# spcl/gms

Hardware: AMD Instinct MI355X
Metric: edges-intersected/sec + achieved HBM GB/s, RMAT-26 triangle count @1/2/4/8 GPU (higher is better)
Workload: dtype int32 ids / uint64 counts

## Files before the change

### gms_amd/csrc/hip/device_graph.hip

```cpp
#include "device_graph.hpp"

#include <algorithm>
#include <mutex>
#include <array>
#include <chrono>
#include <cstdio>
#include <cstdlib>
#include <cstring>
#include <memory>
#include <new>
#include <random>

#include <rocprim/device/device_radix_sort.hpp>
#include <rocprim/device/device_scan.hpp>
#include <rocprim/device/device_segmented_radix_sort.hpp>
#include <rocprim/iterator/transform_iterator.hpp>

#include "../host/gmsx_internal.hpp"

namespace gmsx {

Ctx &ctx() {
    static Ctx c;
    return c;
// ... 173 lines not shown
            const uint32_t gap = uint32_t(row[i]) - cur;
            if (gap > 4095u) break;
            const int pos = 20 + 12 * (k - 1), word = pos >> 5, sh = pos & 31;
            w[word] |= gap << sh;
            if (sh > 20) w[word + 1] |= gap >> (32 - sh);
            ++k;
            cur = row[i];
            ++i;
        }
        w[0] |= uint32_t(k) << 16;
        if (emit) {
            emit[units * 4 + 0] = w[0]; emit[units * 4 + 1] = w[1]; emit[units * 4 + 2] = w[2]; emit[units * 4 + 3] = w[3];
        }
        ++units;
    }
    return units;
}
static constexpr int kHybridB[4] = {512, 1024, 2048, 4096};
__device__ inline int lower_bound_u16(const uint16_t *__restrict__ row, int len, uint32_t key) {
    int lo = 0, hi = len;
    while (lo < hi) {
        const int mid = (lo + hi) >> 1;
        if (uint32_t(row[mid]) < key) lo = mid + 1; else hi = mid;
    }
    return lo;
}
__global__ void k_srow_sizes(int64_t n, const int64_t *__restrict__ hoff, const uint16_t *__restrict__ hadj, const int32_t *__restrict__ dplus,
                             int32_t dense_limit, int delta_mode, int delta_pct, int gap12_mode, int hybrid_mode, int64_t *__restrict__ units_out,
                             int64_t *__restrict__ small_out, uint32_t *__restrict__ real_out, unsigned char *__restrict__ form_out,
                             int32_t *__restrict__ ksplit) {
    const int64_t v = int64_t(blockIdx.x) * blockDim.x + threadIdx.x;
    if (v > n) return;
    if (v == n) { units_out[2 * n] = 0; small_out[2 * n] = 0; return; }
    const int64_t b = hoff[v];
    const int len = int(hoff[v + 1] - b);
    uint32_t best = uint32_t((len + 7) / 8);
    int form = kFormList;
    if (len > 0 && v < dense_limit) {
        const uint32_t bits = uint32_t(bitset_words(int32_t(v)) / 4);
        if (bits * 16u + 32u < uint32_t(len) * 2u) { best = bits; form = kFormBitset; }
    }
    if (len > 0 && delta_mode > 0 && (delta_mode == 2 || len >= 24)) {
        const uint32_t d = delta_encode(hadj + b, len, nullptr);
        if ((delta_mode == 2 && form == kFormList) || d * 100u <= best * uint32_t(delta_pct)) { best = d; form = kFormDelta; }
    }
    if (len > 0 && gap12_mode > 0 && form == kFormList && (gap12_mode == 2 || len >= 24)) {
        const uint32_t d = gap12_encode(hadj + b, len, nullptr);
        if (gap12_mode == 2 || d * 100u <= best * 90u) { best = d; form = kFormGap12; }
    }
    uint32_t best2 = 0;
    int form2 = kFormList, ks = 0;
    if (hybrid_mode > 0 && len >= 32 && dplus[v] >= kHeavy && form != kFormBitset) {
        uint32_t tot = best;
        for (int t = 0; t < 4; ++t) {
            const int B = kHybridB[t];
            if (v <= B) break;
            const int k = lower_bound_u16(hadj + b, len, uint32_t(B));
            if (k * 2 <= B / 8 + 16) continue;
            const int rl = len - k;
            uint32_t r = uint32_t((rl + 7) / 8);
            int rf = kFormList;
            if (rl >= 24 && delta_mode > 0) {
                const uint32_t d = delta_encode(hadj + b + k, rl, nullptr);
                if (d * 100u <= r * uint32_t(delta_pct)) { r = d; rf = kFormDelta; }
            }
            const uint32_t cand = uint32_t(B / 128) + r;
            if (cand < tot && (hybrid_mode == 2 || cand * 100u <= best * 90u)) {
                tot = cand;
                ks = k;
                best2 = r;
                form2 = rf;
            }
        }
        if (ks > 0) {
            best = tot - best2;
            form = kFormBitset;
        }
    }
    ksplit[v] = ks;
    const uint32_t u2[2] = {best, best2};
    const int f2[2] = {form, form2};
    for (int sl = 0; sl < 2; ++sl) {
        const bool big = u2[sl] >= 8u;
        units_out[2 * v + sl] = big ? int64_t((u2[sl] + 7u) & ~7u) : 0;
        small_out[2 * v + sl] = big ? 0 : int64_t(u2[sl]);
        real_out[2 * v + sl] = u2[sl];
        form_out[2 * v + sl] = (unsigned char)f2[sl];
    }
}
__global__ void k_srow_fill(int64_t n, const int64_t *__restrict__ hoff, const uint16_t *__restrict__ hadj, const int64_t *__restrict__ bmoff,
                            const uint32_t *__restrict__ bmpool, const int64_t *__restrict__ uoff, const int64_t *__restrict__ soff,
                            const uint32_t *__restrict__ real, const unsigned char *__restrict__ form, const int32_t *__restrict__ ksplit,
                            unsigned long long *__restrict__ srow, unsigned long long *__restrict__ srow2, uint32_t *__restrict__ spool) {
    const int64_t v = int64_t(blockIdx.x) * blockDim.x + threadIdx.x;
    if (v >= n) return;
    const int64_t b = hoff[v];
    const int len = int(hoff[v + 1] - b);
    const int ks = ksplit[v];
    for (int sl = 0; sl < 2; ++sl) {
        const int64_t units = int64_t(real[2 * v + sl]);
        const int64_t u0 = units >= 8 ? uoff[2 * v + sl] : uoff[2 * n] + soff[2 * v + sl];
        const int fm = form[2 * v + sl];
        const unsigned long long d = units ? ((unsigned long long)u0 << 24) | ((unsigned long long)fm << 22) | (unsigned long long)units : 0ull;
        if (sl == 0) srow[v] = units ? d : ((unsigned long long)u0 << 24) | ((unsigned long long)fm << 22);
        else srow2[v] = d;
        if (units == 0) continue;
        uint32_t *dst = spool + u0 * 4;
        const uint16_t *row = hadj + b + (sl ? ks : 0);
        const int rl = sl ? len - ks : len;
        if (sl == 0 && ks > 0) {
            for (int64_t w = 0; w < units * 4; ++w) dst[w] = 0;
            for (int i = 0; i < ks; ++i) dst[row[i] >> 5] |= 1u << (row[i] & 31u);
        } else if (fm == kFormDelta) {
            delta_encode(row, rl, dst);
        } else if (fm == kFormGap12) {
            gap12_encode(row, rl, dst);
        } else if (fm == kFormBitset) {
            const uint32_t *src = bmpool + bmoff[v];
            for (int64_t w = 0; w < units * 4; ++w) dst[w] = src[w];
        } else {
            for (int64_t w = 0; w < units * 4; ++w) {
                const int i = int(w) * 2;
                const uint32_t lo = i < rl ? row[i] : 0xFFFFu, hi = i + 1 < rl ? row[i + 1] : 0xFFFFu;
                dst[w] = lo | (hi << 16);
            }
        }
    }
}

__device__ inline uint32_t tail_delta_encode(const int32_t *__restrict__ row, int len, uint32_t *__restrict__ emit) {
    uint32_t units = 0;
    int i = 0;
    while (i < len) {
        uint32_t w[4] = {uint32_t(row[i]), 0u, 0u, 0u};
        uint32_t cur = uint32_t(row[i]);
        int slot = 1;
        ++i;
        while (i < len && slot < 6) {
            const uint32_t gap = uint32_t(row[i]) - cur;
            if (gap > 65535u) break;
            w[1 + (slot >> 1)] |= gap << ((slot & 1) * 16);
            ++slot;
            cur = uint32_t(row[i]);
            ++i;
        }
        w[1] |= uint32_t(slot);
        if (emit) {
            emit[units * 4 + 0] = w[0]; emit[units * 4 + 1] = w[1]; emit[units * 4 + 2] = w[2]; emit[units * 4 + 3] = w[3];
        }
        ++units;
    }
    return units;
}
__global__ void k_trow_sizes(int64_t n, const int64_t *__restrict__ toff, const int32_t *__restrict__ tadj, int delta_mode,
                             int64_t *__restrict__ units_out, int64_t *__restrict__ small_out, uint32_t *__restrict__ real_out, unsigned char *__restrict__ form_out) {
    const int64_t v = int64_t(blockIdx.x) * blockDim.x + threadIdx.x;
    if (v > n) return;
    if (v == n) { units_out[n] = 0; small_out[n] = 0; return; }
    const int64_t b = toff[v];
    const int len = int(toff[v + 1] - b);
    uint32_t best = uint32_t((len + 3) / 4);
    int form = kFormList;
    if (len >= 8 && delta_mode > 0) {
        const uint32_t d = tail_delta_encode(tadj + b, len, nullptr);
        if (delta_mode == 2 || d * 100u <= best * 85u) { best = d; form = kFormDelta; }
    }
    const bool big = best >= 8u;
    units_out[v] = big ? int64_t((best + 7u) & ~7u) : 0;
    small_out[v] = big ? 0 : int64_t(best);
    real_out[v] = best;
    form_out[v] = (unsigned char)form;
}
__global__ void k_trow_fill(int64_t n, const int64_t *__restrict__ toff, const int32_t *__restrict__ tadj, const int64_t *__restrict__ uoff,
                            const int64_t *__restrict__ soff, const uint32_t *__restrict__ real, const unsigned char *__restrict__ form,
                            unsigned long long *__restrict__ trow, uint32_t *__restrict__ tpool) {
    const int64_t v = int64_t(blockIdx.x) * blockDim.x + threadIdx.x;
    if (v >= n) return;
    const int64_t units = int64_t(real[v]);
    const int64_t u0 = units >= 8 ? uoff[v] : uoff[n] + soff[v];
    trow[v] = ((unsigned long long)u0 << 24) | ((unsigned long long)form[v] << 22) | (unsigned long long)units;
    if (units == 0) return;
    uint32_t *dst = tpool + u0 * 4;
    const int64_t b = toff[v];
    const int64_t len = toff[v + 1] - b;
    if (form[v] == kFormDelta) tail_delta_encode(tadj + b, int(len), dst);
    else
        for (int64_t w = 0; w < units * 4; ++w) dst[w] = w < len ? uint32_t(tadj[b + w]) : 0xfffffffeu;
}

__global__ void k_dense_sizes(int32_t limit, const int32_t *__restrict__ dplus, int64_t *__restrict__ sizes) {
    const int32_t v = int32_t(blockIdx.x * blockDim.x + threadIdx.x);
    if (v < limit) sizes[v] = bitset_words(v);
    if (v == limit) sizes[v] = 0;
}
__global__ __launch_bounds__(256) void k_dense_fill(int32_t limit, const int64_t *__restrict__ hoff, const uint16_t *__restrict__ hadj,
                                                    const int64_t *__restrict__ toff, const int32_t *__restrict__ tadj,
                                                    const int64_t *__restrict__ bmoff, uint32_t *__restrict__ pool) {
    const int lane = threadIdx.x & 63;
    const int32_t wave0 = int32_t((int64_t(blockIdx.x) * blockDim.x + threadIdx.x) >> 6);
    const int32_t nwaves = int32_t((int64_t(gridDim.x) * blockDim.x) >> 6);
    for (int32_t v = wave0; v < limit; v += nwaves) {
        const int64_t b = bmoff[v];
        if (bmoff[v + 1] == b) continue;
        for (int64_t j = hoff[v] + lane; j < hoff[v + 1]; j += 64) {
            const uint32_t id = hadj[j];
            if (id != 0xFFFFu) atomicOr(&pool[b + (id >> 5)], 1u << (id & 31u));
        }
        for (int64_t j = toff[v] + lane; j < toff[v + 1]; j += 64) {
            const uint32_t id = uint32_t(tadj[j]);
            atomicOr(&pool[b + (id >> 5)], 1u << (id & 31u));
        }
    }
}
__global__ __launch_bounds__(256) void k_tail_split(int64_t n, const int64_t *__restrict__ toff, const int32_t *__restrict__ tadj, int32_t limit,
                                                    int32_t *__restrict__ tsplit) {
    const int lane = threadIdx.x & 63;
    const int64_t wave0 = (int64_t(blockIdx.x) * blockDim.x + threadIdx.x) >> 6;
    const int64_t nwaves = (int64_t(gridDim.x) * blockDim.x) >> 6;
    for (int64_t u = wave0; u < n; u += nwaves) {
        int c = 0;
        for (int64_t j = toff[u] + lane; j < toff[u + 1]; j += 64) c += tadj[j] < limit;
        for (int s = 32; s > 0; s >>= 1) c += __shfl_down(c, s);
        if (lane == 0) tsplit[u] = c;
    }
}

__global__ void k_order_keys(int64_t n, const int32_t *__restrict__ dplus, int32_t *__restrict__ keys, int32_t *__restrict__ vals) {
    const int64_t i = int64_t(blockIdx.x) * blockDim.x + threadIdx.x;
    if (i < n) {
        keys[i] = dplus[i];
        vals[i] = int32_t(i);
    }
}

__global__ void k_warm(unsigned long long *p) {
    if (p) p[0] = 0;
}
__global__ void k_count_ge(int64_t n, const int32_t *__restrict__ order, const int32_t *__restrict__ dplus, int32_t thr, int64_t *__restrict__ out) {
    int64_t lo = 0, hi = n;
    while (lo < hi) {
        const int64_t mid = (lo + hi) >> 1;
        if (dplus[order[mid]] >= thr) lo = mid + 1; else hi = mid;
    }
    out[0] = lo;
}
__global__ void k_task_limits(int64_t n, const unsigned long long *__restrict__ srow, const unsigned long long *__restrict__ srow2,
                              const unsigned long long *__restrict__ trow, uint32_t hub_max, uint32_t tail_max, unsigned long long *__restrict__ out) {
    const int64_t v = int64_t(blockIdx.x) * blockDim.x + threadIdx.x;
    if (v >= n) return;
    if ((srow[v] & 0x3fffffull) > hub_max || (srow2[v] & 0x3fffffull) > hub_max || (trow[v] & 0x3fffffull) > tail_max) atomicOr(out, 1ull);
}

static constexpr int kInlineChunk = 64;
static constexpr int kDefaultInlineFirst = 28;
static constexpr int kInlineFirstMax = 64;
__device__ __forceinline__ bool takes_inline(int32_t v, int32_t inline_limit, const int32_t *__restrict__ dplus) {
    return v < inline_limit || dplus[v] >= kHeavy;
}
template <bool FILL>
__global__ __launch_bounds__(256) void k_inline_rows(int64_t first, int64_t end, const int32_t *__restrict__ order, const int64_t *__restrict__ hoff,
                                                     const uint16_t *__restrict__ hadj, const int64_t *__restrict__ toff, const int32_t *__restrict__ tadj,
                                                     const int32_t *__restrict__ dplus, int32_t inline_limit, int inline_first, const int32_t *__restrict__ opos, int nparts, int part,
                                                     unsigned long long *__restrict__ cnt_h,
                                                     unsigned long long *__restrict__ cnt_t, const int64_t *__restrict__ ihoff,
                                                     const int64_t *__restrict__ itoff, int64_t base_h, uint16_t *__restrict__ pool_h, int64_t base_t,
                                                     int32_t *__restrict__ pool_t) {
    const int lane = threadIdx.x & 63;
    const int64_t wave0 = (int64_t(blockIdx.x) * blockDim.x + threadIdx.x) >> 6;
    const int64_t nwaves = (int64_t(gridDim.x) * blockDim.x) >> 6;
    for (int64_t pos = first + wave0; pos < end; pos += nwaves) {
        const int32_t u = order[pos];
        const int64_t hb = hoff[u], tb = toff[u];
        const int first_u = dplus[u] >= kHeavy ? inline_first : kInlineFirstMax;
        const int hl = min(int(hoff[u + 1] - hb), first_u), tl = min(int(toff[u + 1] - tb), first_u - hl);
        int32_t mv = 0x7fffffff;
        if (lane < hl) {
            const uint32_t x = hadj[hb + lane];
            if (x != 0xFFFFu) mv = int32_t(x);
        } else if (lane - hl < tl) {
            mv = tadj[tb + (lane - hl)];
        }
        const bool valid = mv != 0x7fffffff, is_tail = valid && lane >= hl;
        const unsigned long long vmask = __ballot(valid);
        const int nhub = __popcll(__ballot(valid && lane < hl));
        const int below = __popcll(vmask & ((1ull << lane) - 1ull));
        const bool give = valid && below > 0 && takes_inline(mv, inline_limit, dplus);
        const bool mine = give && (nparts <= 1 || shard_of(opos[mv], nparts) == part);
        const int nh = mine ? (is_tail ? nhub : below) : 0;
        const int nt = mine && is_tail ? lane - hl : 0;
        if (!FILL) {
            if (nh) atomicAdd(&cnt_h[mv], (unsigned long long)nh);
            if (nt) atomicAdd(&cnt_t[mv], (unsigned long long)nt);
        } else {
            int64_t at_h = 0, at_t = 0;
            if (nh) at_h = (base_h + ihoff[mv]) * 8 + int64_t(atomicAdd(&cnt_h[mv], (unsigned long long)nh));
            if (nt) at_t = (base_t + itoff[mv]) * 4 + int64_t(atomicAdd(&cnt_t[mv], (unsigned long long)nt));
            for (int k = 0; k < nhub; ++k) {
                const int32_t x = __shfl(mv, k);
                if (k < nh) pool_h[at_h + k] = uint16_t(x);
            }
            for (int k = 0; k < tl; ++k) {
                const int32_t x = __shfl(mv, hl + k);
                if (k < nt) pool_t[at_t + k] = x;
            }
        }
    }
}
__global__ void k_inline_units(int64_t n, const unsigned long long *__restrict__ ids_h, const unsigned long long *__restrict__ ids_t,
                               int64_t *__restrict__ units_h, int64_t *__restrict__ units_t) {
    const int64_t v = int64_t(blockIdx.x) * blockDim.x + threadIdx.x;
    if (v > n) return;
    units_h[v] = v < n ? int64_t((ids_h[v] + 7) / 8) : 0;
    units_t[v] = v < n ? int64_t((ids_t[v] + 3) / 4) : 0;
}
static constexpr int kDefaultHotWindows = 0, kDefaultHotKB = 2048, kDefaultHotMin = 16;
__device__ __forceinline__ int64_t receiver_of(int32_t w, const int32_t *__restrict__ dplus, const int32_t *__restrict__ opos, const int64_t *__restrict__ lidx,
                                               int64_t n_heavy) {
    return dplus[w] >= kHeavy ? int64_t(opos[w]) : n_heavy + lidx[w];
}
__global__ void k_opos(int64_t n, const int32_t *__restrict__ order, int32_t *__restrict__ opos) {
    const int64_t p = int64_t(blockIdx.x) * blockDim.x + threadIdx.x;
    if (p < n) opos[order[p]] = int32_t(p);
}
__global__ void k_light_flags(int64_t limit, const int32_t *__restrict__ dplus, int64_t *__restrict__ flags) {
    const int64_t w = int64_t(blockIdx.x) * blockDim.x + threadIdx.x;
    if (w <= limit) flags[w] = (w < limit && dplus[w] < kHeavy) ? 1 : 0;
}
__global__ void k_recv_vertices(int64_t n_heavy, int64_t limit, const int32_t *__restrict__ order, const int32_t *__restrict__ dplus, const int64_t *__restrict__ lidx,
                                int32_t *__restrict__ recv_v) {
    const int64_t i = int64_t(blockIdx.x) * blockDim.x + threadIdx.x;
    if (i < n_heavy) recv_v[i] = order[i];
    if (i < limit && dplus[i] < kHeavy) recv_v[n_heavy + lidx[i]] = int32_t(i);
}
template <bool FILL>
__global__ void k_inline_entries(int64_t n, const int32_t *__restrict__ dplus, const int32_t *__restrict__ opos, const int64_t *__restrict__ lidx, int64_t n_heavy,
                                 int32_t inline_limit, const int64_t *__restrict__ ihoff, const int64_t *__restrict__ itoff, int64_t base_h, int64_t base_t,
                                 uint32_t *__restrict__ cnt, uint32_t *__restrict__ cur, const int64_t *__restrict__ hbeg, const int64_t *__restrict__ tbeg,
                                 TaskList htask, TaskList ttask, unsigned long long *__restrict__ totals, TcClasses cc) {
    const int kClasses = cc.count();
    const int64_t v = int64_t(blockIdx.x) * blockDim.x + threadIdx.x;
    if (v >= n) return;
    const int64_t uh = ihoff[v + 1] - ihoff[v], ut = itoff[v + 1] - itoff[v];
    if (uh == 0 && ut == 0) return;
    if (dplus[v] < kHeavy && v >= inline_limit) return;
    const int64_t p = receiver_of(int32_t(v), dplus, opos, lidx, n_heavy);
    uint32_t *c = cnt + p * kClasses;
    for (int64_t o = 0; o < uh; o += kInlineChunk) {
        const unsigned long long units = (unsigned long long)min(int64_t(kInlineChunk), uh - o);
        const unsigned long long d = ((unsigned long long)(base_h + ihoff[v] + o) << 24) | ((unsigned long long)kFormList << 22) | units;
        const int cls = hub_class(cc, d);
        if (!FILL) atomicAdd(&c[cls], 1u);
        else htask.put(hbeg[p] + c[cls] + atomicAdd(&cur[p * kClasses + cls], 1u), d);
    }
    for (int64_t o = 0; o < ut; o += kInlineChunk) {
        const unsigned long long units = (unsigned long long)min(int64_t(kInlineChunk), ut - o);
        const unsigned long long d = ((unsigned long long)(base_t + itoff[v] + o) << 24) | ((unsigned long long)kFormList << 22) | units;
        const int cls = tail_class(cc, d);
        if (!FILL) atomicAdd(&c[cls], 1u);
        else ttask.put(tbeg[p] + c[cls] + atomicAdd(&cur[p * kClasses + cls], 1u), d);
    }
    if (!FILL) {
        atomicAdd(&totals[0], (unsigned long long)((uh + kInlineChunk - 1) / kInlineChunk));
        atomicAdd(&totals[1], (unsigned long long)((ut + kInlineChunk - 1) / kInlineChunk));
    }
}
__global__ void k_list_sizes(int64_t n_recv, uint32_t *__restrict__ cnt, int64_t *__restrict__ hcnt, int64_t *__restrict__ tcnt, TcClasses cc) {
    const int kClasses = cc.count(), hub_end = cc.tail_base();
    const int64_t p = int64_t(blockIdx.x) * blockDim.x + threadIdx.x;
    if (p > n_recv) return;
    if (p == n_recv) { hcnt[p] = 0; tcnt[p] = 0; return; }
    uint32_t *c = cnt + p * kClasses;
    uint32_t run = 0;
    for (int k = 0; k < hub_end; ++k) { const uint32_t x = c[k]; c[k] = run; run += x; }
    hcnt[p] = run;
    run = 0;
    for (int k = hub_end; k < kClasses; ++k) { const uint32_t x = c[k]; c[k] = run; run += x; }
    tcnt[p] = run;
}

__global__ void k_ledge_count(int64_t first, int64_t end, const int32_t *__restrict__ order, const int64_t *__restrict__ toff, const int32_t *__restrict__ tadj,
                              const int32_t *__restrict__ tsplit, const int32_t *__restrict__ dplus, int64_t *__restrict__ cnt) {
    const int64_t pos = first + int64_t(blockIdx.x) * blockDim.x + threadIdx.x;
    if (pos > end) return;
    int64_t c = 0;
    if (pos < end) {
        const int32_t u = order[pos];
        const int64_t tb = toff[u];
        const int tl = int(toff[u + 1] - tb);
        for (int i = tsplit[u]; i < tl; ++i) c += dplus[tadj[tb + i]] < kHeavy ? 1 : 0;
    }
    cnt[pos - first] = c;
}
__global__ void k_ledge_fill(int64_t first, int64_t end, const int32_t *__restrict__ order, const int64_t *__restrict__ hoff, const int64_t *__restrict__ toff,
                             const int32_t *__restrict__ tadj, const int32_t *__restrict__ tsplit, const int32_t *__restrict__ dplus,
                             const int64_t *__restrict__ ebeg, int nparts, int part, uint4 *__restrict__ ledge) {
    const int64_t pos = first + int64_t(blockIdx.x) * blockDim.x + threadIdx.x;
    if (pos >= end) return;
    const int32_t u = order[pos];
    const int64_t hb = hoff[u], tb = toff[u];
    const int tl = int(toff[u + 1] - tb);
    const unsigned long long hu = (unsigned long long)hb | ((unsigned long long)(hoff[u + 1] - hb) << 40);
    int64_t e = ebeg[pos - first];
    for (int i = tsplit[u]; i < tl; ++i) {
        const int32_t v = tadj[tb + i];
        if (dplus[v] >= kHeavy) continue;
        if (nparts <= 1 || shard_of(e, nparts) == part) {
            const unsigned long long tu = (unsigned long long)tb | ((unsigned long long)i << 40);
            const unsigned long long hv = (unsigned long long)hoff[v] | ((unsigned long long)(hoff[v + 1] - hoff[v]) << 40);
            const unsigned long long tv = (unsigned long long)toff[v] | ((unsigned long long)(toff[v + 1] - toff[v]) << 40);
            const int64_t slot = nparts <= 1 ? e : e / nparts;
            ledge[2 * slot] = make_uint4(uint32_t(hu), uint32_t(hu >> 32), uint32_t(tu), uint32_t(tu >> 32));
            ledge[2 * slot + 1] = make_uint4(uint32_t(hv), uint32_t(hv >> 32), uint32_t(tv), uint32_t(tv >> 32));
        }
        ++e;
    }
}

__device__ __forceinline__ uint32_t cut_hub_units(const uint32_t *__restrict__ spool, unsigned long long d, int below, int32_t v) {
    const uint32_t units = uint32_t(d) & 0x3fffffu, form = (uint32_t(d) >> 22) & 3u;
    if (form == kFormList) return min(units, uint32_t(below + 7) / 8u);
    if (form == kFormBitset) return min(units, uint32_t(v + 127) / 128u);
    const uint4 *row = reinterpret_cast<const uint4 *>(spool) + (d >> 24);
    uint32_t lo = 0, hi = units;
    while (lo < hi) {
        const uint32_t mid = (lo + hi) >> 1;
        if (int32_t(row[mid].x & 0xffffu) < v) lo = mid + 1; else hi = mid;
    }
    return lo;
}
__device__ __forceinline__ uint32_t cut_tail_units(const uint32_t *__restrict__ tpool, unsigned long long d, int below, int32_t v) {
    const uint32_t units = uint32_t(d) & 0x3fffffu, form = (uint32_t(d) >> 22) & 3u;
    if (form != kFormDelta) return min(units, uint32_t(below + 3) / 4u);
    const uint4 *row = reinterpret_cast<const uint4 *>(tpool) + (d >> 24);
    uint32_t lo = 0, hi = units;
    while (lo < hi) {
        const uint32_t mid = (lo + hi) >> 1;
        if (int32_t(row[mid].x) < v) lo = mid + 1; else hi = mid;
    }
    return lo;
}
__device__ __forceinline__ uint32_t claim_by_class(uint32_t *ctr, int cls, bool active, int lane) {
    uint32_t mine = 0;
    unsigned long long todo = __ballot(active);
    while (todo) {
        const int leader = __ffsll((long long)todo) - 1;
        const int c = __builtin_amdgcn_readlane(cls, leader);
        const unsigned long long same = __ballot(active && cls == c);
        uint32_t base = 0;
        if (lane == leader) base = atomicAdd(&ctr[c], uint32_t(__popcll(same)));
        base = uint32_t(__builtin_amdgcn_readlane(int(base), leader));
        if (active && cls == c) mine = base + uint32_t(__popcll(same & ((1ull << lane) - 1ull)));
        todo &= ~same;
    }
    return mine;
}
template <bool FILL>
__global__ __launch_bounds__(256) void k_task_lists(int64_t n_heavy, const int32_t *__restrict__ order, const int64_t *__restrict__ hoff,
                                                    const uint16_t *__restrict__ hadj, const int64_t *__restrict__ toff, const int32_t *__restrict__ tadj,
                                                    const int32_t *__restrict__ dplus, const unsigned long long *__restrict__ srow,
                                                    const unsigned long long *__restrict__ srow2, const int32_t *__restrict__ ksplit,
                                                    const unsigned long long *__restrict__ trow, int two_sided, const int32_t *__restrict__ opos,
                                                    uint32_t *__restrict__ cnt, uint32_t *__restrict__ cur, const int64_t *__restrict__ hbeg,
                                                    const int64_t *__restrict__ tbeg, TaskList htask, TaskList ttask,
                                                    int32_t *__restrict__ tunits, unsigned long long *__restrict__ reversed, const uint32_t *__restrict__ spool,
                                                    const uint32_t *__restrict__ tpool, int32_t inline_limit, int inline_first, int nparts, int part, TcClasses cc) {
    const int kClasses = cc.count();
    const int lane = threadIdx.x & 63;
    const int64_t wave0 = (int64_t(blockIdx.x) * blockDim.x + threadIdx.x) >> 6;
    const int64_t nwaves = (int64_t(gridDim.x) * blockDim.x) >> 6;
    unsigned long long rev = 0;
    for (int64_t pos = wave0; pos < n_heavy; pos += nwaves) {
        const int32_t u = order[pos];
        const int64_t hb = hoff[u], tb = toff[u];
        const int hl = int(hoff[u + 1] - hb), tl = int(toff[u + 1] - tb);
        const unsigned long long du_s = srow[u], du_s2 = srow2[u], du_t = trow[u];
        const int ks_u = ksplit[u];
        uint32_t *cu = cnt + pos * kClasses, *ru = cur + pos * kClasses;
        const bool own_u = nparts <= 1 || shard_of(pos, nparts) == part;
        int kept = 0;
        for (int base = 0; base < hl + tl; base += 64) {
            const int i = base + lane;
            int32_t v = -1;
            if (i < hl) {
                const uint32_t x = hadj[hb + i];
                if (x != 0xFFFFu) v = int32_t(x);
            } else if (i < hl + tl) v = tadj[tb + i - hl];
            if (v >= 0 && i > 0 && i < inline_first && takes_inline(v, inline_limit, dplus)) v = -1;
            bool reverse = false;
            uint32_t ch = 0, ch2 = 0, ct = 0;
            if (v >= 0 && i > 0 && two_sided && dplus[v] >= kHeavy) {
                if (i < hl) {
                    ch = cut_hub_units(spool, du_s, i, v);
                    if (du_s2 && i > ks_u) ch2 = cut_hub_units(spool, du_s2, i - ks_u, v);
                } else {
                    ch = uint32_t(du_s) & 0x3fffffu;
                    ch2 = uint32_t(du_s2) & 0x3fffffu;
                }
                ct = (i < hl || toff[v + 1] == toff[v]) ? 0u : cut_tail_units(tpool, du_t, i - hl, v);
                const uint32_t keep = uint32_t(srow[v] & 0x3fffffull) + uint32_t(srow2[v] & 0x3fffffull) + (i > hl ? uint32_t(trow[v] & 0x3fffffull) : 0u);
                reverse = ch + ch2 + ct < keep;
            }
            const bool fwd = v >= 0 && !reverse && own_u;
            if (reverse && nparts > 1 && shard_of(opos[v], nparts) != part) v = -1;
            const unsigned long long fh = (fwd && i > 0) ? srow[v] : 0ull, fh2 = (fwd && i > 0) ? srow2[v] : 0ull, ft = (fwd && i > hl) ? trow[v] : 0ull;
            const bool fh_on = (fh & 0x3fffffull) != 0, fh2_on = (fh2 & 0x3fffffull) != 0, ft_on = (ft & 0x3fffffull) != 0;
            const uint32_t sh = claim_by_class(FILL ? ru : cu, hub_class(cc, fh), fh_on, lane);
            const uint32_t sh2 = claim_by_class(FILL ? ru : cu, hub_class(cc, fh2), fh2_on, lane);
            const uint32_t st = claim_by_class(FILL ? ru : cu, tail_class(cc, ft), ft_on, lane);
            if (FILL) {
                if (fh_on) htask.put(hbeg[pos] + cu[hub_class(cc, fh)] + sh, fh);
                if (fh2_on) htask.put(hbeg[pos] + cu[hub_class(cc, fh2)] + sh2, fh2);
                if (ft_on) ttask.put(tbeg[pos] + cu[tail_class(cc, ft)] + st, ft);
            }
            kept += __popcll(__ballot(fwd));
            if (v >= 0 && reverse) {
                const int64_t pv = opos[v];
                const unsigned long long rh = ch ? (du_s & ~0x3fffffull) | ch : 0ull, rh2 = ch2 ? (du_s2 & ~0x3fffffull) | ch2 : 0ull,
                                         rt = ct ? (du_t & ~0x3fffffull) | ct : 0ull;
                uint32_t *cv = cnt + pv * kClasses;
                if (!FILL) {
                    if (rh) atomicAdd(&cv[hub_class(cc, rh)], 1u);
                    if (rh2) atomicAdd(&cv[hub_class(cc, rh2)], 1u);
                    if (rt) atomicAdd(&cv[tail_class(cc, rt)], 1u);
                    atomicAdd(&tunits[pv], 1);
                    ++rev;
                } else {
                    uint32_t *rv = cur + pv * kClasses;
                    if (rh) htask.put(hbeg[pv] + cv[hub_class(cc, rh)] + atomicAdd(&rv[hub_class(cc, rh)], 1u), rh);
                    if (rh2) htask.put(hbeg[pv] + cv[hub_class(cc, rh2)] + atomicAdd(&rv[hub_class(cc, rh2)], 1u), rh2);
                    if (rt) ttask.put(tbeg[pv] + cv[tail_class(cc, rt)] + atomicAdd(&rv[tail_class(cc, rt)], 1u), rt);
                }
            }
        }
        if (!FILL && lane == 0 && kept) atomicAdd(&tunits[pos], kept);
    }
    if (!FILL) {
        for (int s = 32; s > 0; s >>= 1) rev += __shfl_down(rev, s);
        if (lane == 0 && rev) atomicAdd(reversed, rev);
    }
}
__global__ void k_item_counts(int64_t n_recv, const int64_t *__restrict__ lbeg, const uint32_t *__restrict__ cnt, TcClasses cc, int phases, int64_t *__restrict__ items) {
    const int64_t p = int64_t(blockIdx.x) * blockDim.x + threadIdx.x;
    if (p > n_recv) return;
    if (p == n_recv) { items[int64_t(phases) * n_recv] = 0; return; }
    for (int ph = 0; ph < phases; ++ph) {
        int64_t b = 0, e = lbeg[p + 1] - lbeg[p];
        if (phases > 1) hub_phase_range(cc, cnt + p * cc.count(), e, ph, &b, &e);
        items[int64_t(ph) * n_recv + p] = (e - b + kTaskChunk - 1) / kTaskChunk;
    }
}
__global__ void k_item_fill(int64_t n_recv, const int32_t *__restrict__ recv_v, const int32_t *__restrict__ opos, const int64_t *__restrict__ lbeg,
                            const int64_t *__restrict__ ioff, TaskList task, const int64_t *__restrict__ coff, int kind,
                            const uint32_t *__restrict__ cnt, TcClasses cc, int phases, gmsx_tc_item *__restrict__ items) {
    const int64_t p = int64_t(blockIdx.x) * blockDim.x + threadIdx.x;
    if (p >= n_recv) return;
    const int32_t w = recv_v[p];
    const uint64_t cont = uint64_t(coff[w]) | (uint64_t(coff[w + 1] - coff[w]) << 40);
    for (int ph = 0; ph < phases; ++ph) {
    int64_t b = 0, e = lbeg[p + 1] - lbeg[p];
    if (phases > 1) hub_phase_range(cc, cnt + p * cc.count(), e, ph, &b, &e);
    b += lbeg[p];
    e += lbeg[p];
    int64_t k = ioff[int64_t(ph) * n_recv + p];
    for (int64_t x = b; x < e; x += kTaskChunk, ++k) {
        const int ne = int(min(int64_t(kTaskChunk), e - x));
        gmsx_tc_item it{};
        it.bc = uint64_t(x) | (uint64_t(ne) << 40);
        it.cont = cont;
        it.pivot = w;
        it.pos = opos[w];
        it.kind = uint32_t(kind);
        for (int f = 0; f < 4; ++f) {
            int lo = 0, hi = ne;
            while (lo < hi) {
                const int mid = (lo + hi) >> 1;
                if (int((uint32_t(task.get(x + mid)) >> 22) & 3u) < f) lo = mid + 1; else hi = mid;
            }
            it.fbeg[f] = uint16_t(lo);
        }
        items[k] = it;
    }
    }
}

static int grid_for_waves(int64_t rows) {
    const int64_t want = (rows + 3) / 4;
    const int64_t cap = int64_t(ctx().compute_units > 0 ? ctx().compute_units : 256) * 32;
    return int(want < 1 ? 1 : (want > cap ? cap : want));
}

template <class T>
static int dmalloc(T **p, int64_t count, gmsx_graph *g, int line = __builtin_LINE()) {
    const size_t bytes = size_t(count > 0 ? count : 1) * sizeof(T);
    const bool trace = opt("MEM_TRACE") != nullptr;
    if (trace && g && bytes >= (1u << 20)) std::fprintf(stderr, "gmsx mem: device_graph.hip:%d %.3f GB (elements of %zu B)\n", line, double(bytes) * 1e-9, sizeof(T));
    if (g && g->tc_building && g->tc_limit_bytes > 0 && g->device_bytes + int64_t(bytes) - g->tc_base_bytes > g->tc_limit_bytes) {
        *p = nullptr;
        return GMSX_ERR_DEVICE_MEM;
    }
    if (hipMalloc(reinterpret_cast<void **>(p), bytes) != hipSuccess) {
        (void)hipGetLastError();
        *p = nullptr;
        return GMSX_ERR_DEVICE_MEM;
    }
    if (g) g->device_bytes += int64_t(bytes);
    return GMSX_OK;
}

struct DevGuard {
    void *p;
    ~DevGuard() { (void)hipFree(p); }
};

static void free_tc(gmsx_graph *g) {
    auto drop = [](auto *&p) {
        (void)hipFree(p);
        p = nullptr;
    };
    drop(g->tsplit); drop(g->srow); drop(g->srow2); drop(g->ksplit); drop(g->spool); drop(g->trow); drop(g->htask.lo); drop(g->htask.hi); drop(g->ttask.lo); drop(g->ttask.hi); drop(g->hitem); drop(g->titem); drop(g->tunits);
    drop(g->ledge); drop(g->tpool); drop(g->shard_hitem); drop(g->shard_titem);
    g->shard_idx_part = g->shard_idx_nparts = -1;
    g->device_bytes -= g->tc_bytes;
    g->tc_bytes = 0;
    g->tc_ready = false;
    g->htask_entries = g->ttask_entries = g->hitems = g->titems = g->inline_hentries = g->inline_tentries = 0;
    g->n_ledge = g->ledge_total = 0;
    g->task_reverse = g->inline_units = g->spool_units = g->tpool_units = 0;
    g->stats_part = g->stats_nparts = -1;
}

static void free_graph(gmsx_graph *g) {
    if (!g) return;
    (void)hipFree(g->off);
    (void)hipFree(g->adj);
    (void)hipFree(g->newid);
    (void)hipFree(g->oldid);
    (void)hipFree(g->hoff);
    (void)hipFree(g->hadj);
    (void)hipFree(g->toff);
    (void)hipFree(g->tadj);
    (void)hipFree(g->bmoff);
    (void)hipFree(g->bmpool);
    (void)hipFree(g->tsplit);
    (void)hipFree(g->srow);
    (void)hipFree(g->srow2);
    (void)hipFree(g->ksplit);
    (void)hipFree(g->spool);
    (void)hipFree(g->trow);
    (void)hipFree(g->htask.lo);
    (void)hipFree(g->htask.hi);
    (void)hipFree(g->ttask.lo);
    (void)hipFree(g->ttask.hi);
    (void)hipFree(g->hitem);
    (void)hipFree(g->titem);
    (void)hipFree(g->tunits);
    (void)hipFree(g->shard_hitem);
    (void)hipFree(g->shard_titem);
    (void)hipFree(g->ledge);
    (void)hipFree(g->tpool);
    (void)hipFree(g->dplus);
    (void)hipFree(g->order);
    (void)hipFree(g->kc_rel);
    (void)hipFree(g->kc_aoff);
    (void)hipFree(g->kc_arena);
    (void)hipFree(g->kc_rec);
    (void)hipFree(g->kc_item);
    (void)hipFree(g->kc_relt);
    (void)hipFree(g->kc_rect);
    (void)hipFree(g->kc_itemt);
    (void)hipFree(g->scratch);
    (void)hipFree(g->acc);
    delete g;
}

int exclusive_scan_i64(const int64_t *in, int64_t *out, int64_t count, hipStream_t s) {
    size_t tmp_bytes = 0;
    GMSX_HIP(rocprim::exclusive_scan(nullptr, tmp_bytes, in, out, int64_t(0), size_t(count), rocprim::plus<int64_t>(), s));
    void *tmp = nullptr;
    GMSX_HIP(hipMalloc(&tmp, tmp_bytes ? tmp_bytes : 8));
    DevGuard g_tmp{tmp};
    GMSX_HIP(rocprim::exclusive_scan(tmp, tmp_bytes, in, out, int64_t(0), size_t(count), rocprim::plus<int64_t>(), s));
    GMSX_HIP(hipStreamSynchronize(s));
    return GMSX_OK;
}

struct OffsetMinus {
    int64_t base;
    __host__ __device__ int64_t operator()(int64_t x) const { return x - base; }
};
__global__ void k_lower_bound_i64(int64_t count, const int64_t *__restrict__ a, int64_t target, int64_t *__restrict__ out) {
    int64_t lo = 0, hi = count;
    while (lo < hi) {
        const int64_t mid = (lo + hi) >> 1;
        if (a[mid] < target) lo = mid + 1; else hi = mid;
    }
    out[0] = lo;
}
template <class K>
static int sort_rows(K *keys, int64_t entries, int64_t n, const int64_t *d_off, int end_bit, hipStream_t s) {
    if (n <= 0 || entries <= 0) return GMSX_OK;
    int64_t chunk = int64_t(1) << 31;
    if (const char *e = opt("SORT_CHUNK")) {
        const long long v = std::atoll(e);
        if (v > 0) chunk = v;
    }
    int64_t *d_v = nullptr;
    GMSX_HIP(hipMalloc(reinterpret_cast<void **>(&d_v), sizeof(int64_t)));
    DevGuard g_v{d_v};
    GMSX_HIP(hipStreamSynchronize(s));
    int64_t v0 = 0, base = 0;
    while (v0 < n) {
        int64_t v1 = n;
        if (entries - base > chunk) {
            hipLaunchKernelGGL(k_lower_bound_i64, dim3(1), dim3(1), 0, s, n + 1, d_off, base + chunk + 1, d_v);
            GMSX_HIP(hipStreamSynchronize(s));
            GMSX_HIP(hipMemcpy(&v1, d_v, sizeof(int64_t), hipMemcpyDeviceToHost));
            v1 = std::max(v0 + 1, std::min(n, v1 - 1));
        }
        int64_t end = 0;
        GMSX_HIP(hipMemcpy(&end, d_off + v1, sizeof(int64_t), hipMemcpyDeviceToHost));
        const int64_t cnt = end - base;
        if (cnt >= (int64_t(1) << 32)) return GMSX_ERR_UNSUPPORTED;
        if (cnt > 0) {
            K *sorted = nullptr;
            GMSX_HIP(hipMalloc(reinterpret_cast<void **>(&sorted), size_t(cnt) * sizeof(K)));
            DevGuard g_sorted{sorted};
            auto begin = rocprim::make_transform_iterator(d_off + v0, OffsetMinus{base});
            auto endit = rocprim::make_transform_iterator(d_off + v0 + 1, OffsetMinus{base});
            size_t tmp_bytes = 0;
            GMSX_HIP(rocprim::segmented_radix_sort_keys(nullptr, tmp_bytes, keys + base, sorted, unsigned(cnt), unsigned(v1 - v0), begin, endit, 0, end_bit, s));
            void *tmp = nullptr;
            GMSX_HIP(hipMalloc(&tmp, tmp_bytes ? tmp_bytes : 8));
            DevGuard g_tmp{tmp};
            GMSX_HIP(rocprim::segmented_radix_sort_keys(tmp, tmp_bytes, keys + base, sorted, unsigned(cnt), unsigned(v1 - v0), begin, endit, 0, end_bit, s));
            GMSX_HIP(hipMemcpyAsync(keys + base, sorted, size_t(cnt) * sizeof(K), hipMemcpyDeviceToDevice, s));
            GMSX_HIP(hipStreamSynchronize(s));
        }
        v0 = v1;
        base = end;
    }
    return GMSX_OK;
}

template <class K, class V>
static int sort_segment_pairs(K *keys, V *vals, int64_t entries, int64_t n, const int64_t *d_off, int end_bit, hipStream_t s) {
    if (n <= 0 || entries <= 0) return GMSX_OK;
    int64_t chunk = int64_t(1) << 31;
    if (const char *e = opt("SORT_CHUNK")) {
        const long long v = std::atoll(e);
        if (v > 0) chunk = v;
    }
    int64_t *d_v = nullptr;
    GMSX_HIP(hipMalloc(reinterpret_cast<void **>(&d_v), sizeof(int64_t)));
    DevGuard g_v{d_v};
    GMSX_HIP(hipStreamSynchronize(s));
    int64_t v0 = 0, base = 0;
    while (v0 < n) {
        int64_t v1 = n;
        if (entries - base > chunk) {
            hipLaunchKernelGGL(k_lower_bound_i64, dim3(1), dim3(1), 0, s, n + 1, d_off, base + chunk + 1, d_v);
            GMSX_HIP(hipStreamSynchronize(s));
            GMSX_HIP(hipMemcpy(&v1, d_v, sizeof(int64_t), hipMemcpyDeviceToHost));
            v1 = std::max(v0 + 1, std::min(n, v1 - 1));
        }
        int64_t end = 0;
        GMSX_HIP(hipMemcpy(&end, d_off + v1, sizeof(int64_t), hipMemcpyDeviceToHost));
        const int64_t cnt = end - base;
        if (cnt >= (int64_t(1) << 32)) return GMSX_ERR_UNSUPPORTED;
        if (cnt > 0) {
            K *k_out = nullptr;
            V *v_out = nullptr;
            GMSX_HIP(hipMalloc(reinterpret_cast<void **>(&k_out), size_t(cnt) * sizeof(K)));
            DevGuard g_ko{k_out};
            GMSX_HIP(hipMalloc(reinterpret_cast<void **>(&v_out), size_t(cnt) * sizeof(V)));
            DevGuard g_vo{v_out};
            auto begin = rocprim::make_transform_iterator(d_off + v0, OffsetMinus{base});
            auto endit = rocprim::make_transform_iterator(d_off + v0 + 1, OffsetMinus{base});
            size_t tmp_bytes = 0;
            GMSX_HIP(rocprim::segmented_radix_sort_pairs(nullptr, tmp_bytes, keys + base, k_out, vals + base, v_out, unsigned(cnt), unsigned(v1 - v0), begin, endit, 0,
                                                         end_bit, s));
            void *tmp = nullptr;
            GMSX_HIP(hipMalloc(&tmp, tmp_bytes ? tmp_bytes : 8));
            DevGuard g_tmp{tmp};
            GMSX_HIP(rocprim::segmented_radix_sort_pairs(tmp, tmp_bytes, keys + base, k_out, vals + base, v_out, unsigned(cnt), unsigned(v1 - v0), begin, endit, 0,
                                                         end_bit, s));
            GMSX_HIP(hipMemcpyAsync(vals + base, v_out, size_t(cnt) * sizeof(V), hipMemcpyDeviceToDevice, s));
            GMSX_HIP(hipStreamSynchronize(s));
        }
        v0 = v1;
        base = end;
    }
    return GMSX_OK;
}

struct PhaseTimer {
    hipStream_t s;
    bool on;
    std::chrono::steady_clock::time_point t0;
    const char *what;
    PhaseTimer(hipStream_t st, const char *w) : s(st), on(opt("TIMING") != nullptr), t0(std::chrono::steady_clock::now()), what(w) {}
    void mark(const char *phase) {
        if (!on) return;
        (void)hipStreamSynchronize(s);
        const auto t1 = std::chrono::steady_clock::now();
        std::fprintf(stderr, "[gmsx %s] %-28s %8.1f ms\n", what, phase, std::chrono::duration<double, std::milli>(t1 - t0).count());
        t0 = t1;
    }
};

static constexpr size_t kH2dChunk = size_t(64) << 20;
struct H2dStage {
    char *pin[2] = {nullptr, nullptr};
// ... 36 lines not shown
    for (size_t at = 0; at < bytes; at += kChunk, b ^= 1) {
        const size_t n = std::min(kChunk, bytes - at);
        if (used[b]) GMSX_HIP(hipEventSynchronize(st.ev[b]));
        char *to = st.pin[b];
        parallel_memcpy(to, static_cast<const char *>(src) + at, n);
        GMSX_HIP(hipMemcpyAsync(static_cast<char *>(dst) + at, to, n, hipMemcpyHostToDevice, s));
        GMSX_HIP(hipEventRecord(st.ev[b], s));
        used[b] = true;
    }
    return GMSX_OK;
}

static int build_device_sets(gmsx_graph *g, uint32_t flags) {
    hipStream_t s = ctx().stream;
    PhaseTimer pt(s, "base build");
    const int64_t n = g->n;
    if (int rc = dmalloc(&g->scratch, 16, g)) return rc;
    if (int rc = dmalloc(&g->acc, kAccWords, g)) return rc;
    GMSX_HIP(hipMemsetAsync(g->scratch, 0, 16 * sizeof(unsigned long long), s));

    const int check_sym = (flags & GMSX_UPLOAD_TRUSTED) ? 0 : 1;
    static const std::array<unsigned long long, 2> sym_keys = []() noexcept {
        try {
            std::random_device rd;
            return std::array<unsigned long long, 2>{((unsigned long long)rd() << 32) | rd(), ((unsigned long long)rd() << 32) | rd()};
        } catch (...) {
            const unsigned long long t = (unsigned long long)std::chrono::steady_clock::now().time_since_epoch().count();
            const unsigned long long a = (unsigned long long)reinterpret_cast<uintptr_t>(&t);
            return std::array<unsigned long long, 2>{t * 0x9E3779B97F4A7C15ull ^ a, (a * 0xC2B2AE3D27D4EB4Full) ^ (t << 17)};
        }
    }();
    if (n > 0)
        hipLaunchKernelGGL(k_validate, dim3(grid_for_waves(n)), dim3(256), 0, s, n, g->off, g->adj, check_sym, sym_keys[0], sym_keys[1], g->scratch);
    unsigned long long acc[7] = {0, 0, 0, 0, 0, 0, 0};
    GMSX_HIP(hipMemcpyAsync(acc, g->scratch, sizeof(acc), hipMemcpyDeviceToHost, s));
    GMSX_HIP(hipStreamSynchronize(s));
    if (check_sym && (acc[3] != acc[4] || acc[5] != acc[6])) acc[0] |= 8;
    if (!(flags & GMSX_UPLOAD_TRUSTED) && acc[0] != 0) return GMSX_ERR_NOT_CANONICAL;
    if ((flags & GMSX_UPLOAD_TRUSTED) && (acc[0] & 2)) return GMSX_ERR_NOT_CANONICAL;
    if (!(flags & GMSX_UPLOAD_TRUSTED) && (g->nnz & 1)) return GMSX_ERR_NOT_CANONICAL;
    g->alg_elements = acc[1];
    g->max_deg = int32_t(acc[2]);
    g->m = g->nnz / 2;

    pt.mark("validate");
    const unsigned tb = unsigned((n + 255) / 256);
    if (int rc = dmalloc(&g->newid, n, g)) return rc;
    if (int rc = dmalloc(&g->oldid, n, g)) return rc;
    if (n > 0) {
        unsigned long long *k_in = nullptr, *k_out = nullptr;
        if (int rc = dmalloc(&k_in, n, nullptr)) return rc;
        DevGuard g1{k_in};
        if (int rc = dmalloc(&k_out, n, nullptr)) return rc;
        DevGuard g2{k_out};
        hipLaunchKernelGGL(k_rank_keys, dim3(tb), dim3(256), 0, s, n, g->off, k_in);
        size_t tmp_bytes = 0;
        GMSX_HIP(rocprim::radix_sort_keys_desc(nullptr, tmp_bytes, k_in, k_out, size_t(n), 0, 64, s));
        void *tmp = nullptr;
        GMSX_HIP(hipMalloc(&tmp, tmp_bytes ? tmp_bytes : 8));
        DevGuard g3{tmp};
        GMSX_HIP(rocprim::radix_sort_keys_desc(tmp, tmp_bytes, k_in, k_out, size_t(n), 0, 64, s));
        hipLaunchKernelGGL(k_assign_ids, dim3(tb), dim3(256), 0, s, n, k_out, g->oldid, g->newid);
        GMSX_HIP(hipStreamSynchronize(s));
    }

    pt.mark("rank ids");
    int hub_limit = int((flags >> 8) & 0xffffu);
    if (hub_limit == 0 || hub_limit > kHub) hub_limit = kHub;
    int64_t *hcnt = nullptr, *tcnt = nullptr;
    if (int rc = dmalloc(&hcnt, n + 1, nullptr)) return rc;
    DevGuard g_h{hcnt};
    if (int rc = dmalloc(&tcnt, n + 1, nullptr)) return rc;
    DevGuard g_t{tcnt};
    GMSX_HIP(hipMemsetAsync(hcnt, 0, size_t(n + 1) * sizeof(int64_t), s));
    GMSX_HIP(hipMemsetAsync(tcnt, 0, size_t(n + 1) * sizeof(int64_t), s));
    if (int rc = dmalloc(&g->dplus, n, g)) return rc;
    if (n > 0)
        hipLaunchKernelGGL(k_count_parts, dim3(grid_for_waves(n)), dim3(256), 0, s, n, g->off, g->adj, g->newid, hub_limit, hcnt, tcnt, g->dplus);
    if (int rc = dmalloc(&g->hoff, n + 1, g)) return rc;
    if (int rc = dmalloc(&g->toff, n + 1, g)) return rc;
    if (int rc = exclusive_scan_i64(hcnt, g->hoff, n + 1, s)) return rc;
    if (int rc = exclusive_scan_i64(tcnt, g->toff, n + 1, s)) return rc;
    GMSX_HIP(hipMemcpy(&g->hub_entries, g->hoff + n, sizeof(int64_t), hipMemcpyDeviceToHost));
    GMSX_HIP(hipMemcpy(&g->tail_entries, g->toff + n, sizeof(int64_t), hipMemcpyDeviceToHost));

    if (int rc = dmalloc(&g->hadj, g->hub_entries + 8, g)) return rc;
    if (int rc = dmalloc(&g->tadj, g->tail_entries + 4, g)) return rc;
    GMSX_HIP(hipMemsetAsync(g->hadj + g->hub_entries, 0xff, 8 * sizeof(uint16_t), s));
    GMSX_HIP(hipMemsetAsync(g->tadj + g->tail_entries, 0xff, 4 * sizeof(int32_t), s));
    if (n > 0)
        hipLaunchKernelGGL(k_fill_parts, dim3(grid_for_waves(n)), dim3(256), 0, s, n, g->off, g->adj, g->newid, hub_limit, g->hoff, g->toff,
                           g->hadj, g->tadj);

    pt.mark("containers count+fill");
    if (int rc = sort_rows(g->hadj, g->hub_entries, n, g->hoff, 16, s)) return rc;
    if (int rc = sort_rows(g->tadj, g->tail_entries, n, g->toff, 32, s)) return rc;
    g->rows_sorted = true;

    pt.mark("row sorts");
    g->dense_limit = int32_t(std::min<int64_t>(n, hub_limit));
    g->bitset_limit = g->dense_limit;
    {
        const int32_t K = g->bitset_limit;
        int64_t *sizes = nullptr;
        if (int rc = dmalloc(&sizes, int64_t(K) + 1, nullptr)) return rc;
        DevGuard g_sz{sizes};
        if (int rc = dmalloc(&g->bmoff, int64_t(K) + 1, g)) return rc;
        hipLaunchKernelGGL(k_dense_sizes, dim3(unsigned(K / 256 + 1)), dim3(256), 0, s, K, g->dplus, sizes);
        if (int rc = exclusive_scan_i64(sizes, g->bmoff, int64_t(K) + 1, s)) return rc;
        GMSX_HIP(hipMemcpy(&g->bmpool_words, g->bmoff + K, sizeof(int64_t), hipMemcpyDeviceToHost));
        if (int rc = dmalloc(&g->bmpool, g->bmpool_words + 4, g)) return rc;
        GMSX_HIP(hipMemsetAsync(g->bmpool, 0, size_t(g->bmpool_words + 4) * sizeof(uint32_t), s));
        if (K > 0 && g->bmpool_words > 0)
            hipLaunchKernelGGL(k_dense_fill, dim3(grid_for_waves(K)), dim3(256), 0, s, K, g->hoff, g->hadj, g->toff, g->tadj, g->bmoff, g->bmpool);
    }
    pt.mark("bitsets");
    if (int rc = dmalloc(&g->order, n, g)) return rc;
    if (n > 0) {
        int32_t *keys_in = nullptr, *vals_in = nullptr, *keys_out = nullptr;
        if (int rc = dmalloc(&keys_out, n, nullptr)) return rc;
        DevGuard g_ko{keys_out};
        if (int rc = dmalloc(&keys_in, n, nullptr)) return rc;
        DevGuard g_ki{keys_in};
        if (int rc = dmalloc(&vals_in, n, nullptr)) return rc;
        DevGuard g_vi{vals_in};
        hipLaunchKernelGGL(k_order_keys, dim3(tb), dim3(256), 0, s, n, g->dplus, keys_in, vals_in);
        size_t tmp_bytes = 0;
        GMSX_HIP(rocprim::radix_sort_pairs_desc(nullptr, tmp_bytes, keys_in, keys_out, vals_in, g->order, size_t(n), 0, 32, s));
        void *tmp = nullptr;
        GMSX_HIP(hipMalloc(&tmp, tmp_bytes ? tmp_bytes : 8));
        DevGuard g_tmp{tmp};
        GMSX_HIP(rocprim::radix_sort_pairs_desc(tmp, tmp_bytes, keys_in, keys_out, vals_in, g->order, size_t(n), 0, 32, s));
        int32_t top = 0;
        GMSX_HIP(hipMemcpyAsync(&top, keys_out, sizeof(int32_t), hipMemcpyDeviceToHost, s));
        GMSX_HIP(hipStreamSynchronize(s));
        g->max_dplus = top;
    }

    pt.mark("d+ order");
    GMSX_HIP(hipStreamSynchronize(s));
    GMSX_HIP(hipGetLastError());
    g->hub_limit = hub_limit;
    g->upload_flags = flags;
    return GMSX_OK;
}

static int build_tc_sets(gmsx_graph *g) {
    hipStream_t s = ctx().stream;
    PhaseTimer pt(s, "tc build");
    const int64_t n = g->n;
    const uint32_t flags = g->upload_flags;
    const int hub_limit = g->hub_limit;
    const unsigned tb = unsigned((n + 255) / 256);
    int32_t *opos = nullptr;
    if (int rc = dmalloc(&opos, n + 1, nullptr)) return rc;
    DevGuard g_opos{opos};
    if (n > 0) hipLaunchKernelGGL(k_opos, dim3(tb), dim3(256), 0, s, n, g->order, opos);
    {
        int64_t want = std::min<int64_t>(524288, n / 256);
        bool forced = false;
        if (const char *e = opt("INLINE_LIMIT")) {
            const long long v = std::atoll(e);
            if (v >= 0 && v <= (1ll << 31) - 1) { want = v; forced = true; }
        }
        if (!forced && ((flags >> 8) & 0xffffu)) want = int64_t(4) * hub_limit;
        g->inline_limit = int32_t(std::min<int64_t>(n, std::max<int64_t>(want, g->dense_limit)));
        g->inline_first = kDefaultInlineFirst;
        if (const char *e = opt("TC_INLINE_FIRST")) g->inline_first = std::max(1, std::min(kInlineFirstMax, std::atoi(e)));
        if (int rc = dmalloc(&g->tsplit, n, g)) return rc;
        if (n > 0) hipLaunchKernelGGL(k_tail_split, dim3(grid_for_waves(n)), dim3(256), 0, s, n, g->toff, g->tadj, g->inline_limit, g->tsplit);
    }

    pt.mark("tail split");
    int64_t n_heavy = 0, n_work = 0;
    unsigned long long *inl_h = nullptr, *inl_t = nullptr;
    int64_t *ihoff = nullptr, *itoff = nullptr;
    if (int rc = dmalloc(&inl_h, n + 1, nullptr)) return rc;
    DevGuard g_inl_h{inl_h};
    if (int rc = dmalloc(&inl_t, n + 1, nullptr)) return rc;
    DevGuard g_inl_t{inl_t};
    if (int rc = dmalloc(&ihoff, n + 1, nullptr)) return rc;
    DevGuard g_ihoff{ihoff};
    if (int rc = dmalloc(&itoff, n + 1, nullptr)) return rc;
    DevGuard g_itoff{itoff};
    int64_t inline_h_units = 0, inline_t_units = 0;
    {
        if (n > 0) {
            int64_t *d_cnt = nullptr;
            if (int rc = dmalloc(&d_cnt, 2, nullptr)) return rc;
            DevGuard g_c{d_cnt};
            hipLaunchKernelGGL(k_count_ge, dim3(1), dim3(1), 0, s, n, g->order, g->dplus, int32_t(kHeavy), d_cnt);
            hipLaunchKernelGGL(k_count_ge, dim3(1), dim3(1), 0, s, n, g->order, g->dplus, int32_t(2), d_cnt + 1);
            GMSX_HIP(hipStreamSynchronize(s));
            int64_t h[2] = {0, 0};
            GMSX_HIP(hipMemcpy(h, d_cnt, sizeof(h), hipMemcpyDeviceToHost));
            n_heavy = h[0];
            n_work = h[1];
        }
        GMSX_HIP(hipMemsetAsync(inl_h, 0, size_t(n + 1) * sizeof(unsigned long long), s));
        GMSX_HIP(hipMemsetAsync(inl_t, 0, size_t(n + 1) * sizeof(unsigned long long), s));
        if (n_work > 0)
            hipLaunchKernelGGL(k_inline_rows<false>, dim3(grid_for_waves(n_work)), dim3(256), 0, s, int64_t(0), n_work, g->order, g->hoff, g->hadj,
                               g->toff, g->tadj, g->dplus, g->inline_limit, g->inline_first, opos, g->shard_nparts, g->shard_part, inl_h, inl_t, ihoff, itoff, int64_t(0), static_cast<uint16_t *>(nullptr),
                               int64_t(0), static_cast<int32_t *>(nullptr));
        int64_t *uh = nullptr, *ut = nullptr;
        if (int rc = dmalloc(&uh, n + 1, nullptr)) return rc;
        DevGuard g_uh{uh};
        if (int rc = dmalloc(&ut, n + 1, nullptr)) return rc;
        DevGuard g_ut{ut};
        hipLaunchKernelGGL(k_inline_units, dim3(unsigned(n / 256 + 1)), dim3(256), 0, s, n, inl_h, inl_t, uh, ut);
        if (int rc = exclusive_scan_i64(uh, ihoff, n + 1, s)) return rc;
        if (int rc = exclusive_scan_i64(ut, itoff, n + 1, s)) return rc;
        GMSX_HIP(hipMemcpy(&inline_h_units, ihoff + n, sizeof(int64_t), hipMemcpyDeviceToHost));
        GMSX_HIP(hipMemcpy(&inline_t_units, itoff + n, sizeof(int64_t), hipMemcpyDeviceToHost));
        g->inline_units = inline_h_units + inline_t_units;
    }

    pt.mark("inline row sizes");
    int64_t inline_h_base = 0, inline_t_base = 0;
    {
        int delta_mode = g->rows_sorted ? 1 : 0;
        if (const char *e = opt("TC_DELTA")) {
            const int v = std::atoi(e);
            if (v >= 0 && v <= 2 && g->rows_sorted) delta_mode = v;
        }
        int delta_pct = 85;
        if (const char *e = opt("TC_DELTA_PCT")) {
            const int v = std::atoi(e);
            if (v >= 10 && v <= 100) delta_pct = v;
        }
        int gap12_mode = 0;
        if (const char *e = opt("TC_GAP12")) {
            const int v = std::atoi(e);
            if (v >= 0 && v <= 2 && g->rows_sorted) gap12_mode = v;
        }
        int hybrid_mode = 0;
        if (const char *e = opt("TC_HYBRID")) {
            const int v = std::atoi(e);
            if (v >= 0 && v <= 2 && g->rows_sorted) hybrid_mode = v;
        }
        int64_t *units = nullptr, *uoff = nullptr, *small = nullptr, *soff = nullptr;
        uint32_t *real = nullptr;
        unsigned char *form = nullptr;
        const int64_t n2 = 2 * n;
        if (int rc = dmalloc(&units, n2 + 1, nullptr)) return rc;
        DevGuard g_u{units};
        if (int rc = dmalloc(&uoff, n2 + 1, nullptr)) return rc;
        DevGuard g_o{uoff};
        if (int rc = dmalloc(&small, n2 + 1, nullptr)) return rc;
        DevGuard g_s{small};
        if (int rc = dmalloc(&soff, n2 + 1, nullptr)) return rc;
        DevGuard g_so{soff};
        if (int rc = dmalloc(&real, n2 + 1, nullptr)) return rc;
        DevGuard g_r{real};
        if (int rc = dmalloc(&form, n2 + 1, nullptr)) return rc;
        DevGuard g_f{form};
        if (int rc = dmalloc(&g->ksplit, n + 1, g)) return rc;
        hipLaunchKernelGGL(k_srow_sizes, dim3(unsigned(n / 256 + 1)), dim3(256), 0, s, n, g->hoff, g->hadj, g->dplus, g->dense_limit, delta_mode, delta_pct, gap12_mode,
                           hybrid_mode, units, small, real, form, g->ksplit);
        if (int rc = exclusive_scan_i64(units, uoff, n2 + 1, s)) return rc;
        if (int rc = exclusive_scan_i64(small, soff, n2 + 1, s)) return rc;
        int64_t big_units = 0, small_units = 0;
        GMSX_HIP(hipMemcpy(&big_units, uoff + n2, sizeof(int64_t), hipMemcpyDeviceToHost));
        GMSX_HIP(hipMemcpy(&small_units, soff + n2, sizeof(int64_t), hipMemcpyDeviceToHost));
        g->spool_units = big_units + small_units + inline_h_units;
        inline_h_base = big_units + small_units;
        if (g->spool_units >= (int64_t(1) << 40)) return GMSX_ERR_DEVICE_MEM;
        if (int rc = dmalloc(&g->srow, n, g)) return rc;
        if (int rc = dmalloc(&g->srow2, n, g)) return rc;
        if (int rc = dmalloc(&g->spool, (g->spool_units + kPoolSlack) * 4, g)) return rc;
        GMSX_HIP(hipMemsetAsync(g->spool, 0, size_t((g->spool_units + kPoolSlack) * 4) * sizeof(uint32_t), s));
        if (inline_h_units > 0) GMSX_HIP(hipMemsetAsync(g->spool + inline_h_base * 4, 0xff, size_t(inline_h_units) * 16, s));
        if (n > 0)
            hipLaunchKernelGGL(k_srow_fill, dim3(unsigned((n + 255) / 256)), dim3(256), 0, s, n, g->hoff, g->hadj, g->bmoff, g->bmpool, uoff, soff, real, form,
                               g->ksplit, g->srow, g->srow2, g->spool);
        GMSX_HIP(hipStreamSynchronize(s));
    }
    {
        int delta_mode = g->rows_sorted ? 1 : 0;
        if (const char *e = opt("TC_TAIL_DELTA")) {
            const int v = std::atoi(e);
            if (v >= 0 && v <= 2 && g->rows_sorted) delta_mode = v;
        }
        int64_t *units = nullptr, *uoff = nullptr, *small = nullptr, *soff = nullptr;
        uint32_t *real = nullptr;
        unsigned char *form = nullptr;
        if (int rc = dmalloc(&units, n + 1, nullptr)) return rc;
        DevGuard g_u{units};
        if (int rc = dmalloc(&uoff, n + 1, nullptr)) return rc;
        DevGuard g_o{uoff};
        if (int rc = dmalloc(&small, n + 1, nullptr)) return rc;
        DevGuard g_s{small};
        if (int rc = dmalloc(&soff, n + 1, nullptr)) return rc;
        DevGuard g_so{soff};
        if (int rc = dmalloc(&real, n + 1, nullptr)) return rc;
        DevGuard g_r{real};
        if (int rc = dmalloc(&form, n + 1, nullptr)) return rc;
        DevGuard g_f{form};
        hipLaunchKernelGGL(k_trow_sizes, dim3(unsigned(n / 256 + 1)), dim3(256), 0, s, n, g->toff, g->tadj, delta_mode, units, small, real, form);
        if (int rc = exclusive_scan_i64(units, uoff, n + 1, s)) return rc;
        if (int rc = exclusive_scan_i64(small, soff, n + 1, s)) return rc;
        int64_t big_units = 0, small_units = 0;
        GMSX_HIP(hipMemcpy(&big_units, uoff + n, sizeof(int64_t), hipMemcpyDeviceToHost));
        GMSX_HIP(hipMemcpy(&small_units, soff + n, sizeof(int64_t), hipMemcpyDeviceToHost));
        inline_t_base = big_units + small_units;
        g->tpool_units = inline_t_base + inline_t_units;
        if (g->tpool_units >= (int64_t(1) << 40)) return GMSX_ERR_DEVICE_MEM;
        if (int rc = dmalloc(&g->trow, n, g)) return rc;
        if (int rc = dmalloc(&g->tpool, (g->tpool_units + kPoolSlack) * 4, g)) return rc;
        GMSX_HIP(hipMemsetD32Async(reinterpret_cast<hipDeviceptr_t>(g->tpool), int(0xFFFFFFFEu), size_t(g->tpool_units + kPoolSlack) * 4, s));
        if (n > 0)
            hipLaunchKernelGGL(k_trow_fill, dim3(unsigned((n + 255) / 256)), dim3(256), 0, s, n, g->toff, g->tadj, uoff, soff, real, form, g->trow, g->tpool);
        GMSX_HIP(hipStreamSynchronize(s));
    }

    pt.mark("tail stream rows");
    if (n_work > 0) {
        GMSX_HIP(hipMemsetAsync(inl_h, 0, size_t(n + 1) * sizeof(unsigned long long), s));
        GMSX_HIP(hipMemsetAsync(inl_t, 0, size_t(n + 1) * sizeof(unsigned long long), s));
        hipLaunchKernelGGL(k_inline_rows<true>, dim3(grid_for_waves(n_work)), dim3(256), 0, s, int64_t(0), n_work, g->order, g->hoff, g->hadj, g->toff,
                           g->tadj, g->dplus, g->inline_limit, g->inline_first, opos, g->shard_nparts, g->shard_part, inl_h, inl_t, ihoff, itoff, inline_h_base, reinterpret_cast<uint16_t *>(g->spool),
                           inline_t_base, reinterpret_cast<int32_t *>(g->tpool));
    }
    pt.mark("inline rows fill");
    {
        const int64_t nl = n_work - n_heavy;
        g->n_ledge = g->ledge_total = 0;
        if (nl > 0) {
            int64_t *ecnt = nullptr, *ebeg = nullptr;
            if (int rc = dmalloc(&ecnt, nl + 1, nullptr)) return rc;
            DevGuard g_ec{ecnt};
            if (int rc = dmalloc(&ebeg, nl + 1, nullptr)) return rc;
            DevGuard g_eb{ebeg};
            hipLaunchKernelGGL(k_ledge_count, dim3(unsigned(nl / 256 + 1)), dim3(256), 0, s, n_heavy, n_work, g->order, g->toff, g->tadj, g->tsplit, g->dplus, ecnt);
            if (int rc = exclusive_scan_i64(ecnt, ebeg, nl + 1, s)) return rc;
            GMSX_HIP(hipMemcpy(&g->ledge_total, ebeg + nl, sizeof(int64_t), hipMemcpyDeviceToHost));
            const int np = g->shard_nparts > 1 ? g->shard_nparts : 1, pp = g->shard_nparts > 1 ? g->shard_part : 0;
            {
                const int64_t full = g->ledge_total / np, rem = g->ledge_total % np;
                g->n_ledge = np <= 1 ? g->ledge_total : full + (((full & 1) ? np - 1 - pp : pp) < rem ? 1 : 0);
            }
            if (int rc = dmalloc(&g->ledge, 2 * g->n_ledge + 2, g)) return rc;
            hipLaunchKernelGGL(k_ledge_fill, dim3(unsigned(nl / 256 + 1)), dim3(256), 0, s, n_heavy, n_work, g->order, g->hoff, g->toff, g->tadj, g->tsplit, g->dplus, ebeg,
                               np, pp, g->ledge);
            GMSX_HIP(hipStreamSynchronize(s));
        }
    }
    pt.mark("light pivot list");
    {
        int two_sided = 1;
        if (const char *e = opt("TC_TWO_SIDED")) two_sided = std::atoi(e) != 0;
        const unsigned vb = unsigned(n / 256 + 1);
        const int64_t L = g->inline_limit;
        int64_t *lflag = nullptr, *lidx = nullptr;
        if (int rc = dmalloc(&lflag, L + 1, nullptr)) return rc;
        DevGuard g_lf{lflag};
        if (int rc = dmalloc(&lidx, L + 1, nullptr)) return rc;
        DevGuard g_li{lidx};
        hipLaunchKernelGGL(k_light_flags, dim3(unsigned(L / 256 + 1)), dim3(256), 0, s, L, g->dplus, lflag);
        if (int rc = exclusive_scan_i64(lflag, lidx, L + 1, s)) return rc;
        int64_t n_light_recv = 0;
        GMSX_HIP(hipMemcpy(&n_light_recv, lidx + L, sizeof(int64_t), hipMemcpyDeviceToHost));
        const int64_t n_recv = n_heavy + n_light_recv;
        int32_t *recv_v = nullptr;
        if (int rc = dmalloc(&recv_v, n_recv + 1, nullptr)) return rc;
        DevGuard g_rv{recv_v};
        if (std::max<int64_t>(n_heavy, L) > 0)
            hipLaunchKernelGGL(k_recv_vertices, dim3(unsigned(std::max<int64_t>(n_heavy, L) / 256 + 1)), dim3(256), 0, s, n_heavy, L, g->order, g->dplus, lidx, recv_v);
        {
            auto env_int = [](const char *name, int dflt) { return int(opt_int(name, dflt)); };
            g->tc_hot_windows = std::max(0, std::min(kMaxHotWindows, env_int("TC_HOT_WINDOWS", kDefaultHotWindows)));
            g->tc_window_units = uint32_t(std::max(1, env_int("TC_HOT_KB", kDefaultHotKB))) * 64u;
            g->tc_hot_min = std::max(1, env_int("TC_HOT_MIN", kDefaultHotMin));
        }
        const TcClasses cc{g->tc_hot_windows, g->tc_window_units, g->tc_hot_min};
        const int kClasses = cc.count();
        uint32_t *cnt = nullptr, *cur = nullptr;
        if (int rc = dmalloc(&cnt, n_recv * kClasses + 1, nullptr)) return rc;
        DevGuard g_cnt{cnt};
        if (int rc = dmalloc(&cur, n_recv * kClasses + 1, nullptr)) return rc;
        DevGuard g_cur{cur};
        GMSX_HIP(hipMemsetAsync(cnt, 0, size_t(n_recv * kClasses + 1) * sizeof(uint32_t), s));
        GMSX_HIP(hipMemsetAsync(cur, 0, size_t(n_recv * kClasses + 1) * sizeof(uint32_t), s));
        if (int rc = dmalloc(&g->tunits, n_heavy + 1, g)) return rc;
        GMSX_HIP(hipMemsetAsync(g->tunits, 0, size_t(n_heavy + 1) * sizeof(int32_t), s));
        unsigned long long *totals = nullptr;
        if (int rc = dmalloc(&totals, 4, nullptr)) return rc;
        DevGuard g_tot{totals};
        GMSX_HIP(hipMemsetAsync(totals, 0, 4 * sizeof(unsigned long long), s));
        int64_t *hcnt = nullptr, *tcnt = nullptr, *hbeg = nullptr, *tbeg = nullptr;
        if (int rc = dmalloc(&hcnt, n_recv + 1, nullptr)) return rc;
        DevGuard g_hc{hcnt};
        if (int rc = dmalloc(&tcnt, n_recv + 1, nullptr)) return rc;
        DevGuard g_tc{tcnt};
        if (int rc = dmalloc(&hbeg, n_recv + 1, nullptr)) return rc;
        DevGuard g_hb{hbeg};
        if (int rc = dmalloc(&tbeg, n_recv + 1, nullptr)) return rc;
        DevGuard g_tb{tbeg};
        const int grid = grid_for_waves(n_heavy);
        if (g->spool_units + kPoolSlack >= (int64_t(1) << 32) || g->tpool_units + kPoolSlack >= (int64_t(1) << 32)) return GMSX_ERR_DEVICE_MEM;
        {
            uint32_t hub_max = kTaskHubUnitsMax, tail_max = kTaskTailUnitsMax;
            if (const char *e = opt("TC_TEST_MAX_UNITS")) hub_max = tail_max = uint32_t(std::max(1, std::atoi(e)));
            if (n > 0) hipLaunchKernelGGL(k_task_limits, dim3(vb), dim3(256), 0, s, n, g->srow, g->srow2, g->trow, hub_max, tail_max, totals + 3);
        }
        if (n > 0)
            hipLaunchKernelGGL(k_inline_entries<false>, dim3(vb), dim3(256), 0, s, n, g->dplus, opos, lidx, n_heavy, g->inline_limit, ihoff, itoff, inline_h_base,
                               inline_t_base, cnt, cur, hbeg, tbeg, TaskList{}, TaskList{}, totals, cc);
        if (n_heavy > 0)
            hipLaunchKernelGGL(k_task_lists<false>, dim3(grid), dim3(256), 0, s, n_heavy, g->order, g->hoff, g->hadj, g->toff, g->tadj, g->dplus, g->srow, g->srow2, g->ksplit, g->trow,
                               two_sided, opos, cnt, cur, hbeg, tbeg, TaskList{}, TaskList{}, g->tunits,
                               totals + 2, g->spool, g->tpool, g->inline_limit, g->inline_first, g->shard_nparts, g->shard_part, cc);
        pt.mark("task lists count");
        hipLaunchKernelGGL(k_list_sizes, dim3(unsigned(n_recv / 256 + 1)), dim3(256), 0, s, n_recv, cnt, hcnt, tcnt, cc);
        if (int rc = exclusive_scan_i64(hcnt, hbeg, n_recv + 1, s)) return rc;
        if (int rc = exclusive_scan_i64(tcnt, tbeg, n_recv + 1, s)) return rc;
        unsigned long long tot[4] = {0, 0, 0, 0};
        GMSX_HIP(hipMemcpy(&g->htask_entries, hbeg + n_recv, sizeof(int64_t), hipMemcpyDeviceToHost));
        GMSX_HIP(hipMemcpy(&g->ttask_entries, tbeg + n_recv, sizeof(int64_t), hipMemcpyDeviceToHost));
        GMSX_HIP(hipMemcpy(tot, totals, sizeof(tot), hipMemcpyDeviceToHost));
        if (tot[3]) return GMSX_ERR_UNSUPPORTED;
        g->inline_hentries = int64_t(tot[0]);
        g->inline_tentries = int64_t(tot[1]);
        g->task_reverse = int64_t(tot[2]);
        if (g->htask_entries >= (int64_t(1) << 40) || g->ttask_entries >= (int64_t(1) << 40)) return GMSX_ERR_DEVICE_MEM;
        if (int rc = dmalloc(&g->htask.lo, g->htask_entries + 2, g)) return rc;
        if (int rc = dmalloc(&g->htask.hi, g->htask_entries + 2, g)) return rc;
        if (int rc = dmalloc(&g->ttask.lo, g->ttask_entries + 2, g)) return rc;
        if (int rc = dmalloc(&g->ttask.hi, g->ttask_entries + 2, g)) return rc;
        if (n > 0)
            hipLaunchKernelGGL(k_inline_entries<true>, dim3(vb), dim3(256), 0, s, n, g->dplus, opos, lidx, n_heavy, g->inline_limit, ihoff, itoff, inline_h_base,
                               inline_t_base, cnt, cur, hbeg, tbeg, g->htask, g->ttask, totals, cc);
        if (n_heavy > 0)
            hipLaunchKernelGGL(k_task_lists<true>, dim3(grid), dim3(256), 0, s, n_heavy, g->order, g->hoff, g->hadj, g->toff, g->tadj, g->dplus, g->srow, g->srow2, g->ksplit, g->trow,
                               two_sided, opos, cnt, cur, hbeg, tbeg, g->htask, g->ttask, g->tunits, totals + 2, g->spool, g->tpool, g->inline_limit, g->inline_first, g->shard_nparts, g->shard_part, cc);
        pt.mark("task lists fill");
        const int hub_phases = cc.hub_phases();
        const int64_t slots = int64_t(hub_phases) * n_recv;
        int64_t *icnt = nullptr, *ioff = nullptr;
        if (int rc = dmalloc(&icnt, slots + 1, nullptr)) return rc;
        DevGuard g_ic{icnt};
        if (int rc = dmalloc(&ioff, slots + 1, nullptr)) return rc;
        DevGuard g_io{ioff};
        const unsigned rb = unsigned(n_recv / 256 + 1);
        hipLaunchKernelGGL(k_item_counts, dim3(rb), dim3(256), 0, s, n_recv, hbeg, cnt, cc, hub_phases, icnt);
        if (int rc = exclusive_scan_i64(icnt, ioff, slots + 1, s)) return rc;
        GMSX_HIP(hipMemcpy(&g->hitems, ioff + slots, sizeof(int64_t), hipMemcpyDeviceToHost));
        if (int rc = dmalloc(&g->hitem, g->hitems + 1, g)) return rc;
        if (n_recv > 0) hipLaunchKernelGGL(k_item_fill, dim3(rb), dim3(256), 0, s, n_recv, recv_v, opos, hbeg, ioff, g->htask, g->hoff, 0, cnt, cc, hub_phases, g->hitem);
        hipLaunchKernelGGL(k_item_counts, dim3(rb), dim3(256), 0, s, n_recv, tbeg, cnt, cc, 1, icnt);
        if (int rc = exclusive_scan_i64(icnt, ioff, n_recv + 1, s)) return rc;
        GMSX_HIP(hipMemcpy(&g->titems, ioff + n_recv, sizeof(int64_t), hipMemcpyDeviceToHost));
        if (int rc = dmalloc(&g->titem, g->titems + 1, g)) return rc;
        if (n_recv > 0) hipLaunchKernelGGL(k_item_fill, dim3(rb), dim3(256), 0, s, n_recv, recv_v, opos, tbeg, ioff, g->ttask, g->toff, 1, cnt, cc, 1, g->titem);
        if (g->hitems >= (int64_t(1) << 31) || g->titems >= (int64_t(1) << 31)) return GMSX_ERR_DEVICE_MEM;
        GMSX_HIP(hipStreamSynchronize(s));
    }
    pt.mark("work items");
    GMSX_HIP(hipStreamSynchronize(s));
    GMSX_HIP(hipGetLastError());
    {
        auto drop = [&](auto *&p, size_t bytes) {
            if (!p) return;
            (void)hipFree(p);
            p = nullptr;
            g->device_bytes -= int64_t(bytes);
        };
        const size_t nn = size_t(n > 0 ? n : 1);
        drop(g->tsplit, nn * sizeof(int32_t));
        drop(g->srow2, nn * sizeof(unsigned long long));
        const char *keep = opt("TC_KEEP_ROWS");
        if (!(keep && std::atoi(keep) != 0)) {
            drop(g->srow, nn * sizeof(unsigned long long));
            drop(g->trow, nn * sizeof(unsigned long long));
        }
        drop(g->ksplit, size_t(n + 1) * sizeof(int32_t));
    }
    return GMSX_OK;
}

static int build_tc_once(gmsx_graph *g) {
    g->tc_base_bytes = g->device_bytes;
    g->tc_building = true;
    const int rc = build_tc_sets(g);
    g->tc_building = false;
    g->tc_bytes = g->device_bytes - g->tc_base_bytes;
    if (rc) {
        free_tc(g);
        return rc;
    }
    g->tc_ready = true;
    return GMSX_OK;
}

int ensure_tc(const gmsx_graph *cg) {
    gmsx_graph *g = const_cast<gmsx_graph *>(cg);
    if (g->tc_ready) return GMSX_OK;
    if (const char *e = opt("TC_MEM_LIMIT_MB")) {
        const long long v = std::atoll(e);
        g->tc_limit_bytes = v > 0 ? int64_t(v) << 20 : 0;
    }
    int rc = build_tc_once(g);
    if (rc == GMSX_ERR_DEVICE_MEM && g->shard_nparts == 1) {
        (void)hipGetLastError();
        for (int k = 2; k <= 4096 && rc == GMSX_ERR_DEVICE_MEM; k *= 2) {
            g->shard_part = 0;
            g->shard_nparts = k;
            rc = build_tc_once(g);
            if (rc == GMSX_OK) g->tc_passes = k;
        }
        if (rc) {
            g->shard_part = 0;
            g->shard_nparts = 1;
        }
    }
    return rc;
}

__global__ void k_shard_flags(int64_t n_items, const gmsx_tc_item *__restrict__ items, int nparts, int part, int64_t *__restrict__ flags) {
    const int64_t i = int64_t(blockIdx.x) * blockDim.x + threadIdx.x;
    if (i <= n_items) flags[i] = (i < n_items && shard_of(items[i].pos, nparts) == part) ? 1 : 0;
}
__global__ void k_shard_scatter(int64_t n_items, const int64_t *__restrict__ flags, const int64_t *__restrict__ slot, const gmsx_tc_item *__restrict__ items,
                                gmsx_tc_item *__restrict__ out) {
    const int64_t i = int64_t(blockIdx.x) * blockDim.x + threadIdx.x;
    if (i < n_items && flags[i]) out[slot[i]] = items[i];
}
int tc_shard_items(const gmsx_graph *g, int part, int nparts) {
    if (g->shard_idx_part == part && g->shard_idx_nparts == nparts) return GMSX_OK;
    hipStream_t s = ctx().stream;
    (void)hipFree(g->shard_hitem);
    (void)hipFree(g->shard_titem);
    g->shard_hitem = g->shard_titem = nullptr;
    g->shard_idx_part = g->shard_idx_nparts = -1;
    auto one = [&](const gmsx_tc_item *items, int64_t n_items, gmsx_tc_item **idx, int64_t *count) -> int {
        *count = 0;
        if (n_items == 0) return GMSX_OK;
        int64_t *flags = nullptr, *slot = nullptr;
        if (int rc = dmalloc(&flags, n_items + 1, nullptr)) return rc;
        DevGuard g_f{flags};
        if (int rc = dmalloc(&slot, n_items + 1, nullptr)) return rc;
        DevGuard g_s{slot};
        hipLaunchKernelGGL(k_shard_flags, dim3(unsigned(n_items / 256 + 1)), dim3(256), 0, s, n_items, items, nparts, part, flags);
        if (int rc = exclusive_scan_i64(flags, slot, n_items + 1, s)) return rc;
        GMSX_HIP(hipMemcpy(count, slot + n_items, sizeof(int64_t), hipMemcpyDeviceToHost));
        if (int rc = dmalloc(idx, *count + 1, nullptr)) return rc;
        hipLaunchKernelGGL(k_shard_scatter, dim3(unsigned(n_items / 256 + 1)), dim3(256), 0, s, n_items, flags, slot, items, *idx);
        GMSX_HIP(hipStreamSynchronize(s));
        return GMSX_OK;
    };
    if (int rc = one(g->hitem, g->hitems, &g->shard_hitem, &g->shard_hitems)) return rc;
    if (int rc = one(g->titem, g->titems, &g->shard_titem, &g->shard_titems)) return rc;
    g->shard_idx_part = part;
    g->shard_idx_nparts = nparts;
    return GMSX_OK;
}

int ensure_tc_shard(const gmsx_graph *cg, int part, int nparts) {
    gmsx_graph *g = const_cast<gmsx_graph *>(cg);
    if (g->tc_ready && g->shard_part == part && g->shard_nparts == nparts) return GMSX_OK;
    free_tc(g);
    g->shard_part = part;
    g->shard_nparts = nparts;
    return build_tc_once(g);
}

int count_dplus_ge(const gmsx_graph *g, int32_t threshold, int64_t *out) {
    if (g->n == 0) {
        *out = 0;
        return GMSX_OK;
    }
    for (int i = 0; i < g->ge_used; ++i)
        if (g->ge_thr[i] == threshold) {
            *out = g->ge_cnt[i];
            return GMSX_OK;
        }
    hipStream_t s = ctx().stream;
    hipLaunchKernelGGL(k_count_ge, dim3(1), dim3(1), 0, s, g->n, g->order, g->dplus, threshold, reinterpret_cast<int64_t *>(g->scratch + 8));
    GMSX_HIP(hipMemcpyAsync(out, g->scratch + 8, sizeof(int64_t), hipMemcpyDeviceToHost, s));
    GMSX_HIP(hipStreamSynchronize(s));
    if (g->ge_used < 40) {
        g->ge_thr[g->ge_used] = threshold;
        g->ge_cnt[g->ge_used] = *out;
        ++g->ge_used;
    }
// ... 170 lines not shown
```

### gms_amd/csrc/hip/device_graph.hpp

```cpp
#pragma once
#include <hip/hip_runtime.h>

#include <cstdint>

#include "gmsx.h"
#include "gmsx_internal.hpp"

#if !defined(GMSX_DEV_HOOKS) &&                                                                                                               \
    (defined(GMSX_KC_NO_PROBE) || defined(GMSX_KC_NO_HITS) || defined(GMSX_KC_NO_TAIL) || defined(GMSX_KC_NO_INNER) || defined(GMSX_KC_CELLS_ONLY) ||   \
     defined(GMSX_KC_NO_ROWS) || defined(GMSX_KC_BUILD_ONLY) || defined(GMSX_KC_NO_SLAB_CALL) || defined(GMSX_KC_NO_PAIRS) || defined(GMSX_KC_SLAB_ROW_SCAN) || \
     defined(GMSX_BK_AB) || defined(GMSX_BK_NO_HIT_ATOMICS) || defined(GMSX_BK_STATS) || defined(GMSX_TC_NO_PROBE) || defined(GMSX_TC_STAGING_ONLY))
#error "A/B switches need -DGMSX_DEV_HOOKS (tools/ab_lib.sh sets it); the default build of libgmsx.so carries none of them"
#endif

struct __attribute__((aligned(64))) gmsx_tc_item {
    uint64_t bc;
    uint64_t cont;
    int32_t pivot;
    int32_t pos;
    uint32_t kind;
    uint16_t fbeg[4];
    uint32_t reserved[7];
};
static_assert(sizeof(gmsx_tc_item) == 64, "work item record = one 64-byte line");
constexpr uint32_t kTaskHubUnitsMax = (1u << 14) - 1, kTaskTailUnitsMax = (1u << 15) - 1;
struct TaskList {
    uint32_t *lo = nullptr;
    uint16_t *hi = nullptr;
    bool tail = false;
    __host__ __device__ TaskList at(int64_t first) const { return TaskList{lo + first, hi + first, tail}; }
    __device__ __forceinline__ unsigned long long get(int64_t i) const {
        const uint32_t l = lo[i], h = hi[i];
        const unsigned long long first = ((unsigned long long)h << 16) | (l >> 16);
        const uint32_t form = tail ? ((l >> 15) & 1u) << 1 : (l >> 14) & 3u, units = tail ? l & kTaskTailUnitsMax : l & kTaskHubUnitsMax;
        return (first << 24) | ((unsigned long long)form << 22) | units;
    }
    __device__ __forceinline__ void put(int64_t i, unsigned long long d) const {
        const uint32_t first = uint32_t(d >> 24), form = (uint32_t(d) >> 22) & 3u, units = uint32_t(d) & 0x3fffffu;
        lo[i] = (first << 16) | (tail ? (form >> 1) << 15 : form << 14) | units;
        hi[i] = uint16_t(first >> 16);
    }
};
struct gmsx_graph {
    int64_t n = 0, nnz = 0, m = 0;
    int64_t *off = nullptr;
    int32_t *adj = nullptr;
    int32_t *newid = nullptr;
    int32_t *oldid = nullptr;
    int64_t *hoff = nullptr;
    uint16_t *hadj = nullptr;
    int64_t *toff = nullptr;
    int32_t *tadj = nullptr;
    int64_t *bmoff = nullptr;
    uint32_t *bmpool = nullptr;
    int32_t dense_limit = 0;
    int32_t bitset_limit = 0;
    unsigned long long *srow = nullptr;
    unsigned long long *srow2 = nullptr;
    int32_t *ksplit = nullptr;
    uint32_t *spool = nullptr;
    int64_t spool_units = 0;
    TaskList htask{nullptr, nullptr, false};
    TaskList ttask{nullptr, nullptr, true};
    int64_t htask_entries = 0, ttask_entries = 0;
    struct gmsx_tc_item *hitem = nullptr, *titem = nullptr;
    int64_t hitems = 0, titems = 0;
    int64_t inline_hentries = 0, inline_tentries = 0;
    mutable struct gmsx_tc_item *shard_hitem = nullptr, *shard_titem = nullptr;
    mutable int64_t shard_hitems = 0, shard_titems = 0;
    mutable int shard_idx_part = -1, shard_idx_nparts = -1;
    int32_t *tunits = nullptr;
    int64_t task_reverse = 0;
    uint4 *ledge = nullptr;
    int64_t n_ledge = 0, ledge_total = 0;
    int tc_hot_windows = 0;
    uint32_t tc_window_units = 1;
    int tc_hot_min = 0;
    int inline_first = 64;
    int32_t inline_limit = 0;
    int64_t inline_units = 0;
    unsigned long long *trow = nullptr;
    uint32_t *tpool = nullptr;
    int64_t tpool_units = 0;
    int32_t *tsplit = nullptr;
    int64_t dense_rows = 0, bmpool_words = 0;
    bool rows_sorted = false;
    int32_t *dplus = nullptr;
    int32_t *order = nullptr;
    int64_t hub_entries = 0, tail_entries = 0;
    int32_t max_dplus = 0;
    int32_t max_deg = 0;
    mutable bool kc_rev_tried = false;
    mutable uint32_t *kc_rel = nullptr;
    mutable int64_t *kc_aoff = nullptr;
    mutable uint32_t *kc_arena = nullptr;
    mutable ulonglong2 *kc_rec = nullptr;
    mutable uint4 *kc_item = nullptr;
    mutable uint32_t *kc_relt = nullptr;
    mutable ulonglong2 *kc_rect = nullptr;
    mutable uint4 *kc_itemt = nullptr;
    mutable int64_t kc_recst = 0, kc_itemst = 0;
    mutable int64_t kc_recs = 0, kc_items = 0, kc_arena_words = 0, kc_rev_bytes = 0;
    mutable double kc_rev_build_ms = 0.0;
    unsigned long long *scratch = nullptr;
    unsigned long long *acc = nullptr;
    mutable int32_t ge_thr[40] = {0};
    mutable int64_t ge_cnt[40] = {0};
    mutable int ge_used = 0;
    mutable int stats_part = -1, stats_nparts = -1;
    mutable uint64_t stats_units = 0, stats_probes = 0, stats_bytes = 0;
    int shard_part = 0, shard_nparts = 1;
    int tc_passes = 1;
    int64_t tc_limit_bytes = 0, tc_base_bytes = 0;
    bool tc_building = false;
    bool tc_ready = false;
    int64_t tc_bytes = 0;
    int hub_limit = 0;
    uint32_t upload_flags = 0;
    uint64_t alg_elements = 0;
    int64_t device_bytes = 0;
};

namespace gmsx {

static constexpr int kHub = 65535;
static constexpr int kBitmapWords = 2048;
static constexpr int kAccWords = 64 * 16 + 16;
static constexpr int kFormList = 0, kFormBitset = 1, kFormDelta = 2, kFormGap12 = 3;
static constexpr int kPoolSlack = 64;
static constexpr int kTaskChunk = 512;
static constexpr int kLenClasses = 12;
static constexpr int kHubClasses = 4 * kLenClasses, kTailClasses = 2 * kLenClasses;
static constexpr int kMaxHotWindows = 8;
struct TcClasses {
    int hot_windows;
    uint32_t window_units;
    int hot_min;
    __host__ __device__ int hub_phases() const { return hot_windows + 1; }
    __host__ __device__ int tail_base() const { return hub_phases() * kHubClasses; }
    __host__ __device__ int count() const { return tail_base() + kTailClasses; }
    __host__ __device__ int phase(unsigned long long d) const {
        if (hot_windows <= 0) return 0;
        const unsigned long long w = (d >> 24) / window_units;
        return w < (unsigned long long)hot_windows ? int(w) : hot_windows;
    }
};
__host__ __device__ inline int length_class(uint32_t u) {
    return u <= 16 ? (u <= 4 ? 0 : u <= 8 ? 1 : u <= 12 ? 2 : 3) : u <= 64 ? (u <= 24 ? 4 : u <= 32 ? 5 : u <= 48 ? 6 : 7) : (u <= 96 ? 8 : u <= 128 ? 9 : u <= 192 ? 10 : 11);
}
__host__ __device__ inline int hub_class(const TcClasses &cc, unsigned long long d) {
    return cc.phase(d) * kHubClasses + int((uint32_t(d) >> 22) & 3u) * kLenClasses + length_class(uint32_t(d) & 0x3fffffu);
}
__host__ __device__ inline int tail_class(const TcClasses &cc, unsigned long long d) {
    return cc.tail_base() + (((uint32_t(d) >> 22) & 3u) == 2u ? kLenClasses : 0) + length_class(uint32_t(d) & 0x3fffffu);
}
__host__ __device__ inline void hub_phase_range(const TcClasses &cc, const uint32_t *c, int64_t len, int ph, int64_t *b, int64_t *e) {
    int64_t start = 0;
    for (int q = 0;; ++q) {
        const int64_t end = q < cc.hot_windows ? int64_t(c[(q + 1) * kHubClasses]) : len;
        const bool own = q == cc.hot_windows || end - start >= cc.hot_min;
        if (q == ph) {
            *b = start;
            *e = own ? end : start;
            return;
        }
        if (own) start = end;
    }
}
__host__ __device__ inline int shard_of(int64_t pos, int nparts) {
    const int j = int(pos % nparts);
    return ((pos / nparts) & 1) ? nparts - 1 - j : j;
}
static constexpr int kHeavy = 64;
static constexpr int kDeltaIds = 14;

__host__ __device__ inline int64_t bitset_words(int32_t v) { return ((int64_t(v) + 31) / 32 + 3) & ~int64_t(3); }

struct Ctx {
    int device = -1;
    hipStream_t stream = nullptr;
    hipStream_t own_stream = nullptr;
    hipEvent_t ev[4] = {nullptr, nullptr, nullptr, nullptr};
    hipStream_t side[2] = {nullptr, nullptr};
    hipEvent_t ev_fork = nullptr, ev_join[2] = {nullptr, nullptr};
    int compute_units = 0;
};
Ctx &ctx();
int ensure_init();
int kclique_vertex_counts(const gmsx_graph *g, unsigned long long *d_counts, gmsx_stats *st);
int count_dplus_ge(const gmsx_graph *g, int32_t threshold, int64_t *out);
int exclusive_scan_i64(const int64_t *in, int64_t *out, int64_t count, hipStream_t s);
int ensure_tc(const gmsx_graph *g);
int ensure_tc_shard(const gmsx_graph *g, int part, int nparts);
int tc_shard_items(const gmsx_graph *g, int part, int nparts);
int tc_vertex_counts_device(const gmsx_graph *g, unsigned long long *d_counts, gmsx_stats *st);
int tc_full_partial(const gmsx_graph *g, int part, int nparts, uint64_t *partial, gmsx_stats *st);

__device__ __forceinline__ int uni32(int x) { return __builtin_amdgcn_readfirstlane(x); }
__device__ __forceinline__ uint32_t uni32(uint32_t x) { return uint32_t(__builtin_amdgcn_readfirstlane(int(x))); }
__device__ __forceinline__ int64_t uni64(int64_t x) {
    const uint32_t lo = uint32_t(__builtin_amdgcn_readfirstlane(int(uint32_t(uint64_t(x)))));
    const uint32_t hi = uint32_t(__builtin_amdgcn_readfirstlane(int(uint32_t(uint64_t(x) >> 32))));
    return int64_t((uint64_t(hi) << 32) | lo);
}
__device__ __forceinline__ unsigned long long uni64(unsigned long long x) { return (unsigned long long)uni64(int64_t(x)); }

#define GMSX_HIP(call)                                                    \
    do {                                                                  \
        hipError_t e_ = (call);                                           \
        if (e_ != hipSuccess) {                                           \
            (void)hipGetLastError();                                      \
            return e_ == hipErrorOutOfMemory ? GMSX_ERR_DEVICE_MEM : GMSX_ERR_KERNEL; \
        }                                                                 \
    } while (0)

}
```

### gms_amd/csrc/hip/tc.hip

```cpp
#include "device_graph.hpp"

#include <algorithm>
#include <type_traits>
#include <rocprim/device/device_radix_sort.hpp>
#include <rocprim/device/device_reduce.hpp>
#include <rocprim/device/device_reduce_by_key.hpp>
#include <cstdio>
#include <cstdlib>
#include <cstring>

namespace gmsx {

static constexpr int kAccSlots = 64;
static constexpr int kAccStride = 16;

struct __attribute__((packed, aligned(4))) u4u { uint32_t x, y, z, w; };

__device__ __forceinline__ int64_t readlane64(int64_t x, int l) {
    const uint32_t lo = __builtin_amdgcn_readlane(uint32_t(uint64_t(x)), l);
    const uint32_t hi = __builtin_amdgcn_readlane(uint32_t(uint64_t(x) >> 32), l);
    return int64_t((uint64_t(hi) << 32) | lo);
}

__device__ __forceinline__ uint32_t bit_lo(const uint32_t *bm, uint32_t p) {
    const uint32_t word = bm[(p >> 5) & 0x7ffu];
    return __builtin_amdgcn_ubfe(word, p, 1u);
}
__device__ __forceinline__ uint32_t bit_hi(const uint32_t *bm, uint32_t p) {
    const uint32_t q = p >> 16;
    const uint32_t word = bm[q >> 5];
    return __builtin_amdgcn_ubfe(word, q & 31u, 1u);
}
__device__ __forceinline__ uint32_t hub_hits8(const uint32_t *bm, u4u p) {
    return bit_lo(bm, p.x) + bit_hi(bm, p.x) + bit_lo(bm, p.y) + bit_hi(bm, p.y) + bit_lo(bm, p.z) + bit_hi(bm, p.z) +
           bit_lo(bm, p.w) + bit_hi(bm, p.w);
}

__device__ __forceinline__ uint32_t delta_unit_hits(const uint32_t *bm, uint4 p) {
    uint32_t id[14];
    id[0] = p.x & 0xffffu;
    id[1] = id[0] + (p.x >> 24);
    id[2] = id[1] + (p.y & 0xffu);
    id[3] = id[2] + ((p.y >> 8) & 0xffu);
    id[4] = id[3] + ((p.y >> 16) & 0xffu);
    id[5] = id[4] + (p.y >> 24);
    id[6] = id[5] + (p.z & 0xffu);
    id[7] = id[6] + ((p.z >> 8) & 0xffu);
    id[8] = id[7] + ((p.z >> 16) & 0xffu);
    id[9] = id[8] + (p.z >> 24);
    id[10] = id[9] + (p.w & 0xffu);
    id[11] = id[10] + ((p.w >> 8) & 0xffu);
    id[12] = id[11] + ((p.w >> 16) & 0xffu);
    id[13] = id[12] + (p.w >> 24);
    uint32_t w[14];
#pragma unroll
    for (int k = 0; k < 14; ++k) w[k] = bm[id[k] >> 5];
    uint32_t hits = 0;
#pragma unroll
    for (int k = 0; k < 14; ++k) hits |= __builtin_amdgcn_ubfe(w[k], id[k], 1u) << k;
    const uint32_t n = (p.x >> 16) & 0xffu;
    return uint32_t(__popc(hits & ((1u << n) - 1u)));
}

__device__ __forceinline__ uint32_t gap12_unit_hits(const uint32_t *bm, uint4 p) {
    uint32_t id[10];
    id[0] = p.x & 0xffffu;
    id[1] = id[0] + (p.x >> 20);
    id[2] = id[1] + (p.y & 0xfffu);
    id[3] = id[2] + __builtin_amdgcn_ubfe(p.y, 12u, 12u);
    id[4] = id[3] + (__builtin_amdgcn_alignbit(p.z, p.y, 24u) & 0xfffu);
    id[5] = id[4] + __builtin_amdgcn_ubfe(p.z, 4u, 12u);
    id[6] = id[5] + __builtin_amdgcn_ubfe(p.z, 16u, 12u);
    id[7] = id[6] + (__builtin_amdgcn_alignbit(p.w, p.z, 28u) & 0xfffu);
    id[8] = id[7] + __builtin_amdgcn_ubfe(p.w, 8u, 12u);
    id[9] = id[8] + (p.w >> 20);
    uint32_t w[10];
#pragma unroll
    for (int k = 0; k < 10; ++k) w[k] = bm[id[k] >> 5];
    uint32_t hits = 0;
#pragma unroll
    for (int k = 0; k < 10; ++k) hits |= __builtin_amdgcn_ubfe(w[k], id[k], 1u) << k;
    const uint32_t n = (p.x >> 16) & 0xfu;
    return uint32_t(__popc(hits & ((1u << n) - 1u)));
}

__device__ __forceinline__ uint32_t hash_slot(int32_t w, int shift) { return (uint32_t(w) * 0x9E3779B1u) >> shift; }

__device__ __forceinline__ void set_insert(int32_t *tbl, uint32_t mask, int shift, int32_t w) {
    uint32_t h = hash_slot(w, shift);
    while (atomicCAS(&tbl[h], -1, w) != -1) h = (h + 1) & mask;
}
__device__ __forceinline__ uint32_t set_contains(const int32_t *tbl, uint32_t mask, int shift, int32_t w) {
    uint32_t h = hash_slot(w, shift), found = 0u;
    bool go;
    do {
        const int32_t x = tbl[h];
        found |= x == w ? 1u : 0u;
        go = x != w && x != -1;
        h = (h + 1) & mask;
    } while (go);
    return found;
}
static constexpr int kFilterWords = 1024;
__device__ __forceinline__ uint32_t flt_word(const uint32_t *flt, uint32_t id) { return flt[(id >> 5) & uint32_t(kFilterWords - 1)] >> (id & 31u); }
__device__ __forceinline__ uint32_t pick(uint32_t c, uint32_t x, uint32_t y) { return x ^ ((x ^ y) & (0u - c)); }
__device__ __forceinline__ uint32_t probe_set_bits(const int32_t *tbl, uint32_t mask, int shift, uint32_t m, const uint32_t (&id)[6]) {
    uint32_t c = 0;
    while (m) {
        const uint32_t k = uint32_t(__ffs(int(m)) - 1);
        m &= m - 1u;
        const uint32_t b0 = k & 1u, b1 = (k >> 1) & 1u, b2 = k >> 2;
        const uint32_t w = pick(b2, pick(b1, pick(b0, id[0], id[1]), pick(b0, id[2], id[3])), pick(b0, id[4], id[5]));
        c += set_contains(tbl, mask, shift, int32_t(w));
    }
    return c;
}
__device__ __forceinline__ uint32_t tail_unit_hits(const uint32_t *flt, const int32_t *tbl, uint32_t mask, int shift, uint4 p) {
    const uint32_t w0 = flt_word(flt, p.x), w1 = flt_word(flt, p.y), w2 = flt_word(flt, p.z), w3 = flt_word(flt, p.w);
    if (((w0 | w1 | w2 | w3) & 1u) == 0) return 0u;
    const uint32_t id[6] = {p.x, p.y, p.z, p.w, 0u, 0u};
    return probe_set_bits(tbl, mask, shift, (w0 & 1u) | ((w1 & 1u) << 1) | ((w2 & 1u) << 2) | ((w3 & 1u) << 3), id);
}
__device__ __forceinline__ uint32_t tail_delta_unit_hits(const uint32_t *flt, const int32_t *tbl, uint32_t mask, int shift, uint4 p) {
    const uint32_t id0 = p.x, id1 = id0 + (p.y >> 16), id2 = id1 + (p.z & 0xffffu), id3 = id2 + (p.z >> 16), id4 = id3 + (p.w & 0xffffu),
                   id5 = id4 + (p.w >> 16);
    const uint32_t w0 = flt_word(flt, id0), w1 = flt_word(flt, id1), w2 = flt_word(flt, id2), w3 = flt_word(flt, id3), w4 = flt_word(flt, id4),
                   w5 = flt_word(flt, id5);
    if (((w0 | w1 | w2 | w3 | w4 | w5) & 1u) == 0) return 0u;
    const uint32_t n = p.y & 0xffu;
    const uint32_t m = ((w0 & 1u) | ((w1 & 1u) << 1) | ((w2 & 1u) << 2) | ((w3 & 1u) << 3) | ((w4 & 1u) << 4) | ((w5 & 1u) << 5)) & ((1u << n) - 1u);
    const uint32_t id[6] = {id0, id1, id2, id3, id4, id5};
    return probe_set_bits(tbl, mask, shift, m, id);
}
static constexpr int kBlockLog = 10;
template <int FORM>
__device__ __forceinline__ uint32_t hub_unit_hits(const uint32_t *bm, uint4 p, int j) {
    if (FORM == kFormBitset) {
        const uint4 q = *reinterpret_cast<const uint4 *>(bm + 4 * j);
        return uint32_t(__popc(p.x & q.x) + __popc(p.y & q.y) + __popc(p.z & q.z) + __popc(p.w & q.w));
    }
    if (FORM == kFormDelta) return delta_unit_hits(bm, p);
    if (FORM == kFormGap12) return gap12_unit_hits(bm, p);
    return hub_hits8(bm, u4u{p.x, p.y, p.z, p.w});
}
template <int FORM>
__device__ __forceinline__ uint32_t tail_unit_hits_f(const uint32_t *flt, const int32_t *tbl, uint32_t mask, int shift, uint4 p) {
    return FORM == kFormDelta ? tail_delta_unit_hits(flt, tbl, mask, shift, p) : tail_unit_hits(flt, tbl, mask, shift, p);
}
#ifndef GMSX_TC_TAIL_DEPTH
#define GMSX_TC_TAIL_DEPTH 1
#endif
#ifndef GMSX_TC_HUB_GROUP
#define GMSX_TC_HUB_GROUP 16
#endif
#ifndef GMSX_TC_TAIL_GROUP
#define GMSX_TC_TAIL_GROUP 16
#endif
#ifndef GMSX_TC_HUB_DEPTH
#define GMSX_TC_HUB_DEPTH 1
#endif
struct StagedTasks {
    uint32_t lo[kTaskChunk];
    uint32_t hi[kTaskChunk / 2 + 2];
};
template <int W, int D, bool TAIL>
struct StepStream {
    static constexpr int G = 256 / W;
    const uint32_t *slo;
    const uint16_t *shi;
    const uint4 *pool4;
    int hi, sub;
    int e, units, last, lim, j, form;
    const uint4 *row;
    int pending;
    static constexpr int S = D == 1 ? 2 : D;
    uint4 p[S];
    int pj[S];
    __device__ __forceinline__ void open_row() {
        int ee = e;
        asm volatile("" : "+v"(ee));
        const uint32_t l = e < hi ? slo[ee] : 0u, h = e < hi ? uint32_t(shi[ee]) : 0u;
        row = pool4 + __builtin_amdgcn_alignbit(h, l, 16);
        units = int(l & (TAIL ? kTaskTailUnitsMax : kTaskHubUnitsMax));
        form = TAIL ? int((l >> 15) & 1u) << 25 : int((l >> 14) & 3u) << 24;
        last = max(units - 1, 0);
        lim = units + sub;
        j = sub;
    }
    __device__ __forceinline__ void issue(int k) {
        p[k] = row[uint32_t(min(j, last))];
        pj[k] = j < units ? (j | form) : -1;
        pending += e < hi ? 1 : 0;
        j += W;
        if (j >= lim) {
            e += G;
            open_row();
        }
    }
    __device__ __forceinline__ void start(const StagedTasks &sd, int odd, const uint32_t *__restrict__ pool, int lo, int hi_, int tid) {
        slo = sd.lo;
        shi = reinterpret_cast<const uint16_t *>(sd.hi) + odd;
        pool4 = reinterpret_cast<const uint4 *>(pool);
        hi = hi_;
        sub = tid % W;
        e = lo + tid / W;
        pending = 0;
        open_row();
#pragma unroll
        for (int k = 0; k < D; ++k) issue(k);
    }
    template <class Hit>
    __device__ __forceinline__ uint32_t run(Hit hit) {
        uint32_t cnt = 0;
        if constexpr (D == 1) {
            auto step = [&](int cur, int nxt) {
                pending -= 1;
                issue(nxt);
#ifdef GMSX_TC_NO_PROBE
                if (pj[cur] >= 0) cnt += p[cur].x & 1u;
#else
                if (pj[cur] >= 0) cnt += hit(p[cur], pj[cur] & 0xffffff, pj[cur] >> 24);
#endif
            };
            while (pending > 0) {
                step(0, 1);
                if (!(pending > 0)) break;
                step(1, 0);
            }
            return cnt;
        }
        while (pending > 0) {
#pragma unroll
            for (int k = 0; k < D; ++k) {
                const uint4 pc = p[k];
                const int jc = pj[k];
                pending -= 1;
                issue(k);
#ifdef GMSX_TC_NO_PROBE
                if (jc >= 0) cnt += pc.x & 1u;
#else
                if (jc >= 0) cnt += hit(pc, jc & 0xffffff, jc >> 24);
#endif
            }
        }
        return cnt;
    }
};
__device__ __forceinline__ uint32_t hub_hits_by_form(const uint32_t *bm, uint4 p, int j, int f) {
    if (f == kFormList) return hub_unit_hits<kFormList>(bm, p, j);
    if (f == kFormDelta) return hub_unit_hits<kFormDelta>(bm, p, j);
    if (f == kFormBitset) return hub_unit_hits<kFormBitset>(bm, p, j);
    return hub_unit_hits<kFormGap12>(bm, p, j);
}
__device__ __forceinline__ uint32_t tail_hits_by_form(const uint32_t *flt, const int32_t *tbl, uint32_t mask, int shift, uint4 p, int f) {
    return f == kFormDelta ? tail_delta_unit_hits(flt, tbl, mask, shift, p) : tail_unit_hits(flt, tbl, mask, shift, p);
}
__device__ __forceinline__ void stage_item(const TaskList ent, int ne, int tid, StagedTasks &sd) {
    for (int i = tid; i < ne; i += 256) {
        sd.lo[i] = ent.lo[i];
        reinterpret_cast<uint16_t *>(sd.hi)[i] = ent.hi[i];
    }
    __syncthreads();
}
__device__ __forceinline__ void block_add(unsigned long long cnt, unsigned long long *red, int lane, int wave, int tid, unsigned long long *__restrict__ acc) {
    for (int s = 32; s > 0; s >>= 1) cnt += __shfl_down(cnt, s);
    if (lane == 0) red[wave] = cnt;
    __syncthreads();
    if (tid == 0) {
        const unsigned long long t = red[0] + red[1] + red[2] + red[3];
        if (t) atomicAdd(&acc[(blockIdx.x & (kAccSlots - 1)) * kAccStride], t);
    }
}


__global__ __launch_bounds__(256) __attribute__((amdgpu_waves_per_eu(8, 8))) void k_tc_block(const int64_t *__restrict__ hoff, const uint16_t *__restrict__ hadj,
                                                  const uint32_t *__restrict__ spool, const TaskList htask,
                                                  const gmsx_tc_item *__restrict__ items, unsigned long long *__restrict__ acc) {
    __shared__ __attribute__((aligned(16))) uint32_t bm[kBitmapWords + 128];
    __shared__ StagedTasks sdesc;
    __shared__ unsigned long long red[4];
    const int tid = threadIdx.x, lane = tid & 63, wave = tid >> 6;
    const gmsx_tc_item &it = items[blockIdx.x];
    const int32_t u = it.pivot;
    const int64_t hb = hoff[u];
    const int hl = int(hoff[u + 1] - hb);
    const int ne = int(it.bc >> 40);
    for (int i = tid; i < (kBitmapWords + 128) / 4; i += 256) reinterpret_cast<uint4 *>(bm)[i] = make_uint4(0u, 0u, 0u, 0u);
    stage_item(htask.at(int64_t(it.bc & 0xffffffffffull)), ne, tid, sdesc);
    for (int i = tid; i < hl; i += 256) {
        const uint32_t id = hadj[hb + i];
        if (id != 0xFFFFu) atomicOr(&bm[id >> 5], 1u << (id & 31u));
    }
    __syncthreads();
    uint32_t cnt = 0;
#ifndef GMSX_TC_STAGING_ONLY
    StepStream<GMSX_TC_HUB_GROUP, GMSX_TC_HUB_DEPTH, false> st;
    st.start(sdesc, 0, spool, 0, ne, tid);
    cnt += st.run([](uint4 p, int j, int f) { return hub_hits_by_form(bm, p, j, f); });
#endif
    block_add(cnt, red, lane, wave, tid, acc);
}

__global__ __launch_bounds__(256) __attribute__((amdgpu_waves_per_eu(8, 8))) void k_tc_tail(const int64_t *__restrict__ toff, const int32_t *__restrict__ tadj,
                                                 const uint32_t *__restrict__ tpool, const TaskList ttask,
                                                 const gmsx_tc_item *__restrict__ items, unsigned long long *__restrict__ acc) {
    __shared__ __attribute__((aligned(16))) int32_t tbl[1 << kBlockLog];
    __shared__ __attribute__((aligned(16))) uint32_t flt[kFilterWords];
    __shared__ StagedTasks sdesc;
    __shared__ unsigned long long red[4];
    constexpr int TILE = (1 << kBlockLog) / 2;
    const int tid = threadIdx.x, lane = tid & 63, wave = tid >> 6;
    const gmsx_tc_item &it = items[blockIdx.x];
    const int32_t u = it.pivot;
    const int64_t tb = toff[u];
    const int tl = int(toff[u + 1] - tb);
    const int ne = int(it.bc >> 40);
    stage_item(ttask.at(int64_t(it.bc & 0xffffffffffull)), ne, tid, sdesc);
    int log = 6;
    while ((1 << log) < 2 * min(tl, TILE)) ++log;
    const int size = 1 << log, shift = 32 - log;
    const uint32_t mask = uint32_t(size - 1);
    uint32_t cnt = 0;
    for (int t0 = 0; t0 < tl; t0 += TILE) {
        const int tn = min(TILE, tl - t0);
        __syncthreads();
        for (int i = tid; i < size; i += 256) tbl[i] = -1;
        reinterpret_cast<uint4 *>(flt)[tid] = make_uint4(0u, 0u, 0u, 0u);
        __syncthreads();
        for (int i = tid; i < tn; i += 256) {
            const int32_t t = tadj[tb + t0 + i];
            set_insert(tbl, mask, shift, t);
            atomicOr(&flt[(uint32_t(t) >> 5) & uint32_t(kFilterWords - 1)], 1u << (uint32_t(t) & 31u));
        }
        __syncthreads();
#ifndef GMSX_TC_STAGING_ONLY
        StepStream<GMSX_TC_TAIL_GROUP, GMSX_TC_TAIL_DEPTH, true> st;
        st.start(sdesc, 0, tpool, 0, ne, tid);
        cnt += st.run([mask, shift](uint4 p, int, int f) { return tail_hits_by_form(flt, tbl, mask, shift, p, f); });
#endif
    }
    block_add(cnt, red, lane, wave, tid, acc);
}

static constexpr int kGrab = 8;
static constexpr int kIdStage = 256;
static constexpr int kQueueStride = 16;

__device__ __forceinline__ uint32_t lds_addr(const void *p) { return uint32_t(uintptr_t((const __attribute__((address_space(3))) void *)p)); }
__device__ __forceinline__ void glds_dword(const uint32_t *src, uint32_t lds_byte_addr) {
    unsigned keep;
    const unsigned dst = uni32(lds_byte_addr);
    asm volatile("s_mov_b32 %0, m0\n\ts_mov_b32 m0, %2\n\ts_nop 0\n\tglobal_load_lds_dword %1, off\n\ts_mov_b32 m0, %0" : "=&s"(keep) : "v"(src), "s"(dst) : "memory");
}
__device__ __forceinline__ void stage_dwords(const uint32_t *__restrict__ src, uint32_t lds_byte_addr, int ndw, int lane, int wave) {
    asm volatile("" : "+v"(lane));
    for (int base = wave * 64; base < ndw; base += 256)
        if (base + lane < ndw) glds_dword(src + base + lane, lds_byte_addr + 4u * uint32_t(base));
}
struct ItemLds {
    uint32_t bm[kBitmapWords + 128];
    StagedTasks sdesc[2];
    uint32_t idst[2][kIdStage];
    uint32_t rec[3][16];
    unsigned long long red[4];
    int chunk[2];
};
template <bool TAIL>
__device__ __forceinline__ void item_loop(ItemLds &L, const uint16_t *__restrict__ hadj, const int32_t *__restrict__ tadj, const uint32_t *__restrict__ pool,
                                          const TaskList task, const gmsx_tc_item *__restrict__ items, int n_items,
                                          unsigned int *__restrict__ qhead, unsigned long long &total) {
    constexpr int TILE = (1 << kBlockLog) / 2;
    const int tid = threadIdx.x, lane = tid & 63, wave = tid >> 6;
    uint32_t *bm = L.bm;
    const uint32_t a_slo = lds_addr(&L.sdesc[0].lo[0]), a_shi = lds_addr(&L.sdesc[0].hi[0]), a_idst = lds_addr(&L.idst[0][0]), a_rec = lds_addr(&L.rec[0][0]);
    __syncthreads();
    if (tid == 0) {
        const unsigned a = atomicAdd(qhead, unsigned(kGrab));
        const unsigned b = a < unsigned(n_items) ? atomicAdd(qhead, unsigned(kGrab)) : a;
        L.chunk[0] = a < unsigned(n_items) ? int(a) : -1;
        L.chunk[1] = b < unsigned(n_items) ? int(b) : -1;
    }
    if (!TAIL)
        for (int i = tid; i < (kBitmapWords + 128) / 4; i += 256) reinterpret_cast<uint4 *>(bm)[i] = make_uint4(0u, 0u, 0u, 0u);
    __syncthreads();
    int ci = uni32(L.chunk[0]);
    int ce = ci < 0 ? 0 : min(ci + kGrab, n_items);
    auto advance = [&]() -> bool {
        if (ci < 0) return false;
        if (++ci < ce) return false;
        ci = uni32(L.chunk[1]);
        ce = ci < 0 ? 0 : min(ci + kGrab, n_items);
        return true;
    };
    auto fetch_rec = [&](int slot, int lane, int wave) {
        if (wave == 0 && lane < 16) glds_dword(reinterpret_cast<const uint32_t *>(items + ci) + lane, a_rec + 64u * uint32_t(slot));
    };
    auto stage = [&](const uint32_t *rec, int b, int lane, int wave) {
        const uint32_t bc_lo = uni32(rec[0]), bc_hi = uni32(rec[1]), c_lo = uni32(rec[2]), c_hi = uni32(rec[3]);
        const uint64_t first = (uint64_t(bc_hi & 0xffu) << 32) | bc_lo, cb = (uint64_t(c_hi & 0xffu) << 32) | c_lo;
        const int ne = int(bc_hi >> 8), cn = int(c_hi >> 8);
        stage_dwords(task.lo + first, a_slo + uint32_t(b) * uint32_t(sizeof(StagedTasks)), ne, lane, wave);
        stage_dwords(reinterpret_cast<const uint32_t *>(task.hi + (first & ~uint64_t(1))), a_shi + uint32_t(b) * uint32_t(sizeof(StagedTasks)), (int(first & 1u) + ne + 1) / 2, lane, wave);
        if (TAIL) stage_dwords(reinterpret_cast<const uint32_t *>(tadj + cb), a_idst + uint32_t(b) * uint32_t(sizeof(L.idst[0])), min(cn, kIdStage), lane, wave);
        else stage_dwords(reinterpret_cast<const uint32_t *>(hadj + cb), a_idst + uint32_t(b) * uint32_t(sizeof(L.idst[0])), min(cn, 2 * kIdStage) / 2, lane, wave);
    };
    auto flip2 = [&](uint32_t w) {
        const uint32_t lo = w & 0xffffu, hi = w >> 16;
        if (lo != 0xFFFFu) atomicXor(&bm[lo >> 5], 1u << (lo & 31u));
        if (hi != 0xFFFFu) atomicXor(&bm[hi >> 5], 1u << (hi & 31u));
    };
    bool vA = ci >= 0, vB = false;
    if (vA) fetch_rec(0, lane, wave);
    if (advance()) {
        __syncthreads();
        if (tid == 0 && ci >= 0) {
            const unsigned x = atomicAdd(qhead, unsigned(kGrab));
            L.chunk[1] = x < unsigned(n_items) ? int(x) : -1;
        }
    }
    vB = ci >= 0;
    if (vB) fetch_rec(1, lane, wave);
    asm volatile("s_waitcnt vmcnt(0)" ::: "memory");
    __syncthreads();
    if (vA) stage(L.rec[0], 0, lane, wave);
    int ra = 0, buf = 0;
    bool bm_valid = true, bm_small = true;
    int bm_pivot = -1, bm_n = 0;
    const int tid0 = tid;
    while (vA) {
        int tid = tid0;
        asm volatile("" : "+v"(tid));
        const int lane = tid & 63, wave = tid >> 6;
        const int rb = ra == 2 ? 0 : ra + 1, rc = rb == 2 ? 0 : rb + 1;
        asm volatile("s_waitcnt vmcnt(0)" ::: "memory");
        __syncthreads();
        const bool crossed = advance();
        const bool vC = ci >= 0;
        if (vC) fetch_rec(rc, lane, wave);
        unsigned pend = 0;
        const bool fetch = tid == 0 && crossed && vC;
        if (fetch) pend = atomicAdd(qhead, unsigned(kGrab));
        const uint32_t *recA = L.rec[ra];
        const uint32_t c_lo = uni32(recA[2]), c_hi = uni32(recA[3]);
        const int64_t cb = int64_t((uint64_t(c_hi & 0xffu) << 32) | c_lo);
        const int cn = int(c_hi >> 8);
        const StagedTasks &sd = L.sdesc[buf];
        const int neA = int(uni32(recA[1]) >> 8), oddA = int(uni32(recA[0]) & 1u);
        uint32_t c = 0;
        StepStream<TAIL ? GMSX_TC_TAIL_GROUP : GMSX_TC_HUB_GROUP, TAIL ? GMSX_TC_TAIL_DEPTH : GMSX_TC_HUB_DEPTH, TAIL> st;
#ifndef GMSX_TC_STAGING_ONLY
        if (!TAIL) st.start(sd, oddA, pool, 0, neA, tid);
#endif
        if (!TAIL) {
            const int pivotA = int(uni32(recA[4]));
            if (!(bm_valid && bm_pivot == pivotA)) {
                if (bm_valid && bm_small) {
                    for (int i = tid; i < bm_n / 2; i += 256) flip2(L.idst[buf ^ 1][i]);
                } else {
                    for (int i = tid; i < (kBitmapWords + 128) / 4; i += 256) reinterpret_cast<uint4 *>(bm)[i] = make_uint4(0u, 0u, 0u, 0u);
                    __syncthreads();
                }
                const int ns = min(cn, 2 * kIdStage);
                for (int i = tid; i < ns / 2; i += 256) flip2(L.idst[buf][i]);
                for (int i = 2 * kIdStage + 2 * tid; i < cn; i += 512) flip2(*reinterpret_cast<const uint32_t *>(hadj + cb + i));
                bm_valid = true;
                bm_pivot = pivotA;
                bm_n = ns;
                bm_small = cn <= 2 * kIdStage;
            }
            __syncthreads();
            if (vB) stage(L.rec[rb], buf ^ 1, lane, wave);
            if (fetch) L.chunk[1] = pend < unsigned(n_items) ? int(pend) : -1;
#ifndef GMSX_TC_STAGING_ONLY
            c += st.run([bm](uint4 p, int j, int f) { return hub_hits_by_form(bm, p, j, f); });
#endif
        } else {
            int32_t *tbl = reinterpret_cast<int32_t *>(bm);
            uint32_t *flt = bm + (1 << kBlockLog);
            int log = 6;
            while ((1 << log) < 2 * min(cn, TILE)) ++log;
            const int size = 1 << log, shift = 32 - log;
            const uint32_t mask = uint32_t(size - 1);
            bool staged = false;
            for (int t0 = 0; t0 < cn; t0 += TILE) {
                const int tn = min(TILE, cn - t0);
                if (t0 > 0) __syncthreads();
                for (int i = tid; i < size; i += 256) tbl[i] = -1;
                reinterpret_cast<uint4 *>(flt)[tid] = make_uint4(0u, 0u, 0u, 0u);
                __syncthreads();
                int tin = tid0;
                asm volatile("" : "+v"(tin));
                for (int i = tin; i < tn; i += 256) {
                    const int32_t t = t0 + i < kIdStage ? int32_t(L.idst[buf][t0 + i]) : tadj[cb + t0 + i];
                    set_insert(tbl, mask, shift, t);
                    atomicOr(&flt[(uint32_t(t) >> 5) & uint32_t(kFilterWords - 1)], 1u << (uint32_t(t) & 31u));
                }
                __syncthreads();
                if (!staged && vB) stage(L.rec[rb], buf ^ 1, lane, wave);
                if (!staged && fetch) L.chunk[1] = pend < unsigned(n_items) ? int(pend) : -1;
                staged = true;
#ifndef GMSX_TC_STAGING_ONLY
                const int nl = int(uni32(recA[8]) & 0xffffu);
                if (nl > 0) {
                    st.start(sd, oddA, pool, 0, nl, tid);
                    c += st.run([=](uint4 p, int, int) { return tail_unit_hits(flt, tbl, mask, shift, p); });
                }
                if (neA > nl) {
                    st.start(sd, oddA, pool, nl, neA, tid);
                    c += st.run([=](uint4 p, int, int) { return tail_delta_unit_hits(flt, tbl, mask, shift, p); });
                }
#endif
            }
            if (!staged) {
                __syncthreads();
                if (vB) stage(L.rec[rb], buf ^ 1, lane, wave);
                if (fetch) L.chunk[1] = pend < unsigned(n_items) ? int(pend) : -1;
            }
        }
        total += c;
        ra = rb;
        vA = vB;
        vB = vC;
        buf ^= 1;
    }
}

#ifndef GMSX_TC_HUB_MIN_WAVES
#define GMSX_TC_HUB_MIN_WAVES 8
#endif
#ifndef GMSX_TC_TAIL_MIN_WAVES
#define GMSX_TC_TAIL_MIN_WAVES 8
#endif
template <bool TAIL>
__global__ __launch_bounds__(256) __attribute__((amdgpu_waves_per_eu(TAIL ? GMSX_TC_TAIL_MIN_WAVES : GMSX_TC_HUB_MIN_WAVES, 8))) void k_tc_items(
    const uint16_t *__restrict__ hadj, const int32_t *__restrict__ tadj, const uint32_t *__restrict__ pool, const TaskList task,
    const gmsx_tc_item *__restrict__ items, int n_items, unsigned int *__restrict__ qhead, unsigned long long *__restrict__ acc) {
    __shared__ __attribute__((aligned(16))) ItemLds L;
    const int tid = threadIdx.x;
    unsigned long long total = 0;
    item_loop<TAIL>(L, hadj, tadj, pool, task, items, n_items, qhead, total);
    block_add(total, L.red, tid & 63, tid >> 6, tid, acc);
}

template <int K>
__device__ __forceinline__ uint32_t ror_in_row(uint32_t x) {
    if constexpr (K == 0) return x;
    else return uint32_t(__builtin_amdgcn_mov_dpp(int(x), 0x120 + K, 0xf, 0xf, false));
}
__device__ __forceinline__ bool row_has(uint32_t a, uint32_t x) {
    bool m = false;
#define GMSX_ROT(K) m |= a == ror_in_row<K>(x);
    GMSX_ROT(0) GMSX_ROT(1) GMSX_ROT(2) GMSX_ROT(3) GMSX_ROT(4) GMSX_ROT(5) GMSX_ROT(6) GMSX_ROT(7)
    GMSX_ROT(8) GMSX_ROT(9) GMSX_ROT(10) GMSX_ROT(11) GMSX_ROT(12) GMSX_ROT(13) GMSX_ROT(14) GMSX_ROT(15)
#undef GMSX_ROT
    return m;
}
struct LightRows {
    uint32_t ah[4], at[4], bh[4], bt[4];
};
struct LightRec {
    uint4 r0, r1;
};
__global__ __launch_bounds__(256) void k_tc_light(const uint16_t *__restrict__ hadj, const int32_t *__restrict__ tadj, const uint4 *__restrict__ ledge, int nparts,
                                                  int part, int64_t count, unsigned long long *__restrict__ acc) {
    __shared__ unsigned long long red[4];
    const int tid = threadIdx.x, lane = tid & 63, wave = tid >> 6, sub = lane & 15;
    const int64_t ngroups = int64_t(gridDim.x) * 16, g0 = int64_t(blockIdx.x) * 16 + (tid >> 4);
    const int64_t trips = (count + ngroups - 1) / ngroups;
    auto load_rec = [&](int64_t t) -> LightRec {
        const int64_t k = g0 + t * ngroups;
        const int64_t kk = k < count ? k : 0;
        const int64_t e = nparts <= 1 ? kk : kk * nparts + ((kk & 1) ? nparts - 1 - part : part);
        LightRec r;
        r.r0 = ledge[2 * e];
        r.r1 = ledge[2 * e + 1];
        if (k >= count) {
            r.r0.y &= 0xffu;
            r.r0.w &= 0xffu;
            r.r1.y &= 0xffu;
            r.r1.w &= 0xffu;
        }
        return r;
    };
    auto wave_max = [](int x) {
        return max(max(__builtin_amdgcn_readlane(x, 0), __builtin_amdgcn_readlane(x, 16)), max(__builtin_amdgcn_readlane(x, 32), __builtin_amdgcn_readlane(x, 48)));
    };
    auto load_rows = [&](const LightRec &r) -> LightRows {
        const int64_t hu = int64_t((uint64_t(r.r0.y & 0xffu) << 32) | r.r0.x), tu = int64_t((uint64_t(r.r0.w & 0xffu) << 32) | r.r0.z);
        const int64_t hv = int64_t((uint64_t(r.r1.y & 0xffu) << 32) | r.r1.x), tv = int64_t((uint64_t(r.r1.w & 0xffu) << 32) | r.r1.z);
        const int hlu = int(r.r0.y >> 8), tlu = int(r.r0.w >> 8), hlv = int(r.r1.y >> 8), tlv = int(r.r1.w >> 8);
        const int more = wave_max((max(max(hlu, hlv), max(tlu, tlv)) + 15) >> 4);
        LightRows w;
        w.ah[0] = hadj[hlu ? hu + min(sub, hlu - 1) : 0];
        w.bh[0] = hadj[hlv ? hv + min(sub, hlv - 1) : 0];
        w.at[0] = uint32_t(tadj[tlu ? tu + min(sub, tlu - 1) : 0]);
        w.bt[0] = uint32_t(tadj[tlv ? tv + min(sub, tlv - 1) : 0]);
#pragma unroll
        for (int k = 1; k < 4; ++k) {
            w.ah[k] = w.bh[k] = w.at[k] = w.bt[k] = 0;
            if (k < more) {
                const int i = sub + 16 * k;
                w.ah[k] = hadj[hlu ? hu + min(i, hlu - 1) : 0];
                w.bh[k] = hadj[hlv ? hv + min(i, hlv - 1) : 0];
                w.at[k] = uint32_t(tadj[tlu ? tu + min(i, tlu - 1) : 0]);
                w.bt[k] = uint32_t(tadj[tlv ? tv + min(i, tlv - 1) : 0]);
            }
        }
        return w;
    };
    unsigned long long total = 0;
    if (trips > 0) {
        LightRec rec = load_rec(0);
        LightRows rows = load_rows(rec);
        LightRec rec_n = load_rec(1);
        for (int64_t t = 0; t < trips; ++t) {
            const LightRows rows_n = load_rows(rec_n);
            const LightRec rec_nn = load_rec(t + 2);
            const int hlu = int(rec.r0.y >> 8), tlu = int(rec.r0.w >> 8), hlv = int(rec.r1.y >> 8), tlv = int(rec.r1.w >> 8);
            const int nah = wave_max((hlu + 15) >> 4), nbh = wave_max((hlv + 15) >> 4), nat = wave_max((tlu + 15) >> 4), nbt = wave_max((tlv + 15) >> 4);
            uint32_t c = 0;
#pragma unroll
            for (int ka = 0; ka < 4; ++ka) {
                if (ka >= nah) break;
                const int ia = sub + 16 * ka;
                const uint32_t a = (ia < hlu && rows.ah[ka] != 0xFFFFu) ? rows.ah[ka] : 0xFFFFFFFFu;
                bool m = false;
#pragma unroll
                for (int kb = 0; kb < 4; ++kb) {
                    if (kb >= nbh) break;
                    const int ib = sub + 16 * kb;
                    const uint32_t x = (ib < hlv && rows.bh[kb] != 0xFFFFu) ? rows.bh[kb] : 0xFFFFFFFEu;
                    m |= row_has(a, x);
                }
                c += m ? 1u : 0u;
            }
#pragma unroll
            for (int ka = 0; ka < 4; ++ka) {
                if (ka >= nat) break;
                const int ia = sub + 16 * ka;
                const uint32_t a = ia < tlu ? rows.at[ka] : 0xFFFFFFFFu;
                bool m = false;
#pragma unroll
                for (int kb = 0; kb < 4; ++kb) {
                    if (kb >= nbt) break;
                    const int ib = sub + 16 * kb;
                    const uint32_t x = ib < tlv ? rows.bt[kb] : 0xFFFFFFFEu;
                    m |= row_has(a, x);
                }
                c += m ? 1u : 0u;
            }
            total += c;
            rec = rec_n;
            rows = rows_n;
            rec_n = rec_nn;
        }
    }
    block_add(total, red, lane, wave, tid, acc);
}

__global__ __launch_bounds__(256) void k_tc_stats(const int64_t *__restrict__ hoff, const uint16_t *__restrict__ hadj,
                                                  const int64_t *__restrict__ toff, const int32_t *__restrict__ tadj,
                                                  const int32_t *__restrict__ dplus, const int32_t *__restrict__ order,
                                                  const int32_t *__restrict__ tunits, int32_t inline_limit, int inline_first, int64_t end, int nparts, int part,
                                                  unsigned long long *__restrict__ out) {
    const int lane = threadIdx.x & 63;
    const int64_t wave0 = (int64_t(blockIdx.x) * blockDim.x + threadIdx.x) >> 6;
    const int64_t nwaves = (int64_t(gridDim.x) * blockDim.x) >> 6;
    unsigned long long units = 0, probes = 0, bytes = 0;
    for (int64_t pos = wave0; pos < end; pos += nwaves) {
        if (nparts > 1 && shard_of(pos, nparts) != part) continue;
        const int32_t u = order[pos];
        const int du = dplus[u];
        if (du >= kHeavy) {
            if (lane == 0) units += (unsigned long long)tunits[pos];
            const int hl = min(int(hoff[u + 1] - hoff[u]), inline_first), tl = min(int(toff[u + 1] - toff[u]), inline_first - hl);
            int32_t v = -1;
            if (lane < hl) {
                const uint32_t x = hadj[hoff[u] + lane];
                if (x != 0xFFFFu) v = int32_t(x);
            } else if (lane - hl < tl) v = tadj[toff[u] + lane - hl];
            if (v >= 0 && lane > 0 && (v < inline_limit || dplus[v] >= kHeavy)) ++units;
            continue;
        }
        const int hl = int(hoff[u + 1] - hoff[u]);
        if (lane == 0) units += (unsigned long long)du;
        if (du < 2) continue;
        for (int64_t j = toff[u] + lane; j < toff[u + 1]; j += 64) {
            const int32_t v = tadj[j];
            if (v < inline_limit || dplus[v] >= kHeavy) continue;
            const unsigned long long hv = (unsigned long long)(hoff[v + 1] - hoff[v]), tv = (unsigned long long)(toff[v + 1] - toff[v]);
            bytes += 32ull + 2ull * hl + 4ull * (unsigned long long)(j - toff[u]) + 2ull * hv + 4ull * tv;
            probes += hv + tv;
        }
    }
    for (int s = 32; s > 0; s >>= 1) {
        units += __shfl_down(units, s);
        probes += __shfl_down(probes, s);
        bytes += __shfl_down(bytes, s);
    }
    if (lane == 0) {
        if (units) atomicAdd(&out[0], units);
        if (probes) atomicAdd(&out[1], probes);
        if (bytes) atomicAdd(&out[2], bytes);
    }
}
__global__ __launch_bounds__(256) void k_tc_item_stats(const int64_t *__restrict__ coff, int bytes_per_id, int tail, const TaskList task,
                                                       const gmsx_tc_item *__restrict__ items, int64_t n_items, int nparts, int part,
                                                       unsigned long long *__restrict__ out) {
    const int lane = threadIdx.x & 63;
    const int64_t wave0 = (int64_t(blockIdx.x) * blockDim.x + threadIdx.x) >> 6;
    const int64_t nwaves = (int64_t(gridDim.x) * blockDim.x) >> 6;
    unsigned long long probes = 0, bytes = 0;
    auto slots = [tail](unsigned long long d) -> unsigned long long {
        const unsigned long long n = d & 0x3fffffull, f = (d >> 22) & 3ull;
        return n * (tail ? (f == kFormDelta ? 6ull : 4ull) : (f == kFormList ? 8ull : f == kFormDelta ? 14ull : f == kFormGap12 ? 10ull : 4ull));
    };
    for (int64_t q = wave0; q < n_items; q += nwaves) {
        const gmsx_tc_item &it = items[q];
        if (nparts > 1 && shard_of(it.pos, nparts) != part) continue;
        const int ne = int(it.bc >> 40);
        const int64_t b = int64_t(it.bc & 0xffffffffffull);
        if (lane == 0) bytes += (unsigned long long)bytes_per_id * (unsigned long long)(coff[it.pivot + 1] - coff[it.pivot]);
        for (int i = lane; i < ne; i += 64) {
            const unsigned long long d = task.get(b + i);
            bytes += 6ull + 16ull * (d & 0x3fffffull);
            probes += slots(d);
        }
    }
    for (int s = 32; s > 0; s >>= 1) {
        probes += __shfl_down(probes, s);
        bytes += __shfl_down(bytes, s);
    }
    if (lane == 0) {
        if (probes) atomicAdd(&out[1], probes);
        if (bytes) atomicAdd(&out[2], bytes);
    }
}

__global__ __launch_bounds__(256) void k_tc_breakdown(const int64_t *__restrict__ hoff, const int64_t *__restrict__ toff, const int32_t *__restrict__ tadj,
                                                      const int32_t *__restrict__ dplus, const int32_t *__restrict__ order,
                                                      const TaskList htask, const gmsx_tc_item *__restrict__ hitem, int64_t hitems,
                                                      const TaskList ttask, const gmsx_tc_item *__restrict__ titem, int64_t titems,
                                                      int32_t inline_limit, int64_t first_light, int64_t end_light,
                                                      unsigned long long *__restrict__ out) {
    const int lane = threadIdx.x & 63;
    const int64_t wave0 = (int64_t(blockIdx.x) * blockDim.x + threadIdx.x) >> 6;
    const int64_t nwaves = (int64_t(gridDim.x) * blockDim.x) >> 6;
    unsigned long long c[15] = {0, 0, 0, 0, 0, 0, 0, 0, 0, 0, 0, 0, 0, 0, 0};
    for (int64_t q = wave0; q < hitems + titems; q += nwaves) {
        const bool tail = q >= hitems;
        const gmsx_tc_item &it = tail ? titem[q - hitems] : hitem[q];
        const TaskList task = tail ? ttask : htask;
        const int ne = int(it.bc >> 40);
        const int64_t b0 = int64_t(it.bc & 0xffffffffffull);
        if (lane == 0) {
            c[6] += tail ? 4ull * (unsigned long long)(toff[it.pivot + 1] - toff[it.pivot]) : 2ull * (unsigned long long)(hoff[it.pivot + 1] - hoff[it.pivot]);
            c[11] += (unsigned long long)ne;
            c[13] += 1;
        }
        for (int i = lane; i < ne; i += 64) {
            const unsigned long long d = task.get(b0 + i);
            const unsigned long long db = 16ull * (d & 0x3fffffull);
            const int fd = int((d >> 22) & 3);
            if (tail) c[fd == kFormDelta ? 4 : 3] += db;
            else c[fd == kFormList ? 0 : fd == kFormBitset ? 1 : 2] += db;
            c[5] += 6;
        }
    }
    for (int64_t pos = first_light + wave0; pos < end_light; pos += nwaves) {
        const int32_t u = order[pos];
        const int64_t tb0 = toff[u], te = toff[u + 1];
        const unsigned long long hl = (unsigned long long)(hoff[u + 1] - hoff[u]);
        for (int64_t j = tb0 + lane; j < te; j += 64) {
            const int32_t v = tadj[j];
            if (v < inline_limit || dplus[v] >= kHeavy) continue;
            c[8] += 2ull * (unsigned long long)(hoff[v + 1] - hoff[v]);
            c[9] += 4ull * (unsigned long long)(toff[v + 1] - toff[v]);
            c[10] += 32ull + 2ull * hl + 4ull * (unsigned long long)(j - tb0);
            c[14] += 1;
        }
    }
    for (int k = 0; k < 15; ++k) {
        unsigned long long x = c[k];
        for (int s = 32; s > 0; s >>= 1) x += __shfl_down(x, s);
        if (lane == 0 && x) atomicAdd(&out[k], x);
    }
}

__device__ __forceinline__ int hist_bin(unsigned long long units) {
    if (units <= 16) return int(units) - 1;
    int b = 16;
    for (unsigned long long lim = 32; units > lim && b < 23; lim <<= 1) ++b;
    return b;
}
__global__ __launch_bounds__(256) void k_tc_comember_keys(const TaskList htask, const gmsx_tc_item *__restrict__ hitem, int64_t hitems, int batch,
                                                         unsigned long long *__restrict__ keys, uint32_t *__restrict__ vals, unsigned long long *__restrict__ sums) {
    unsigned long long ents = 0, units = 0;
    for (int64_t i = blockIdx.x; i < hitems; i += gridDim.x) {
        const gmsx_tc_item it = hitem[i];
        const unsigned long long first = it.bc & 0xffffffffffull;
        const int n = int(it.bc >> 40);
        const unsigned long long b = (unsigned long long)(it.pos / batch) << 40;
        for (int e = threadIdx.x; e < n; e += 256) {
            const unsigned long long d = htask.get(int64_t(first + e));
            keys[first + e] = b | (d >> 24);
            vals[first + e] = uint32_t(d & 0x3fffffull);
            ++ents;
            units += d & 0x3fffffull;
        }
    }
    for (int sft = 32; sft > 0; sft >>= 1) {
        ents += __shfl_xor(ents, sft);
        units += __shfl_xor(units, sft);
    }
    if ((threadIdx.x & 63) == 0) {
        atomicAdd(&sums[0], ents);
        atomicAdd(&sums[1], units);
    }
}
__global__ __launch_bounds__(256) void k_tc_sum_u32(const uint32_t *__restrict__ v, unsigned long long n, unsigned long long *__restrict__ out) {
    unsigned long long t = 0;
    for (unsigned long long i = (unsigned long long)blockIdx.x * 256 + threadIdx.x; i < n; i += (unsigned long long)gridDim.x * 256) t += v[i];
    for (int sft = 32; sft > 0; sft >>= 1) t += __shfl_xor(t, sft);
    if ((threadIdx.x & 63) == 0) atomicAdd(out, t);
}
__global__ __launch_bounds__(256) void k_tc_row_hist(const int64_t *__restrict__ hoff, const uint16_t *__restrict__ hadj,
                                                     const int64_t *__restrict__ toff, const int32_t *__restrict__ tadj,
                                                     const int32_t *__restrict__ dplus, const int32_t *__restrict__ order,
                                                     const unsigned long long *__restrict__ srow, const unsigned long long *__restrict__ trow,
                                                     const TaskList htask, const gmsx_tc_item *__restrict__ hitem, int64_t hitems,
                                                     const TaskList ttask, const gmsx_tc_item *__restrict__ titem, int64_t titems,
                                                     int64_t end, unsigned long long *__restrict__ out) {
    __shared__ unsigned long long h[256];
    for (int i = threadIdx.x; i < 256; i += 256) h[i] = 0;
    __syncthreads();
    const int lane = threadIdx.x & 63;
    const int64_t wave0 = (int64_t(blockIdx.x) * blockDim.x + threadIdx.x) >> 6;
    const int64_t nwaves = (int64_t(gridDim.x) * blockDim.x) >> 6;
    auto add = [&](int cls, unsigned long long units) {
        if (units == 0) return;
        const int b = (cls * 24 + hist_bin(units)) * 2;
        atomicAdd(&h[b], 1ull);
        atomicAdd(&h[b + 1], units);
    };
    for (int64_t q = wave0; q < hitems + titems; q += nwaves) {
        const bool tail = q >= hitems;
        const gmsx_tc_item &it = tail ? titem[q - hitems] : hitem[q];
        const TaskList task = tail ? ttask : htask;
        const int ne = int(it.bc >> 40);
        const int64_t b0 = int64_t(it.bc & 0xffffffffffull);
        if (lane == 0) {
            atomicAdd(&h[240], (unsigned long long)ne);
            atomicAdd(&h[242], 1ull);
            atomicAdd(&h[243], tail ? 4ull * (unsigned long long)(toff[it.pivot + 1] - toff[it.pivot]) : 2ull * (unsigned long long)(hoff[it.pivot + 1] - hoff[it.pivot]));
        }
        for (int i = lane; i < ne; i += 64) {
            const unsigned long long d = task.get(b0 + i);
            if (tail) add(((d >> 22) & 3) == kFormDelta ? 4 : 3, d & 0x3fffffull);
            else add(min(int((d >> 22) & 3), 2), d & 0x3fffffull);
        }
    }
    for (int64_t pos = wave0; pos < end; pos += nwaves) {
        if (!srow || !trow) break;
        const int32_t u = order[pos];
        const int du = dplus[u];
        if (du < 2) continue;
        const int64_t hb = hoff[u], tb = toff[u];
        const int hl = int(hoff[u + 1] - hb), tl = int(toff[u + 1] - tb);
        const unsigned long long su = (srow[u] & 0x3fffffull) + (trow[u] & 0x3fffffull);
        unsigned long long cur = 0, best = 0, cut = 0;
        for (int i = lane; i < hl + tl; i += 64) {
            int32_t v;
            if (i < hl) {
                const uint32_t x = hadj[hb + i];
                if (x == 0xFFFFu) continue;
                v = int32_t(x);
            } else v = tadj[tb + i - hl];
            const unsigned long long sv = (srow[v] & 0x3fffffull) + (trow[v] & 0x3fffffull);
            cur += sv;
            best += min(su, sv);
            cut += min(sv, dplus[v] >= kHeavy ? (su * (unsigned long long)i + du - 1) / (unsigned long long)du : ~0ull);
        }
        atomicAdd(&h[du >= kHeavy ? 248 : 250], cur);
        atomicAdd(&h[du >= kHeavy ? 249 : 251], best);
        if (du >= kHeavy) atomicAdd(&h[252], cut);
    }
    __syncthreads();
    for (int i = threadIdx.x; i < 256; i += 256)
        if (h[i]) atomicAdd(&out[i], h[i]);
}

static int tc_one(const gmsx_graph *g, int part, int nparts, uint64_t *partial, gmsx_stats *st);

static int tc_oriented(const gmsx_graph *g, int part, int nparts, uint64_t *partial, gmsx_stats *st) {
    if (int rc = ensure_tc(g)) return rc;
    if (g->tc_passes == 1) return tc_one(g, part, nparts, partial, st);
    if (nparts > 1) {
        auto restore = [&](int rc) {
            gmsx_graph *m = const_cast<gmsx_graph *>(g);
            if (m->tc_ready && m->shard_part == 0 && m->shard_nparts == m->tc_passes) return rc;
            (void)ensure_tc_shard(g, 0, g->tc_passes);
            return rc;
        };
        int J = nparts >= g->tc_passes ? 1 : (g->tc_passes + nparts - 1) / nparts;
        if (J > 1 && (J & 1)) ++J;
        for (;; J *= 2) {
            uint64_t total = 0;
            gmsx_stats sum{};
            int rc = GMSX_OK;
            for (int a = 0; a < J && rc == GMSX_OK; ++a) {
                const int sub = a * nparts + ((a & 1) ? nparts - 1 - part : part);
                rc = ensure_tc_shard(g, sub, nparts * J);
                if (rc) break;
                uint64_t pp = 0;
                gmsx_stats sp{};
                rc = tc_one(g, sub, nparts * J, &pp, st ? &sp : nullptr);
                total += pp;
                sum.kernel_ms += sp.kernel_ms;
                sum.setup_ms += sp.setup_ms;
                sum.units += sp.units;
                sum.probes += sp.probes;
                sum.stream_bytes += sp.stream_bytes;
                sum.launches += sp.launches;
            }
            if (rc == GMSX_ERR_DEVICE_MEM && nparts * J <= (1 << 20)) continue;
            if (rc) return restore(rc);
            *partial = total;
            if (st) *st = sum;
            return GMSX_OK;
        }
    }
    uint64_t total = 0;
    gmsx_stats sum{};
    for (int p = 0; p < g->tc_passes; ++p) {
        if (int rc = ensure_tc_shard(g, p, g->tc_passes)) return rc;
        uint64_t pp = 0;
        gmsx_stats sp{};
        if (int rc = tc_one(g, p, g->tc_passes, &pp, st ? &sp : nullptr)) return rc;
        total += pp;
        sum.kernel_ms += sp.kernel_ms;
        sum.setup_ms += sp.setup_ms;
        sum.units += sp.units;
        sum.probes += sp.probes;
        sum.stream_bytes += sp.stream_bytes;
        sum.launches += sp.launches;
    }
    *partial = total;
    if (st) {
        sum.alg_elements = g->alg_elements;
        *st = sum;
    }
    return GMSX_OK;
}

static int tc_one(const gmsx_graph *g, int part, int nparts, uint64_t *partial, gmsx_stats *st) {
    const bool use_idx = nparts > 1 && g->shard_nparts == 1;
    if (use_idx)
        if (int rc = tc_shard_items(g, part, nparts)) return rc;
    const gmsx_tc_item *hitem = use_idx ? g->shard_hitem : g->hitem, *titem = use_idx ? g->shard_titem : g->titem;
    int64_t n_hitems = use_idx ? g->shard_hitems : g->hitems, n_titems = use_idx ? g->shard_titems : g->titems;
#ifdef GMSX_DEV_HOOKS
    const char *only = std::getenv("GMSX_TC_ONLY");
    if (only) {
        if (std::strcmp(only, "hub") != 0) n_hitems = 0;
        if (std::strcmp(only, "tail") != 0) n_titems = 0;
    }
#else
    const char *only = nullptr;
#endif
    Ctx &c = ctx();
    hipStream_t s = c.stream;
    unsigned long long *acc = g->acc;
    static_assert(kAccSlots * kAccStride + 16 <= kAccWords, "gmsx_graph::acc too small");
    unsigned int *qhead = reinterpret_cast<unsigned int *>(acc + kAccSlots * kAccStride + 4);
    static_assert((kQueueStride + 1) * sizeof(unsigned int) <= 12 * sizeof(unsigned long long), "queue heads past gmsx_graph::acc");
    GMSX_HIP(hipEventRecord(c.ev[0], s));
    GMSX_HIP(hipMemsetAsync(acc, 0, sizeof(unsigned long long) * kAccWords, s));
    GMSX_HIP(hipEventRecord(c.ev[1], s));

    int launches = 0;
    const int cus = c.compute_units > 0 ? c.compute_units : 256;
    const int64_t cap_blocks = int64_t(cus) * 16;
    const bool run_light = !only || std::strcmp(only, "light") == 0;
    const bool strided = nparts > 1 && g->shard_nparts == 1;
    const int64_t cnt_light = [&]() -> int64_t {
        if (!run_light) return 0;
        if (!strided) return g->n_ledge;
        const int64_t full = g->n_ledge / nparts, rem = g->n_ledge % nparts;
        return full + (((full & 1) ? nparts - 1 - part : part) < rem ? 1 : 0);
    }();
    const int overlap = [] { const char *e = opt("TC_OVERLAP"); return e ? std::atoi(e) : 0; }();
    const int persist = [] { const char *e = opt("TC_PERSIST"); return e ? std::atoi(e) : 1; }();
    const bool sides = overlap && c.side[0] && c.side[1];
    struct Join {
        Ctx &c;
        hipStream_t s;
        bool armed[2] = {false, false};
        ~Join() {
            for (int i = 0; i < 2; ++i)
                if (armed[i] && hipEventRecord(c.ev_join[i], c.side[i]) == hipSuccess) (void)hipStreamWaitEvent(s, c.ev_join[i], 0);
        }
    } join{c, s};
    const bool side_light = sides && cnt_light > 0 && n_hitems + n_titems > 0;
    const bool side_tail = sides && !persist && n_hitems > 0 && n_titems > 0;
    if (side_light || side_tail) GMSX_HIP(hipEventRecord(c.ev_fork, s));
    if (side_tail) {
        GMSX_HIP(hipStreamWaitEvent(c.side[0], c.ev_fork, 0));
        join.armed[0] = true;
    }
    if (side_light) {
        GMSX_HIP(hipStreamWaitEvent(c.side[1], c.ev_fork, 0));
        join.armed[1] = true;
    }
    if (persist) {
        const int wgs_env = [] { const char *e = opt("TC_ITEM_WGS"); return e ? std::atoi(e) : 0; }();
        auto grid = [&](int64_t n, int wgs) {
            return unsigned(std::max<int64_t>(1, std::min<int64_t>((n + kGrab - 1) / kGrab, int64_t(cus) * (wgs_env > 0 ? wgs_env : wgs))));
        };
        if (n_hitems > 0) {
            hipLaunchKernelGGL(k_tc_items<false>, dim3(grid(n_hitems, GMSX_TC_HUB_MIN_WAVES)), dim3(256), 0, s, g->hadj, g->tadj, g->spool, g->htask, hitem, int(n_hitems), qhead, acc);
            ++launches;
        }
        if (n_titems > 0) {
            hipLaunchKernelGGL(k_tc_items<true>, dim3(grid(n_titems, GMSX_TC_TAIL_MIN_WAVES)), dim3(256), 0, s, g->hadj, g->tadj, g->tpool, g->ttask, titem, int(n_titems),
                               qhead + kQueueStride, acc);
            ++launches;
        }
    } else {
        if (n_hitems > 0) {
            hipLaunchKernelGGL(k_tc_block, dim3(unsigned(n_hitems)), dim3(256), 0, s, g->hoff, g->hadj, g->spool, g->htask, hitem, acc);
            ++launches;
        }
        if (n_titems > 0) {
            hipLaunchKernelGGL(k_tc_tail, dim3(unsigned(n_titems)), dim3(256), 0, side_tail ? c.side[0] : s, g->toff, g->tadj, g->tpool, g->ttask, titem, acc);
            ++launches;
        }
    }
    if (cnt_light > 0) {
        const int64_t blocks = std::min<int64_t>((cnt_light + 15) / 16, int64_t(cus) * 8);
        hipLaunchKernelGGL(k_tc_light, dim3(unsigned(blocks)), dim3(256), 0, side_light ? c.side[1] : s, g->hadj, g->tadj, g->ledge, strided ? nparts : 1,
                           strided ? part : 0, cnt_light, acc);
        ++launches;
    }
    for (int i = 0; i < 2; ++i)
        if (join.armed[i]) {
            join.armed[i] = false;
            GMSX_HIP(hipEventRecord(c.ev_join[i], c.side[i]));
            GMSX_HIP(hipStreamWaitEvent(s, c.ev_join[i], 0));
        }
    GMSX_HIP(hipEventRecord(c.ev[2], s));
    GMSX_HIP(hipGetLastError());

    const bool need_stats = st && !(g->stats_part == part && g->stats_nparts == nparts);
    if (need_stats) {
        if (g->n > 0) {
            const int64_t blocks = std::min<int64_t>((g->n + 3) / 4, cap_blocks);
            hipLaunchKernelGGL(k_tc_stats, dim3(unsigned(blocks)), dim3(256), 0, s, g->hoff, g->hadj, g->toff, g->tadj, g->dplus, g->order,
                               g->tunits, g->inline_limit, g->inline_first, g->n, nparts, part, acc + kAccSlots * kAccStride);
        }
        if (g->hitems > 0)
            hipLaunchKernelGGL(k_tc_item_stats, dim3(unsigned(std::min<int64_t>((g->hitems + 3) / 4, cap_blocks))), dim3(256), 0, s, g->hoff, 2, 0, g->htask, g->hitem,
                               g->hitems, nparts, part, acc + kAccSlots * kAccStride);
        if (g->titems > 0)
            hipLaunchKernelGGL(k_tc_item_stats, dim3(unsigned(std::min<int64_t>((g->titems + 3) / 4, cap_blocks))), dim3(256), 0, s, g->toff, 4, 1, g->ttask, g->titem,
                               g->titems, nparts, part, acc + kAccSlots * kAccStride);
    }
    unsigned long long host[kAccSlots * kAccStride + 3];
    GMSX_HIP(hipMemcpyAsync(host, acc, sizeof(host), hipMemcpyDeviceToHost, s));
    GMSX_HIP(hipStreamSynchronize(s));
    unsigned long long total = 0;
    for (int i = 0; i < kAccSlots; ++i) total += host[i * kAccStride];
    *partial = total;
    if (st) {
        float ms_setup = 0.f, ms_kernel = 0.f;
        GMSX_HIP(hipEventElapsedTime(&ms_setup, c.ev[0], c.ev[1]));
        GMSX_HIP(hipEventElapsedTime(&ms_kernel, c.ev[1], c.ev[2]));
        st->kernel_ms = ms_kernel;
        st->setup_ms = ms_setup;
        if (need_stats) {
            g->stats_part = part;
            g->stats_nparts = nparts;
            g->stats_units = host[kAccSlots * kAccStride];
            g->stats_probes = host[kAccSlots * kAccStride + 1];
            g->stats_bytes = host[kAccSlots * kAccStride + 2];
        }
        st->units = g->stats_units;
        st->probes = g->stats_probes;
        st->alg_elements = nparts == 1 ? g->alg_elements : 0;
        st->launches = launches;
        st->reserved = 0;
        st->stream_bytes = g->stats_bytes;
    }
    return GMSX_OK;
}

}

using namespace gmsx;

extern "C" {

int gmsx_tc_divisor(int algo) { return algo == GMSX_TC_FULL ? 3 : 1; }

int gmsx_tc_stream_breakdown(const gmsx_graph *g, uint64_t *out21) {
    return gmsx::guard([&]() -> int {
        if (!g || !out21) return GMSX_ERR_INVALID;
        if (int rc = ensure_init()) return rc;
        if (int rc = ensure_tc(g)) return rc;
        hipStream_t s = ctx().stream;
        std::memset(out21, 0, 21 * sizeof(uint64_t));
        if (g->n == 0) return GMSX_OK;
        int64_t n_block = 0, n_work = 0;
        if (int rc = count_dplus_ge(g, kHeavy, &n_block)) return rc;
        if (int rc = count_dplus_ge(g, 2, &n_work)) return rc;
        unsigned long long *acc = nullptr;
        GMSX_HIP(hipMalloc(reinterpret_cast<void **>(&acc), 21 * 8));
        struct Guard { void *p; ~Guard() { (void)hipFree(p); } } g1{acc};
        GMSX_HIP(hipMemsetAsync(acc, 0, 21 * 8, s));
        const int cus = ctx().compute_units > 0 ? ctx().compute_units : 256;
        hipLaunchKernelGGL(k_tc_breakdown, dim3(unsigned(cus * 16)), dim3(256), 0, s, g->hoff, g->toff, g->tadj, g->dplus, g->order, g->htask,
                           g->hitem, g->hitems, g->ttask, g->titem, g->titems, g->inline_limit, n_block, n_work, acc);
        GMSX_HIP(hipMemcpyAsync(out21, acc, 21 * 8, hipMemcpyDeviceToHost, s));
        GMSX_HIP(hipStreamSynchronize(s));
        GMSX_HIP(hipGetLastError());
        out21[7] = uint64_t(g->inline_units) * 16ull;
        out21[12] = uint64_t(g->inline_hentries + g->inline_tentries);
        return GMSX_OK;
    });
}

int gmsx_tc_row_histogram(const gmsx_graph *g, uint64_t *out256) {
    return gmsx::guard([&]() -> int {
        uint64_t *out248 = out256;
        if (!g || !out248) return GMSX_ERR_INVALID;
        if (int rc = ensure_init()) return rc;
        if (int rc = ensure_tc(g)) return rc;
        hipStream_t s = ctx().stream;
        std::memset(out248, 0, 256 * sizeof(uint64_t));
        if (g->n == 0) return GMSX_OK;
        unsigned long long *acc = nullptr;
        GMSX_HIP(hipMalloc(reinterpret_cast<void **>(&acc), 256 * 8));
        struct Guard { void *p; ~Guard() { (void)hipFree(p); } } g1{acc};
        GMSX_HIP(hipMemsetAsync(acc, 0, 256 * 8, s));
        const int cus = ctx().compute_units > 0 ? ctx().compute_units : 256;
        hipLaunchKernelGGL(k_tc_row_hist, dim3(unsigned(cus * 8)), dim3(256), 0, s, g->hoff, g->hadj, g->toff, g->tadj, g->dplus, g->order, g->srow, g->trow,
                           g->htask, g->hitem, g->hitems, g->ttask, g->titem, g->titems, g->n, acc);
        GMSX_HIP(hipGetLastError());
        GMSX_HIP(hipMemcpyAsync(out248, acc, 256 * 8, hipMemcpyDeviceToHost, s));
        GMSX_HIP(hipStreamSynchronize(s));
        GMSX_HIP(hipGetLastError());
        out248[241] = uint64_t(g->inline_hentries + g->inline_tentries);
        return GMSX_OK;
    });
}

int gmsx_tc_comembership(const gmsx_graph *g, int batch, uint64_t *out8) {
    return gmsx::guard([&]() -> int {
        if (!g || !out8 || batch < 1) return GMSX_ERR_INVALID;
        if (int rc = ensure_init()) return rc;
        if (int rc = ensure_tc(g)) return rc;
        hipStream_t s = ctx().stream;
        std::memset(out8, 0, 8 * sizeof(uint64_t));
        const int64_t ne = g->htask_entries;
        if (g->n == 0 || ne == 0 || g->hitems == 0) return GMSX_OK;
        struct Guard { void *p = nullptr; ~Guard() { (void)hipFree(p); } } gk0, gk1, gv0, gv1, gu, ga, gc, gt, gsum;
        unsigned long long *k0 = nullptr, *k1 = nullptr, *uk = nullptr, *cnt = nullptr, *sum = nullptr;
        uint32_t *v0 = nullptr, *v1 = nullptr, *agg = nullptr;
        GMSX_HIP(hipMalloc(reinterpret_cast<void **>(&k0), size_t(ne) * 8)); gk0.p = k0;
        GMSX_HIP(hipMalloc(reinterpret_cast<void **>(&k1), size_t(ne) * 8)); gk1.p = k1;
        GMSX_HIP(hipMalloc(reinterpret_cast<void **>(&v0), size_t(ne) * 4)); gv0.p = v0;
        GMSX_HIP(hipMalloc(reinterpret_cast<void **>(&v1), size_t(ne) * 4)); gv1.p = v1;
        GMSX_HIP(hipMalloc(reinterpret_cast<void **>(&sum), 4 * 8)); gsum.p = sum;
        GMSX_HIP(hipMemsetAsync(k0, 0xff, size_t(ne) * 8, s));
        GMSX_HIP(hipMemsetAsync(v0, 0, size_t(ne) * 4, s));
        GMSX_HIP(hipMemsetAsync(sum, 0, 4 * 8, s));
        hipLaunchKernelGGL(k_tc_comember_keys, dim3(unsigned(std::min<int64_t>(g->hitems, 1 << 20))), dim3(256), 0, s, g->htask, g->hitem, g->hitems, batch, k0, v0, sum);
        size_t tb = 0;
        GMSX_HIP(rocprim::radix_sort_pairs(nullptr, tb, k0, k1, v0, v1, size_t(ne), 0, 64, s));
        void *tmp = nullptr;
        GMSX_HIP(hipMalloc(&tmp, tb ? tb : 8)); gt.p = tmp;
        GMSX_HIP(rocprim::radix_sort_pairs(tmp, tb, k0, k1, v0, v1, size_t(ne), 0, 64, s));
        uk = k0;
        agg = v0;
        GMSX_HIP(hipMalloc(reinterpret_cast<void **>(&cnt), 8)); gc.p = cnt;
        size_t rb = 0;
        GMSX_HIP(rocprim::reduce_by_key(nullptr, rb, k1, v1, size_t(ne), uk, agg, cnt, rocprim::maximum<uint32_t>(), rocprim::equal_to<unsigned long long>(), s));
        void *tmp2 = nullptr;
// ... 45 lines not shown
```

### gms_amd/csrc/host/loader.cpp

```cpp
#include "gmsx_internal.hpp"

#include <fcntl.h>
#include <sys/mman.h>
#include <sys/stat.h>
#include <unistd.h>

#include <algorithm>
#ifdef _OPENMP
#include <parallel/algorithm>
#endif
#include <atomic>
#include <cerrno>
#include <cmath>
#include <cstdio>
#include <cstdlib>
#include <cstring>
#include <ctime>
#include <fstream>
#include <limits>
#include <memory>
#include <new>
#include <random>
#include <sstream>
#include <string>
// ... 499 lines not shown
                if (int rc = push_edge(us, vs, u, v - 1)) return rc;
        }
        ++u;
    }
    return finish_el(us, vs, el);
}
static int read_mtx(const std::string &path, EdgeList &el) {
    std::ifstream in(path);
    if (!in.is_open()) return GMSX_ERR_IO;
    std::string start, object, format, field, symmetry, line;
    if (!(in >> start >> object >> format >> field >> symmetry)) return GMSX_ERR_FORMAT;
    if (start != "%%MatrixMarket" || object != "matrix" || format != "coordinate" || field == "complex") return GMSX_ERR_FORMAT;
    const bool weights = field == "real" || field == "double" || field == "integer";
    if (!weights && field != "pattern") return GMSX_ERR_FORMAT;
    if (symmetry != "symmetric" && symmetry != "general" && symmetry != "skew-symmetric") return GMSX_ERR_FORMAT;
    std::getline(in, line);
    long long rows = -1, cols = -1, nz = -1;
    while (std::getline(in, line)) {
        if (!line.empty() && line[0] == '%') continue;
        std::istringstream hs(line);
        if (!(hs >> rows >> cols >> nz)) return GMSX_ERR_FORMAT;
        break;
    }
    if (rows < 0 || rows != cols) return GMSX_ERR_FORMAT;
    std::vector<int32_t> us, vs;
    while (std::getline(in, line)) {
        std::istringstream ls(line);
        long long a, b;
        if (!(ls >> a >> b)) continue;
        if (int rc = push_edge(us, vs, a - 1, b - 1)) return rc;
        if (symmetry == "symmetric")
            if (int rc = push_edge(us, vs, b - 1, a - 1)) return rc;
    }
    return finish_el(us, vs, el);
}

static int validate_csr_arrays(const int64_t *off, const int32_t *ng, int64_t n, int64_t nnz);
static int read_sg(const std::string &path, Csr &g) {
    std::FILE *f = std::fopen(path.c_str(), "rb");
    if (!f) return GMSX_ERR_IO;
    struct Closer { std::FILE *f; ~Closer() { std::fclose(f); } } closer{f};
    unsigned char directed = 0;
    int64_t nnz = 0, n = 0;
    if (std::fread(&directed, 1, 1, f) != 1 || std::fread(&nnz, 8, 1, f) != 1 || std::fread(&n, 8, 1, f) != 1)
        return GMSX_ERR_FORMAT;
    if (n < 0 || nnz < 0 || n > std::numeric_limits<int32_t>::max()) return GMSX_ERR_FORMAT;
    if (int rc = alloc_csr(g, n, nnz)) return rc;
    if (std::fread(g.off.get(), 8, size_t(n + 1), f) != size_t(n + 1)) return GMSX_ERR_FORMAT;
    if (nnz && std::fread(g.neigh.get(), 4, size_t(nnz), f) != size_t(nnz)) return GMSX_ERR_FORMAT;
    if (int rc = validate_csr_arrays(g.off.get(), g.neigh.get(), n, nnz)) return rc;
    g.directed = directed != 0;
    return GMSX_OK;
}


static constexpr char kSgxMagic[8] = {'G', 'M', 'S', 'X', 'C', 'S', 'R', '1'};
static constexpr int64_t kSgxAlign = 64;
static int64_t sgx_neigh_offset(int64_t n) { return (kSgxAlign + (n + 1) * 8 + kSgxAlign - 1) / kSgxAlign * kSgxAlign; }

void ArrayFree::unmap(void *base, size_t bytes) { (void)munmap(base, bytes); }

static int write_sgx(const Csr &g, const char *path) {
    std::FILE *f = std::fopen(path, "wb");
    if (!f) return GMSX_ERR_IO;
    int64_t head[8] = {0, g.directed ? 1 : 0, g.n, g.nnz, 0, 0, 0, 0};
    std::memcpy(head, kSgxMagic, 8);
    const int64_t pad = sgx_neigh_offset(g.n) - (kSgxAlign + (g.n + 1) * 8);
    const char zeros[64] = {0};
    bool ok = std::fwrite(head, 8, 8, f) == 8 && std::fwrite(g.off.get(), 8, size_t(g.n + 1), f) == size_t(g.n + 1) &&
              (pad == 0 || std::fwrite(zeros, 1, size_t(pad), f) == size_t(pad)) &&
              (g.nnz == 0 || std::fwrite(g.neigh.get(), 4, size_t(g.nnz), f) == size_t(g.nnz));
    ok = (std::fclose(f) == 0) && ok;
    return ok ? GMSX_OK : GMSX_ERR_IO;
}

static int validate_csr_arrays(const int64_t *off, const int32_t *ng, int64_t n, int64_t nnz) {
    if (off[0] != 0 || off[n] != nnz) return GMSX_ERR_FORMAT;
    int bad = 0;
#pragma omp parallel for reduction(| : bad) schedule(static)
    for (int64_t u = 0; u < n; ++u) bad |= int(off[u + 1] < off[u]);
    if (bad) return GMSX_ERR_FORMAT;
#pragma omp parallel for reduction(| : bad) schedule(static)
    for (int64_t j = 0; j < nnz; ++j) bad |= int(ng[j] < 0 || int64_t(ng[j]) >= n);
    return bad ? GMSX_ERR_FORMAT : GMSX_OK;
}

static int read_sgx(const std::string &path, Csr &g) {
    const int fd = open(path.c_str(), O_RDONLY | O_CLOEXEC);
    if (fd < 0) return GMSX_ERR_IO;
    struct Closer { int fd; ~Closer() { close(fd); } } closer{fd};
    struct stat st;
    if (fstat(fd, &st) != 0) return GMSX_ERR_IO;
    int64_t head[8];
    if (pread(fd, head, sizeof(head), 0) != ssize_t(sizeof(head)) || std::memcmp(head, kSgxMagic, 8) != 0) return GMSX_ERR_FORMAT;
    const int64_t n = head[2], nnz = head[3];
    if (n < 0 || nnz < 0 || n > std::numeric_limits<int32_t>::max() || (head[1] != 0 && head[1] != 1)) return GMSX_ERR_FORMAT;
    const int64_t noff = sgx_neigh_offset(n);
    if (nnz > (std::numeric_limits<int64_t>::max() - noff) / 4 || int64_t(st.st_size) < noff + nnz * 4) return GMSX_ERR_FORMAT;
    const int64_t page = int64_t(sysconf(_SC_PAGESIZE));
    auto map_part = [&](int64_t at, int64_t bytes, void **base, size_t *len) -> void * {
        const int64_t lo = at / page * page;
        *len = size_t(at - lo + std::max<int64_t>(bytes, 1));
        *base = mmap(nullptr, *len, PROT_READ | PROT_WRITE, MAP_PRIVATE, fd, off_t(lo));
        if (*base == MAP_FAILED) return nullptr;
        (void)madvise(*base, *len, MADV_WILLNEED);
        return static_cast<char *>(*base) + (at - lo);
    };
    void *b0 = nullptr, *b1 = nullptr;
    size_t l0 = 0, l1 = 0;
    void *p_off = map_part(kSgxAlign, (n + 1) * 8, &b0, &l0);
    if (!p_off) return GMSX_ERR_NOMEM;
    g.off = std::unique_ptr<int64_t[], ArrayFree>(static_cast<int64_t *>(p_off), ArrayFree{b0, l0});
    void *p_ng = map_part(noff, nnz * 4, &b1, &l1);
    if (!p_ng) return GMSX_ERR_NOMEM;
    g.neigh = std::unique_ptr<int32_t[], ArrayFree>(static_cast<int32_t *>(p_ng), ArrayFree{b1, l1});
    g.n = n;
    g.nnz = nnz;
    g.directed = head[1] != 0;
    g.mapped = true;
    return validate_csr_arrays(g.off.get(), g.neigh.get(), n, nnz);
}

}

namespace gmsx {
int host_threads() {
#ifdef _OPENMP
    return omp_get_max_threads();
#else
    return 1;
#endif
}
void parallel_memcpy(void *dst, const void *src, size_t bytes) {
#ifdef _OPENMP
#pragma omp parallel
    {
        const size_t nt = size_t(omp_get_num_threads()), t = size_t(omp_get_thread_num());
        const size_t per = ((bytes + nt - 1) / nt + 4095) & ~size_t(4095), lo = std::min(bytes, per * t), hi = std::min(bytes, lo + per);
        if (hi > lo) std::memcpy(static_cast<char *>(dst) + lo, static_cast<const char *>(src) + lo, hi - lo);
    }
#else
    std::memcpy(dst, src, bytes);
#endif
}
namespace {
struct Option {
    const char *name;
    char value[32];
    bool set;
};
Option g_options[] = {
    {"TIMING", "", false}, {"MEM_TRACE", "", false}, {"BK_VERBOSE", "", false},
    {"INLINE_LIMIT", "", false}, {"TC_INLINE_FIRST", "", false}, {"TC_DELTA", "", false}, {"TC_DELTA_PCT", "", false}, {"TC_GAP12", "", false},
    {"TC_HYBRID", "", false}, {"TC_TAIL_DELTA", "", false}, {"TC_TWO_SIDED", "", false}, {"TC_HOT_WINDOWS", "", false}, {"TC_HOT_KB", "", false},
    {"TC_HOT_MIN", "", false}, {"TC_TEST_MAX_UNITS", "", false}, {"TC_KEEP_ROWS", "", false}, {"TC_MEM_LIMIT_MB", "", false}, {"TC_OVERLAP", "", false},
    {"TC_PERSIST", "", false}, {"TC_ITEM_WGS", "", false}, {"SORT_CHUNK", "", false}, {"UPLOAD_STAGED", "", false}, {"INIT_LAZY", "", false},
    {"KC_SLAB_MB", "", false}, {"KC_MAXD", "", false}, {"KC_STREAMS", "", false}, {"KC_PIPE_ALL", "", false}, {"KC_STREAM_BUILD", "", false},
    {"KC_REVERSE", "", false}, {"KC_REV_MIN", "", false}, {"KC_REV_FACTOR", "", false}, {"KC_REV_TAIL", "", false}, {"KC_REV_TAIL_MIN", "", false}, {"KC_REV_GW", "", false}, {"KC_TRI", "", false}, {"KC_MFMA", "", false}, {"KC_POOL_MB", "", false},
    {"BK_MAXC", "", false}, {"BK_ARENA_MB", "", false}, {"BK_GROUPS", "", false}, {"BK_SMALL_P", "", false}, {"BK_SMALL_P_GROUPS", "", false},
    {"BK_BUDGET", "", false}, {"BK_BUDGET0", "", false}, {"BK_RESUME_GRAB", "", false}, {"BK_SPLIT_BUILD", "", false}, {"BK_TINY_ROOTS", "", false},
    {"BK_TINY_BESIDE", "", false},
    {"BK_LIST_ARENA_MB", "", false},
};
Option *find_option(const char *name) {
    if (!name) return nullptr;
    for (Option &o : g_options)
        if (std::strcmp(o.name, name) == 0) return &o;
    return nullptr;
}
}

const char *opt(const char *name) {
    const Option *o = find_option(name);
    return o && o->set ? o->value : nullptr;
}

}

using namespace gmsx;

extern "C" {

int gmsx_csr_generate(int generator, int scale, int degree, int relabel, int threads, gmsx_csr **out) {
    return gmsx::guard([&]() -> int {
        if (!out || scale < 1 || degree < 1 || relabel < 0 || relabel > 2) return GMSX_ERR_INVALID;
        if (scale > 30) return GMSX_ERR_OVERFLOW;
        if (generator != GMSX_GEN_KRONECKER && generator != GMSX_GEN_UNIFORM) return GMSX_ERR_INVALID;
    #ifdef _OPENMP
        struct Threads {
            int saved, set;
            ~Threads() { if (set > 0) omp_set_num_threads(saved); }
        } threads_guard{omp_get_max_threads(), threads};
        if (threads > 0) omp_set_num_threads(threads);
    #else
        (void)threads;
    #endif
        int rc;
        {
            Csr g;
            {
                PhaseTimer pt;
                EdgeList el;
                rc = generator == GMSX_GEN_UNIFORM ? make_uniform(scale, degree, el) : make_rmat(scale, degree, el);
                pt.lap("generate edge list");
                if (!rc) rc = build_from_el(el, -1, true, g);
            }
            PhaseTimer pf;
            if (!rc) rc = finish(std::move(g), relabel, out);
            pf.lap("relabel decision + relabel");
        }
        return rc;
    });
}

int gmsx_csr_generate_rmat(int scale, int degree, double a, double b, double c, int relabel, int threads, gmsx_csr **out) {
    return gmsx::guard([&]() -> int {
        if (!out || scale < 1 || degree < 1 || relabel < 0 || relabel > 2) return GMSX_ERR_INVALID;
        if (!(a > 0 && b >= 0 && c >= 0 && a + b + c < 1.0)) return GMSX_ERR_INVALID;
        if (scale > 30) return GMSX_ERR_OVERFLOW;
    #ifdef _OPENMP
        struct Threads {
            int saved, set;
            ~Threads() { if (set > 0) omp_set_num_threads(saved); }
        } threads_guard{omp_get_max_threads(), threads};
        if (threads > 0) omp_set_num_threads(threads);
    #else
        (void)threads;
    #endif
        int rc;
        {
            Csr g;
            {
                EdgeList el;
                rc = make_rmat(scale, degree, el, float(a), float(b), float(c));
                if (!rc) rc = build_from_el(el, -1, true, g);
            }
            if (!rc) rc = finish(std::move(g), relabel, out);
        }
        return rc;
    });
}

int gmsx_csr_from_edges(int64_t num_nodes, int64_t num_edges, const int32_t *src, const int32_t *dst,
                        int symmetrize, int relabel, gmsx_csr **out) {
    return gmsx::guard([&]() -> int {
        if (!out || num_edges < 0 || (num_edges && (!src || !dst)) || relabel < 0 || relabel > 2) return GMSX_ERR_INVALID;
        EdgeList el;
        if (int rc = el.alloc(num_edges)) return rc;
        if (num_edges) {
            std::memcpy(el.u.get(), src, size_t(num_edges) * 4);
            std::memcpy(el.v.get(), dst, size_t(num_edges) * 4);
        }
        Csr g;
        if (int rc = build_from_el(el, num_nodes, symmetrize != 0, g)) return rc;
        return finish(std::move(g), relabel, out);
    });
}

int gmsx_csr_load(const char *path, int symmetrize, int relabel, gmsx_csr **out) {
    return gmsx::guard([&]() -> int {
        if (!path || !out || relabel < 0 || relabel > 2) return GMSX_ERR_INVALID;
        const std::string p(path), suf = suffix_of(p);
        Csr g;
        if (suf == ".sg") {
            if (int rc = read_sg(p, g)) return rc;
        } else if (suf == ".sgx") {
            if (int rc = read_sgx(p, g)) return rc;
        } else if (suf == ".el" || suf == ".wel" || suf == ".gr" || suf == ".graph" || suf == ".mtx") {
            EdgeList el;
            const int rc = suf == ".el" ? read_el(p, el) : suf == ".wel" ? read_wel(p, el) : suf == ".gr" ? read_gr(p, el)
                         : suf == ".graph" ? read_metis(p, el) : read_mtx(p, el);
            if (rc) return rc;
            if (int rc2 = build_from_el(el, -1, symmetrize != 0, g)) return rc2;
        } else {
            return GMSX_ERR_FORMAT;
        }
        return finish(std::move(g), relabel, out);
    });
}

int gmsx_csr_save_sg(const gmsx_csr *h, const char *path) {
    return gmsx::guard([&]() -> int {
        if (!h || !path) return GMSX_ERR_INVALID;
        std::FILE *f = std::fopen(path, "wb");
        if (!f) return GMSX_ERR_IO;
        const Csr &g = h->g;
        const unsigned char directed = g.directed ? 1 : 0;
        bool ok = std::fwrite(&directed, 1, 1, f) == 1 && std::fwrite(&g.nnz, 8, 1, f) == 1 &&
                  std::fwrite(&g.n, 8, 1, f) == 1 && std::fwrite(g.off.get(), 8, size_t(g.n + 1), f) == size_t(g.n + 1) &&
                  (g.nnz == 0 || std::fwrite(g.neigh.get(), 4, size_t(g.nnz), f) == size_t(g.nnz));
        ok = (std::fclose(f) == 0) && ok;
        return ok ? GMSX_OK : GMSX_ERR_IO;
    });
}

int gmsx_csr_save_sgx(const gmsx_csr *h, const char *path) {
    return gmsx::guard([&]() -> int {
        if (!h || !path) return GMSX_ERR_INVALID;
        return write_sgx(h->g, path);
    });
}
int gmsx_csr_is_mapped(const gmsx_csr *h) { return h ? int(h->g.mapped) : GMSX_ERR_INVALID; }

int gmsx_csr_from_arrays(int64_t n, const int64_t *offsets, const int32_t *neigh, gmsx_csr **out) {
    return gmsx::guard([&]() -> int {
        if (!out || n < 0 || !offsets || n > std::numeric_limits<int32_t>::max()) return GMSX_ERR_INVALID;
        if (offsets[0] != 0) return GMSX_ERR_INVALID;
// ... 109 lines not shown
```

Before: 15.64 billion.

## Split tail row ids into separate low and high 16-bit key planes

Adds a new tail-row storage form, enabled by default, where each 32-bit neighbor id is split into a low-16 plane in tpool and a high-16 plane in a parallel tpool_hi buffer, packing 8 ids per unit. The tail intersection kernels probe the hash table using the low halves first and queue candidates, then resolve them with a second pass that reads the high halves. The aim is to cut the bytes streamed per probe on the hot path. In exchange it adds an extra pool allocation, a shared-memory key queue with an extra synchronisation and resolve pass, and it replaces delta encoding for tail rows.

Result: no change. 15.68 billion (median of 6 runs) (+0.3%).

```diff
diff --git a/gms_amd/csrc/hip/device_graph.hip b/gms_amd/csrc/hip/device_graph.hip
--- a/gms_amd/csrc/hip/device_graph.hip
+++ b/gms_amd/csrc/hip/device_graph.hip
@@ -349,16 +349,16 @@
     }
     return units;
 }
-__global__ void k_trow_sizes(int64_t n, const int64_t *__restrict__ toff, const int32_t *__restrict__ tadj, int delta_mode,
+__global__ void k_trow_sizes(int64_t n, const int64_t *__restrict__ toff, const int32_t *__restrict__ tadj, int delta_mode, int keys,
                              int64_t *__restrict__ units_out, int64_t *__restrict__ small_out, uint32_t *__restrict__ real_out, unsigned char *__restrict__ form_out) {
     const int64_t v = int64_t(blockIdx.x) * blockDim.x + threadIdx.x;
     if (v > n) return;
     if (v == n) { units_out[n] = 0; small_out[n] = 0; return; }
     const int64_t b = toff[v];
     const int len = int(toff[v + 1] - b);
-    uint32_t best = uint32_t((len + 3) / 4);
-    int form = kFormList;
-    if (len >= 8 && delta_mode > 0) {
+    uint32_t best = keys ? uint32_t((len + 7) / 8) : uint32_t((len + 3) / 4);
+    int form = keys ? kFormKeys : kFormList;
+    if (!keys && len >= 8 && delta_mode > 0) {
         const uint32_t d = tail_delta_encode(tadj + b, len, nullptr);
         if (delta_mode == 2 || d * 100u <= best * 85u) { best = d; form = kFormDelta; }
     }
@@ -370,7 +370,7 @@
 }
 __global__ void k_trow_fill(int64_t n, const int64_t *__restrict__ toff, const int32_t *__restrict__ tadj, const int64_t *__restrict__ uoff,
                             const int64_t *__restrict__ soff, const uint32_t *__restrict__ real, const unsigned char *__restrict__ form,
-                            unsigned long long *__restrict__ trow, uint32_t *__restrict__ tpool) {
+                            unsigned long long *__restrict__ trow, uint32_t *__restrict__ tpool, uint32_t *__restrict__ tpool_hi) {
     const int64_t v = int64_t(blockIdx.x) * blockDim.x + threadIdx.x;
     if (v >= n) return;
     const int64_t units = int64_t(real[v]);
@@ -380,7 +380,14 @@
     uint32_t *dst = tpool + u0 * 4;
     const int64_t b = toff[v];
     const int64_t len = toff[v + 1] - b;
-    if (form[v] == kFormDelta) tail_delta_encode(tadj + b, int(len), dst);
+    if (form[v] == kFormKeys) {
+        uint16_t *lo = reinterpret_cast<uint16_t *>(dst), *hi = reinterpret_cast<uint16_t *>(tpool_hi + u0 * 4);
+        for (int64_t w = 0; w < units * 8; ++w) {
+            const uint32_t id = w < len ? uint32_t(tadj[b + w]) : 0xfffffffeu;
+            lo[w] = uint16_t(id);
+            hi[w] = uint16_t(id >> 16);
+        }
+    } else if (form[v] == kFormDelta) tail_delta_encode(tadj + b, int(len), dst);
     else
         for (int64_t w = 0; w < units * 4; ++w) dst[w] = w < len ? uint32_t(tadj[b + w]) : 0xfffffffeu;
 }
@@ -461,7 +468,8 @@
                                                      unsigned long long *__restrict__ cnt_h,
                                                      unsigned long long *__restrict__ cnt_t, const int64_t *__restrict__ ihoff,
                                                      const int64_t *__restrict__ itoff, int64_t base_h, uint16_t *__restrict__ pool_h, int64_t base_t,
-                                                     int32_t *__restrict__ pool_t) {
+                                                     int32_t *__restrict__ pool_t, uint16_t *__restrict__ pool_thi) {
+    const bool keys = pool_thi != nullptr;
     const int lane = threadIdx.x & 63;
     const int64_t wave0 = (int64_t(blockIdx.x) * blockDim.x + threadIdx.x) >> 6;
     const int64_t nwaves = (int64_t(gridDim.x) * blockDim.x) >> 6;
@@ -491,24 +499,29 @@
         } else {
             int64_t at_h = 0, at_t = 0;
             if (nh) at_h = (base_h + ihoff[mv]) * 8 + int64_t(atomicAdd(&cnt_h[mv], (unsigned long long)nh));
-            if (nt) at_t = (base_t + itoff[mv]) * 4 + int64_t(atomicAdd(&cnt_t[mv], (unsigned long long)nt));
+            if (nt) at_t = (base_t + itoff[mv]) * (keys ? 8 : 4) + int64_t(atomicAdd(&cnt_t[mv], (unsigned long long)nt));
             for (int k = 0; k < nhub; ++k) {
                 const int32_t x = __shfl(mv, k);
                 if (k < nh) pool_h[at_h + k] = uint16_t(x);
             }
             for (int k = 0; k < tl; ++k) {
                 const int32_t x = __shfl(mv, hl + k);
-                if (k < nt) pool_t[at_t + k] = x;
+                if (k < nt) {
+                    if (keys) {
+                        reinterpret_cast<uint16_t *>(pool_t)[at_t + k] = uint16_t(uint32_t(x));
+                        pool_thi[at_t + k] = uint16_t(uint32_t(x) >> 16);
+                    } else pool_t[at_t + k] = x;
+                }
             }
         }
     }
 }
-__global__ void k_inline_units(int64_t n, const unsigned long long *__restrict__ ids_h, const unsigned long long *__restrict__ ids_t,
+__global__ void k_inline_units(int64_t n, const unsigned long long *__restrict__ ids_h, const unsigned long long *__restrict__ ids_t, int keys,
                                int64_t *__restrict__ units_h, int64_t *__restrict__ units_t) {
     const int64_t v = int64_t(blockIdx.x) * blockDim.x + threadIdx.x;
     if (v > n) return;
     units_h[v] = v < n ? int64_t((ids_h[v] + 7) / 8) : 0;
-    units_t[v] = v < n ? int64_t((ids_t[v] + 3) / 4) : 0;
+    units_t[v] = v < n ? int64_t(keys ? (ids_t[v] + 7) / 8 : (ids_t[v] + 3) / 4) : 0;
 }
 static constexpr int kDefaultHotWindows = 0, kDefaultHotKB = 2048, kDefaultHotMin = 16;
 __device__ __forceinline__ int64_t receiver_of(int32_t w, const int32_t *__restrict__ dplus, const int32_t *__restrict__ opos, const int64_t *__restrict__ lidx,
@@ -533,7 +546,7 @@
 __global__ void k_inline_entries(int64_t n, const int32_t *__restrict__ dplus, const int32_t *__restrict__ opos, const int64_t *__restrict__ lidx, int64_t n_heavy,
                                  int32_t inline_limit, const int64_t *__restrict__ ihoff, const int64_t *__restrict__ itoff, int64_t base_h, int64_t base_t,
                                  uint32_t *__restrict__ cnt, uint32_t *__restrict__ cur, const int64_t *__restrict__ hbeg, const int64_t *__restrict__ tbeg,
-                                 TaskList htask, TaskList ttask, unsigned long long *__restrict__ totals, TcClasses cc) {
+                                 TaskList htask, TaskList ttask, int keys, unsigned long long *__restrict__ totals, TcClasses cc) {
     const int kClasses = cc.count();
     const int64_t v = int64_t(blockIdx.x) * blockDim.x + threadIdx.x;
     if (v >= n) return;
@@ -551,7 +564,7 @@
     }
     for (int64_t o = 0; o < ut; o += kInlineChunk) {
         const unsigned long long units = (unsigned long long)min(int64_t(kInlineChunk), ut - o);
-        const unsigned long long d = ((unsigned long long)(base_t + itoff[v] + o) << 24) | ((unsigned long long)kFormList << 22) | units;
+        const unsigned long long d = ((unsigned long long)(base_t + itoff[v] + o) << 24) | ((unsigned long long)(keys ? kFormKeys : kFormList) << 22) | units;
         const int cls = tail_class(cc, d);
         if (!FILL) atomicAdd(&c[cls], 1u);
         else ttask.put(tbeg[p] + c[cls] + atomicAdd(&cur[p * kClasses + cls], 1u), d);
@@ -627,6 +640,7 @@
 }
 __device__ __forceinline__ uint32_t cut_tail_units(const uint32_t *__restrict__ tpool, unsigned long long d, int below, int32_t v) {
     const uint32_t units = uint32_t(d) & 0x3fffffu, form = (uint32_t(d) >> 22) & 3u;
+    if (form == kFormKeys) return min(units, uint32_t(below + 7) / 8u);
     if (form != kFormDelta) return min(units, uint32_t(below + 3) / 4u);
     const uint4 *row = reinterpret_cast<const uint4 *>(tpool) + (d >> 24);
     uint32_t lo = 0, hi = units;
@@ -815,7 +829,7 @@
         p = nullptr;
     };
     drop(g->tsplit); drop(g->srow); drop(g->srow2); drop(g->ksplit); drop(g->spool); drop(g->trow); drop(g->htask.lo); drop(g->htask.hi); drop(g->ttask.lo); drop(g->ttask.hi); drop(g->hitem); drop(g->titem); drop(g->tunits);
-    drop(g->ledge); drop(g->tpool); drop(g->shard_hitem); drop(g->shard_titem);
+    drop(g->ledge); drop(g->tpool); drop(g->tpool_hi); drop(g->shard_hitem); drop(g->shard_titem);
     g->shard_idx_part = g->shard_idx_nparts = -1;
     g->device_bytes -= g->tc_bytes;
     g->tc_bytes = 0;
@@ -855,6 +869,7 @@
     (void)hipFree(g->shard_titem);
     (void)hipFree(g->ledge);
     (void)hipFree(g->tpool);
+    (void)hipFree(g->tpool_hi);
     (void)hipFree(g->dplus);
     (void)hipFree(g->order);
     (void)hipFree(g->kc_rel);
@@ -1197,6 +1212,8 @@
     const uint32_t flags = g->upload_flags;
     const int hub_limit = g->hub_limit;
     const unsigned tb = unsigned((n + 255) / 256);
+    g->tail_keys = opt_int("TC_TAIL_KEYS", 1) != 0;
+    g->ttask.keys = g->tail_keys;
     int32_t *opos = nullptr;
     if (int rc = dmalloc(&opos, n + 1, nullptr)) return rc;
     DevGuard g_opos{opos};
@@ -1247,13 +1264,13 @@
         if (n_work > 0)
             hipLaunchKernelGGL(k_inline_rows<false>, dim3(grid_for_waves(n_work)), dim3(256), 0, s, int64_t(0), n_work, g->order, g->hoff, g->hadj,
                                g->toff, g->tadj, g->dplus, g->inline_limit, g->inline_first, opos, g->shard_nparts, g->shard_part, inl_h, inl_t, ihoff, itoff, int64_t(0), static_cast<uint16_t *>(nullptr),
-                               int64_t(0), static_cast<int32_t *>(nullptr));
+                               int64_t(0), static_cast<int32_t *>(nullptr), static_cast<uint16_t *>(nullptr));
         int64_t *uh = nullptr, *ut = nullptr;
         if (int rc = dmalloc(&uh, n + 1, nullptr)) return rc;
         DevGuard g_uh{uh};
         if (int rc = dmalloc(&ut, n + 1, nullptr)) return rc;
         DevGuard g_ut{ut};
-        hipLaunchKernelGGL(k_inline_units, dim3(unsigned(n / 256 + 1)), dim3(256), 0, s, n, inl_h, inl_t, uh, ut);
+        hipLaunchKernelGGL(k_inline_units, dim3(unsigned(n / 256 + 1)), dim3(256), 0, s, n, inl_h, inl_t, int(g->tail_keys), uh, ut);
         if (int rc = exclusive_scan_i64(uh, ihoff, n + 1, s)) return rc;
         if (int rc = exclusive_scan_i64(ut, itoff, n + 1, s)) return rc;
         GMSX_HIP(hipMemcpy(&inline_h_units, ihoff + n, sizeof(int64_t), hipMemcpyDeviceToHost));
@@ -1342,7 +1359,7 @@
         DevGuard g_r{real};
         if (int rc = dmalloc(&form, n + 1, nullptr)) return rc;
         DevGuard g_f{form};
-        hipLaunchKernelGGL(k_trow_sizes, dim3(unsigned(n / 256 + 1)), dim3(256), 0, s, n, g->toff, g->tadj, delta_mode, units, small, real, form);
+        hipLaunchKernelGGL(k_trow_sizes, dim3(unsigned(n / 256 + 1)), dim3(256), 0, s, n, g->toff, g->tadj, delta_mode, int(g->tail_keys), units, small, real, form);
         if (int rc = exclusive_scan_i64(units, uoff, n + 1, s)) return rc;
         if (int rc = exclusive_scan_i64(small, soff, n + 1, s)) return rc;
         int64_t big_units = 0, small_units = 0;
@@ -1353,9 +1370,14 @@
         if (g->tpool_units >= (int64_t(1) << 40)) return GMSX_ERR_DEVICE_MEM;
         if (int rc = dmalloc(&g->trow, n, g)) return rc;
         if (int rc = dmalloc(&g->tpool, (g->tpool_units + kPoolSlack) * 4, g)) return rc;
-        GMSX_HIP(hipMemsetD32Async(reinterpret_cast<hipDeviceptr_t>(g->tpool), int(0xFFFFFFFEu), size_t(g->tpool_units + kPoolSlack) * 4, s));
+        if (g->tail_keys) {
+            if (int rc = dmalloc(&g->tpool_hi, (g->tpool_units + kPoolSlack) * 4, g)) return rc;
+            GMSX_HIP(hipMemsetD32Async(reinterpret_cast<hipDeviceptr_t>(g->tpool), int(0xFFFEFFFEu), size_t(g->tpool_units + kPoolSlack) * 4, s));
+            GMSX_HIP(hipMemsetD32Async(reinterpret_cast<hipDeviceptr_t>(g->tpool_hi), int(0xFFFFFFFFu), size_t(g->tpool_units + kPoolSlack) * 4, s));
+        } else
+            GMSX_HIP(hipMemsetD32Async(reinterpret_cast<hipDeviceptr_t>(g->tpool), int(0xFFFFFFFEu), size_t(g->tpool_units + kPoolSlack) * 4, s));
         if (n > 0)
-            hipLaunchKernelGGL(k_trow_fill, dim3(unsigned((n + 255) / 256)), dim3(256), 0, s, n, g->toff, g->tadj, uoff, soff, real, form, g->trow, g->tpool);
+            hipLaunchKernelGGL(k_trow_fill, dim3(unsigned((n + 255) / 256)), dim3(256), 0, s, n, g->toff, g->tadj, uoff, soff, real, form, g->trow, g->tpool, g->tpool_hi);
         GMSX_HIP(hipStreamSynchronize(s));
     }
 
@@ -1365,7 +1387,7 @@
         GMSX_HIP(hipMemsetAsync(inl_t, 0, size_t(n + 1) * sizeof(unsigned long long), s));
         hipLaunchKernelGGL(k_inline_rows<true>, dim3(grid_for_waves(n_work)), dim3(256), 0, s, int64_t(0), n_work, g->order, g->hoff, g->hadj, g->toff,
                            g->tadj, g->dplus, g->inline_limit, g->inline_first, opos, g->shard_nparts, g->shard_part, inl_h, inl_t, ihoff, itoff, inline_h_base, reinterpret_cast<uint16_t *>(g->spool),
-                           inline_t_base, reinterpret_cast<int32_t *>(g->tpool));
+                           inline_t_base, reinterpret_cast<int32_t *>(g->tpool), reinterpret_cast<uint16_t *>(g->tpool_hi));
     }
     pt.mark("inline rows fill");
     {
@@ -1451,7 +1473,7 @@
         }
         if (n > 0)
             hipLaunchKernelGGL(k_inline_entries<false>, dim3(vb), dim3(256), 0, s, n, g->dplus, opos, lidx, n_heavy, g->inline_limit, ihoff, itoff, inline_h_base,
-                               inline_t_base, cnt, cur, hbeg, tbeg, TaskList{}, TaskList{}, totals, cc);
+                               inline_t_base, cnt, cur, hbeg, tbeg, TaskList{}, TaskList{}, int(g->tail_keys), totals, cc);
         if (n_heavy > 0)
             hipLaunchKernelGGL(k_task_lists<false>, dim3(grid), dim3(256), 0, s, n_heavy, g->order, g->hoff, g->hadj, g->toff, g->tadj, g->dplus, g->srow, g->srow2, g->ksplit, g->trow,
                                two_sided, opos, cnt, cur, hbeg, tbeg, TaskList{}, TaskList{}, g->tunits,
@@ -1475,7 +1497,7 @@
         if (int rc = dmalloc(&g->ttask.hi, g->ttask_entries + 2, g)) return rc;
         if (n > 0)
             hipLaunchKernelGGL(k_inline_entries<true>, dim3(vb), dim3(256), 0, s, n, g->dplus, opos, lidx, n_heavy, g->inline_limit, ihoff, itoff, inline_h_base,
-                               inline_t_base, cnt, cur, hbeg, tbeg, g->htask, g->ttask, totals, cc);
+                               inline_t_base, cnt, cur, hbeg, tbeg, g->htask, g->ttask, int(g->tail_keys), totals, cc);
         if (n_heavy > 0)
             hipLaunchKernelGGL(k_task_lists<true>, dim3(grid), dim3(256), 0, s, n_heavy, g->order, g->hoff, g->hadj, g->toff, g->tadj, g->dplus, g->srow, g->srow2, g->ksplit, g->trow,
                                two_sided, opos, cnt, cur, hbeg, tbeg, g->htask, g->ttask, g->tunits, totals + 2, g->spool, g->tpool, g->inline_limit, g->inline_first, g->shard_nparts, g->shard_part, cc);
diff --git a/gms_amd/csrc/hip/device_graph.hpp b/gms_amd/csrc/hip/device_graph.hpp
--- a/gms_amd/csrc/hip/device_graph.hpp
+++ b/gms_amd/csrc/hip/device_graph.hpp
@@ -28,11 +28,12 @@
     uint32_t *lo = nullptr;
     uint16_t *hi = nullptr;
     bool tail = false;
-    __host__ __device__ TaskList at(int64_t first) const { return TaskList{lo + first, hi + first, tail}; }
+    bool keys = false;
+    __host__ __device__ TaskList at(int64_t first) const { return TaskList{lo + first, hi + first, tail, keys}; }
     __device__ __forceinline__ unsigned long long get(int64_t i) const {
         const uint32_t l = lo[i], h = hi[i];
         const unsigned long long first = ((unsigned long long)h << 16) | (l >> 16);
-        const uint32_t form = tail ? ((l >> 15) & 1u) << 1 : (l >> 14) & 3u, units = tail ? l & kTaskTailUnitsMax : l & kTaskHubUnitsMax;
+        const uint32_t form = tail ? ((l >> 15) & 1u) * (keys ? 3u : 2u) : (l >> 14) & 3u, units = tail ? l & kTaskTailUnitsMax : l & kTaskHubUnitsMax;
         return (first << 24) | ((unsigned long long)form << 22) | units;
     }
     __device__ __forceinline__ void put(int64_t i, unsigned long long d) const {
@@ -81,6 +82,8 @@
     int64_t inline_units = 0;
     unsigned long long *trow = nullptr;
     uint32_t *tpool = nullptr;
+    uint32_t *tpool_hi = nullptr;
+    bool tail_keys = false;
     int64_t tpool_units = 0;
     int32_t *tsplit = nullptr;
     int64_t dense_rows = 0, bmpool_words = 0;
@@ -127,6 +130,7 @@
 static constexpr int kBitmapWords = 2048;
 static constexpr int kAccWords = 64 * 16 + 16;
 static constexpr int kFormList = 0, kFormBitset = 1, kFormDelta = 2, kFormGap12 = 3;
+static constexpr int kFormKeys = 3;
 static constexpr int kPoolSlack = 64;
 static constexpr int kTaskChunk = 512;
 static constexpr int kLenClasses = 12;
@@ -152,7 +156,7 @@
     return cc.phase(d) * kHubClasses + int((uint32_t(d) >> 22) & 3u) * kLenClasses + length_class(uint32_t(d) & 0x3fffffu);
 }
 __host__ __device__ inline int tail_class(const TcClasses &cc, unsigned long long d) {
-    return cc.tail_base() + (((uint32_t(d) >> 22) & 3u) == 2u ? kLenClasses : 0) + length_class(uint32_t(d) & 0x3fffffu);
+    return cc.tail_base() + (((uint32_t(d) >> 22) & 3u) >= 2u ? kLenClasses : 0) + length_class(uint32_t(d) & 0x3fffffu);
 }
 __host__ __device__ inline void hub_phase_range(const TcClasses &cc, const uint32_t *c, int64_t len, int ph, int64_t *b, int64_t *e) {
     int64_t start = 0;
diff --git a/gms_amd/csrc/hip/tc.hip b/gms_amd/csrc/hip/tc.hip
--- a/gms_amd/csrc/hip/tc.hip
+++ b/gms_amd/csrc/hip/tc.hip
@@ -132,6 +132,49 @@
     const uint32_t id[6] = {id0, id1, id2, id3, id4, id5};
     return probe_set_bits(tbl, mask, shift, m, id);
 }
+static constexpr uint32_t kKeyQueue = 256;
+struct KeyQueue {
+    uint32_t n, pad;
+    uint2 e[kKeyQueue];
+};
+__device__ __forceinline__ uint32_t tail_key_unit_hits(const uint32_t *flt, uint4 p) {
+    const uint32_t w0 = flt_word(flt, p.x), w1 = flt_word(flt, p.x >> 16), w2 = flt_word(flt, p.y), w3 = flt_word(flt, p.y >> 16),
+                   w4 = flt_word(flt, p.z), w5 = flt_word(flt, p.z >> 16), w6 = flt_word(flt, p.w), w7 = flt_word(flt, p.w >> 16);
+    if (((w0 | w1 | w2 | w3 | w4 | w5 | w6 | w7) & 1u) == 0) return 0u;
+    return (w0 & 1u) | ((w1 & 1u) << 1) | ((w2 & 1u) << 2) | ((w3 & 1u) << 3) | ((w4 & 1u) << 4) | ((w5 & 1u) << 5) | ((w6 & 1u) << 6) | ((w7 & 1u) << 7);
+}
+__device__ __forceinline__ uint32_t probe_key_unit(const int32_t *tbl, uint32_t mask, int shift, uint4 lo, uint4 hi, uint32_t m) {
+    uint32_t c = 0;
+    while (m) {
+        const uint32_t k = uint32_t(__ffs(int(m)) - 1);
+        m &= m - 1u;
+        const uint32_t b1 = (k >> 1) & 1u, b2 = k >> 2, sh = (k & 1u) << 4;
+        const uint32_t wl = pick(b2, pick(b1, lo.x, lo.y), pick(b1, lo.z, lo.w)), wh = pick(b2, pick(b1, hi.x, hi.y), pick(b1, hi.z, hi.w));
+        c += set_contains(tbl, mask, shift, int32_t(((wh >> sh) << 16) | ((wl >> sh) & 0xffffu)));
+    }
+    return c;
+}
+__device__ __forceinline__ uint32_t tail_key_step(const uint32_t *flt, const int32_t *tbl, uint32_t mask, int shift, KeyQueue &q, const uint4 *__restrict__ hi4, uint4 p,
+                                                  uint32_t unit) {
+    const uint32_t m = tail_key_unit_hits(flt, p);
+    if (m == 0u) return 0u;
+    const uint32_t slot = atomicAdd(&q.n, 1u);
+    if (slot < kKeyQueue) {
+        q.e[slot] = make_uint2(unit, m);
+        return 0u;
+    }
+    return probe_key_unit(tbl, mask, shift, p, hi4[unit], m);
+}
+__device__ __forceinline__ uint32_t resolve_key_queue(const KeyQueue &q, const int32_t *tbl, uint32_t mask, int shift, const uint4 *__restrict__ lo4,
+                                                      const uint4 *__restrict__ hi4, int tid) {
+    const uint32_t n = min(uni32(q.n), kKeyQueue);
+    uint32_t c = 0;
+    for (uint32_t i = uint32_t(tid); i < n; i += 256u) {
+        const uint2 e = q.e[i];
+        c += probe_key_unit(tbl, mask, shift, lo4[e.x], hi4[e.x], e.y);
+    }
+    return c;
+}
 static constexpr int kBlockLog = 10;
 template <int FORM>
 __device__ __forceinline__ uint32_t hub_unit_hits(const uint32_t *bm, uint4 p, int j) {
@@ -163,7 +206,7 @@
     uint32_t lo[kTaskChunk];
     uint32_t hi[kTaskChunk / 2 + 2];
 };
-template <int W, int D, bool TAIL>
+template <int W, int D, bool TAIL, bool KEYS = false>
 struct StepStream {
     static constexpr int G = 256 / W;
     const uint32_t *slo;
@@ -171,6 +214,7 @@
     const uint4 *pool4;
     int hi, sub;
     int e, units, last, lim, j, form;
+    uint32_t ru;
     const uint4 *row;
     int pending;
     static constexpr int S = D == 1 ? 2 : D;
@@ -180,7 +224,8 @@
         int ee = e;
         asm volatile("" : "+v"(ee));
         const uint32_t l = e < hi ? slo[ee] : 0u, h = e < hi ? uint32_t(shi[ee]) : 0u;
-        row = pool4 + __builtin_amdgcn_alignbit(h, l, 16);
+        ru = __builtin_amdgcn_alignbit(h, l, 16);
+        row = pool4 + ru;
         units = int(l & (TAIL ? kTaskTailUnitsMax : kTaskHubUnitsMax));
         form = TAIL ? int((l >> 15) & 1u) << 25 : int((l >> 14) & 3u) << 24;
         last = max(units - 1, 0);
@@ -189,7 +234,7 @@
     }
     __device__ __forceinline__ void issue(int k) {
         p[k] = row[uint32_t(min(j, last))];
-        pj[k] = j < units ? (j | form) : -1;
+        pj[k] = j < units ? (KEYS ? int(ru + uint32_t(j)) : (j | form)) : -1;
         pending += e < hi ? 1 : 0;
         j += W;
         if (j >= lim) {
@@ -217,9 +262,11 @@
                 pending -= 1;
                 issue(nxt);
 #ifdef GMSX_TC_NO_PROBE
-                if (pj[cur] >= 0) cnt += p[cur].x & 1u;
+                if (KEYS ? pj[cur] != -1 : pj[cur] >= 0) cnt += p[cur].x & 1u;
 #else
-                if (pj[cur] >= 0) cnt += hit(p[cur], pj[cur] & 0xffffff, pj[cur] >> 24);
+                if constexpr (KEYS) {
+                    if (pj[cur] != -1) cnt += hit(p[cur], pj[cur], 0);
+                } else if (pj[cur] >= 0) cnt += hit(p[cur], pj[cur] & 0xffffff, pj[cur] >> 24);
 #endif
             };
             while (pending > 0) {
@@ -237,9 +284,11 @@
                 pending -= 1;
                 issue(k);
 #ifdef GMSX_TC_NO_PROBE
-                if (jc >= 0) cnt += pc.x & 1u;
+                if (KEYS ? jc != -1 : jc >= 0) cnt += pc.x & 1u;
 #else
-                if (jc >= 0) cnt += hit(pc, jc & 0xffffff, jc >> 24);
+                if constexpr (KEYS) {
+                    if (jc != -1) cnt += hit(pc, jc, 0);
+                } else if (jc >= 0) cnt += hit(pc, jc & 0xffffff, jc >> 24);
 #endif
             }
         }
@@ -301,13 +350,15 @@
     block_add(cnt, red, lane, wave, tid, acc);
 }
 
+template <bool KEYS>
 __global__ __launch_bounds__(256) __attribute__((amdgpu_waves_per_eu(8, 8))) void k_tc_tail(const int64_t *__restrict__ toff, const int32_t *__restrict__ tadj,
-                                                 const uint32_t *__restrict__ tpool, const TaskList ttask,
+                                                 const uint32_t *__restrict__ tpool, const uint32_t *__restrict__ tpool_hi, const TaskList ttask,
                                                  const gmsx_tc_item *__restrict__ items, unsigned long long *__restrict__ acc) {
     __shared__ __attribute__((aligned(16))) int32_t tbl[1 << kBlockLog];
     __shared__ __attribute__((aligned(16))) uint32_t flt[kFilterWords];
     __shared__ StagedTasks sdesc;
     __shared__ unsigned long long red[4];
+    __shared__ KeyQueue kq;
     constexpr int TILE = (1 << kBlockLog) / 2;
     const int tid = threadIdx.x, lane = tid & 63, wave = tid >> 6;
     const gmsx_tc_item &it = items[blockIdx.x];
@@ -326,6 +377,7 @@
         __syncthreads();
         for (int i = tid; i < size; i += 256) tbl[i] = -1;
         reinterpret_cast<uint4 *>(flt)[tid] = make_uint4(0u, 0u, 0u, 0u);
+        if (KEYS && tid == 0) kq.n = 0u;
         __syncthreads();
         for (int i = tid; i < tn; i += 256) {
             const int32_t t = tadj[tb + t0 + i];
@@ -334,9 +386,18 @@
         }
         __syncthreads();
 #ifndef GMSX_TC_STAGING_ONLY
-        StepStream<GMSX_TC_TAIL_GROUP, GMSX_TC_TAIL_DEPTH, true> st;
-        st.start(sdesc, 0, tpool, 0, ne, tid);
-        cnt += st.run([mask, shift](uint4 p, int, int f) { return tail_hits_by_form(flt, tbl, mask, shift, p, f); });
+        if constexpr (KEYS) {
+            const uint4 *lo4 = reinterpret_cast<const uint4 *>(tpool), *hi4 = reinterpret_cast<const uint4 *>(tpool_hi);
+            StepStream<GMSX_TC_TAIL_GROUP, GMSX_TC_TAIL_DEPTH, true, true> st;
+            st.start(sdesc, 0, tpool, 0, ne, tid);
+            cnt += st.run([mask, shift, hi4](uint4 p, int unit, int) { return tail_key_step(flt, tbl, mask, shift, kq, hi4, p, uint32_t(unit)); });
+            __syncthreads();
+            cnt += resolve_key_queue(kq, tbl, mask, shift, lo4, hi4, tid);
+        } else {
+            StepStream<GMSX_TC_TAIL_GROUP, GMSX_TC_TAIL_DEPTH, true> st;
+            st.start(sdesc, 0, tpool, 0, ne, tid);
+            cnt += st.run([mask, shift](uint4 p, int, int f) { return tail_hits_by_form(flt, tbl, mask, shift, p, f); });
+        }
 #endif
     }
     block_add(cnt, red, lane, wave, tid, acc);
@@ -365,9 +426,9 @@
     unsigned long long red[4];
     int chunk[2];
 };
-template <bool TAIL>
-__device__ __forceinline__ void item_loop(ItemLds &L, const uint16_t *__restrict__ hadj, const int32_t *__restrict__ tadj, const uint32_t *__restrict__ pool,
-                                          const TaskList task, const gmsx_tc_item *__restrict__ items, int n_items,
+template <bool TAIL, bool KEYS>
+__device__ __forceinline__ void item_loop(ItemLds &L, KeyQueue &kq, const uint16_t *__restrict__ hadj, const int32_t *__restrict__ tadj, const uint32_t *__restrict__ pool,
+                                          const uint32_t *__restrict__ pool_hi, const TaskList task, const gmsx_tc_item *__restrict__ items, int n_items,
                                           unsigned int *__restrict__ qhead, unsigned long long &total) {
     constexpr int TILE = (1 << kBlockLog) / 2;
     const int tid = threadIdx.x, lane = tid & 63, wave = tid >> 6;
@@ -447,7 +508,7 @@
         const StagedTasks &sd = L.sdesc[buf];
         const int neA = int(uni32(recA[1]) >> 8), oddA = int(uni32(recA[0]) & 1u);
         uint32_t c = 0;
-        StepStream<TAIL ? GMSX_TC_TAIL_GROUP : GMSX_TC_HUB_GROUP, TAIL ? GMSX_TC_TAIL_DEPTH : GMSX_TC_HUB_DEPTH, TAIL> st;
+        StepStream<TAIL ? GMSX_TC_TAIL_GROUP : GMSX_TC_HUB_GROUP, TAIL ? GMSX_TC_TAIL_DEPTH : GMSX_TC_HUB_DEPTH, TAIL, KEYS> st;
 #ifndef GMSX_TC_STAGING_ONLY
         if (!TAIL) st.start(sd, oddA, pool, 0, neA, tid);
 #endif
@@ -487,6 +548,7 @@
                 if (t0 > 0) __syncthreads();
                 for (int i = tid; i < size; i += 256) tbl[i] = -1;
                 reinterpret_cast<uint4 *>(flt)[tid] = make_uint4(0u, 0u, 0u, 0u);
+                if (KEYS && tid == 0) kq.n = 0u;
                 __syncthreads();
                 int tin = tid0;
                 asm volatile("" : "+v"(tin));
@@ -500,6 +562,13 @@
                 if (!staged && fetch) L.chunk[1] = pend < unsigned(n_items) ? int(pend) : -1;
                 staged = true;
 #ifndef GMSX_TC_STAGING_ONLY
+                if constexpr (KEYS) {
+                    const uint4 *hi4 = reinterpret_cast<const uint4 *>(pool_hi);
+                    st.start(sd, oddA, pool, 0, neA, tid);
+                    c += st.run([=, &kq](uint4 p, int unit, int) { return tail_key_step(flt, tbl, mask, shift, kq, hi4, p, uint32_t(unit)); });
+                    __syncthreads();
+                    c += resolve_key_queue(kq, tbl, mask, shift, reinterpret_cast<const uint4 *>(pool), hi4, tid);
+                } else {
                 const int nl = int(uni32(recA[8]) & 0xffffu);
                 if (nl > 0) {
                     st.start(sd, oddA, pool, 0, nl, tid);
@@ -509,6 +578,7 @@
                     st.start(sd, oddA, pool, nl, neA, tid);
                     c += st.run([=](uint4 p, int, int) { return tail_delta_unit_hits(flt, tbl, mask, shift, p); });
                 }
+                }
 #endif
             }
             if (!staged) {
@@ -531,14 +601,16 @@
 #ifndef GMSX_TC_TAIL_MIN_WAVES
 #define GMSX_TC_TAIL_MIN_WAVES 8
 #endif
-template <bool TAIL>
+template <bool TAIL, bool KEYS = false>
 __global__ __launch_bounds__(256) __attribute__((amdgpu_waves_per_eu(TAIL ? GMSX_TC_TAIL_MIN_WAVES : GMSX_TC_HUB_MIN_WAVES, 8))) void k_tc_items(
-    const uint16_t *__restrict__ hadj, const int32_t *__restrict__ tadj, const uint32_t *__restrict__ pool, const TaskList task,
+    const uint16_t *__restrict__ hadj, const int32_t *__restrict__ tadj, const uint32_t *__restrict__ pool, const uint32_t *__restrict__ pool_hi, const TaskList task,
     const gmsx_tc_item *__restrict__ items, int n_items, unsigned int *__restrict__ qhead, unsigned long long *__restrict__ acc) {
+    static_assert(TAIL || !KEYS, "key rows are tail rows");
     __shared__ __attribute__((aligned(16))) ItemLds L;
+    __shared__ KeyQueue kq;
     const int tid = threadIdx.x;
     unsigned long long total = 0;
-    item_loop<TAIL>(L, hadj, tadj, pool, task, items, n_items, qhead, total);
+    item_loop<TAIL, KEYS>(L, kq, hadj, tadj, pool, pool_hi, task, items, n_items, qhead, total);
     block_add(total, L.red, tid & 63, tid >> 6, tid, acc);
 }
 
@@ -713,7 +785,7 @@
     unsigned long long probes = 0, bytes = 0;
     auto slots = [tail](unsigned long long d) -> unsigned long long {
         const unsigned long long n = d & 0x3fffffull, f = (d >> 22) & 3ull;
-        return n * (tail ? (f == kFormDelta ? 6ull : 4ull) : (f == kFormList ? 8ull : f == kFormDelta ? 14ull : f == kFormGap12 ? 10ull : 4ull));
+        return n * (tail ? (f == kFormKeys ? 8ull : f == kFormDelta ? 6ull : 4ull) : (f == kFormList ? 8ull : f == kFormDelta ? 14ull : f == kFormGap12 ? 10ull : 4ull));
     };
     for (int64_t q = wave0; q < n_items; q += nwaves) {
         const gmsx_tc_item &it = items[q];
@@ -1018,12 +1090,16 @@
             return unsigned(std::max<int64_t>(1, std::min<int64_t>((n + kGrab - 1) / kGrab, int64_t(cus) * (wgs_env > 0 ? wgs_env : wgs))));
         };
         if (n_hitems > 0) {
-            hipLaunchKernelGGL(k_tc_items<false>, dim3(grid(n_hitems, GMSX_TC_HUB_MIN_WAVES)), dim3(256), 0, s, g->hadj, g->tadj, g->spool, g->htask, hitem, int(n_hitems), qhead, acc);
+            hipLaunchKernelGGL(k_tc_items<false>, dim3(grid(n_hitems, GMSX_TC_HUB_MIN_WAVES)), dim3(256), 0, s, g->hadj, g->tadj, g->spool, static_cast<const uint32_t *>(nullptr), g->htask, hitem, int(n_hitems), qhead, acc);
             ++launches;
         }
         if (n_titems > 0) {
-            hipLaunchKernelGGL(k_tc_items<true>, dim3(grid(n_titems, GMSX_TC_TAIL_MIN_WAVES)), dim3(256), 0, s, g->hadj, g->tadj, g->tpool, g->ttask, titem, int(n_titems),
-                               qhead + kQueueStride, acc);
+            if (g->tail_keys)
+                hipLaunchKernelGGL((k_tc_items<true, true>), dim3(grid(n_titems, GMSX_TC_TAIL_MIN_WAVES)), dim3(256), 0, s, g->hadj, g->tadj, g->tpool, g->tpool_hi, g->ttask, titem,
+                                   int(n_titems), qhead + kQueueStride, acc);
+            else
+                hipLaunchKernelGGL(k_tc_items<true>, dim3(grid(n_titems, GMSX_TC_TAIL_MIN_WAVES)), dim3(256), 0, s, g->hadj, g->tadj, g->tpool, g->tpool_hi, g->ttask, titem,
+                                   int(n_titems), qhead + kQueueStride, acc);
             ++launches;
         }
     } else {
@@ -1032,7 +1108,10 @@
             ++launches;
         }
         if (n_titems > 0) {
-            hipLaunchKernelGGL(k_tc_tail, dim3(unsigned(n_titems)), dim3(256), 0, side_tail ? c.side[0] : s, g->toff, g->tadj, g->tpool, g->ttask, titem, acc);
+            if (g->tail_keys)
+                hipLaunchKernelGGL(k_tc_tail<true>, dim3(unsigned(n_titems)), dim3(256), 0, side_tail ? c.side[0] : s, g->toff, g->tadj, g->tpool, g->tpool_hi, g->ttask, titem, acc);
+            else
+                hipLaunchKernelGGL(k_tc_tail<false>, dim3(unsigned(n_titems)), dim3(256), 0, side_tail ? c.side[0] : s, g->toff, g->tadj, g->tpool, g->tpool_hi, g->ttask, titem, acc);
             ++launches;
         }
     }
diff --git a/gms_amd/csrc/host/loader.cpp b/gms_amd/csrc/host/loader.cpp
--- a/gms_amd/csrc/host/loader.cpp
+++ b/gms_amd/csrc/host/loader.cpp
@@ -675,7 +675,7 @@
 Option g_options[] = {
     {"TIMING", "", false}, {"MEM_TRACE", "", false}, {"BK_VERBOSE", "", false},
     {"INLINE_LIMIT", "", false}, {"TC_INLINE_FIRST", "", false}, {"TC_DELTA", "", false}, {"TC_DELTA_PCT", "", false}, {"TC_GAP12", "", false},
-    {"TC_HYBRID", "", false}, {"TC_TAIL_DELTA", "", false}, {"TC_TWO_SIDED", "", false}, {"TC_HOT_WINDOWS", "", false}, {"TC_HOT_KB", "", false},
+    {"TC_HYBRID", "", false}, {"TC_TAIL_DELTA", "", false}, {"TC_TAIL_KEYS", "", false}, {"TC_TWO_SIDED", "", false}, {"TC_HOT_WINDOWS", "", false}, {"TC_HOT_KB", "", false},
     {"TC_HOT_MIN", "", false}, {"TC_TEST_MAX_UNITS", "", false}, {"TC_KEEP_ROWS", "", false}, {"TC_MEM_LIMIT_MB", "", false}, {"TC_OVERLAP", "", false},
     {"TC_PERSIST", "", false}, {"TC_ITEM_WGS", "", false}, {"SORT_CHUNK", "", false}, {"UPLOAD_STAGED", "", false}, {"INIT_LAZY", "", false},
     {"KC_SLAB_MB", "", false}, {"KC_MAXD", "", false}, {"KC_STREAMS", "", false}, {"KC_PIPE_ALL", "", false}, {"KC_STREAM_BUILD", "", false},
```
